# kornelski/cavif-rs

Measured on AMD Instinct MI355X. Metric: MPix/s encoded at speed=4 q=80, 1080p batch; bit-exact vs CPU oracle, higher is better.
Workload: dtype u16 samples / i32 transform / i64 RD cost

## Files before the change

### cavif_rs_amd/csrc/dev_predict.h

```cpp
#pragma once
#include "dev_common.h"

#define EDGE_OFF 16
#define EDGE_LEN(N) (EDGE_OFF + 2 * (N) + 16)

__device__ __forceinline__ const uint8_t *sm_weights_dev(int log2w) {
  static __device__ const uint8_t sw[124] = { 255, 149, 85, 64,
                                              255, 197, 146, 105, 73, 50, 37, 32,
                                              255, 225, 196, 170, 145, 123, 102, 84, 68, 54, 43, 33, 26, 20, 17, 16,
                                              255, 240, 225, 210, 196, 182, 169, 157, 145, 133, 122, 111, 101, 92, 83, 74,
                                              66, 59, 52, 45, 39, 34, 29, 25, 21, 17, 14, 12, 10, 9, 8, 8,
                                              255, 248, 240, 233, 225, 218, 210, 203, 196, 189, 182, 176, 169, 163, 156, 150,
                                              144, 138, 133, 127, 121, 116, 111, 106, 101, 96, 91, 86, 82, 77, 73, 69,
                                              65, 61, 57, 54, 50, 47, 44, 41, 38, 35, 32, 29, 27, 25, 22, 20,
                                              18, 16, 15, 13, 12, 10, 9, 8, 7, 6, 6, 5, 5, 4, 4, 4 };
  const int l = ((log2w >= 2) & (log2w <= 5)) ? log2w : 6;
  return sw + ((1 << l) - 4);
}
__device__ __forceinline__ int dr_deriv_dev(int a) {
  const int aa = (unsigned)a < 90u ? a : 0;
  const int k = (aa * 43) >> 7;
  const unsigned long long w01 = k < 8 ? 0x97b2d7117423ff00ULL : 0x4047505a00667484ULL, w23 = k < 24 ? 0x171b1f23282d3339ULL : 0x000003070b000f13ULL;
  const unsigned long long w = k < 16 ? w01 : w23;
  const int v = lut8(w, k & 7) | ((int)((0x16cULL >> (2 * k)) & 3) << 8);
  const int r = (int)((0xf035554000eaaa03ULL >> (2 * k)) & 3);
  return aa - 3 * k == r ? v : 0;
}
__device__ __forceinline__ int edge_strength_dev(int w, int h, int ft, int delta) {
  const int d = imin_(iabs_(delta), 254), blk = w + h;
  const int c = (blk > 8) + (blk > 12) + (blk > 16) + (blk > 24) + (blk > 32);
  const unsigned long long t1 = ft == 0 ? 0x010108282838ULL : 0x010104141428ULL, t2 = ft == 0 ? 0x010410ffffffULL : 0x010104303040ULL;
  const unsigned long long t3 = ft == 0 ? 0x012020ffffffULL : 0x010104ffffffULL;
  return (d >= lut8(t1, c)) + (d >= lut8(t2, c)) + (d >= lut8(t3, c));
}
__device__ __forceinline__ int edge_upsample_sel_dev(int w, int h, int ft, int delta) {
  const int d = iabs_(delta), blk = w + h;
  return (int)((d > 0) & (d < 40) & (blk <= (ft == 0 ? 16 : 8)));
}
__device__ __forceinline__ void dr_dxdy_dev(int pa, int *dx, int *dy) {
  *dx = dr_deriv_dev(pa < 90 ? pa : 180 - pa);
  *dy = dr_deriv_dev(pa < 180 ? pa - 90 : 270 - pa);
}
static __device__ const uint32_t dr_dxdy_tab[91] = {
    0x300000, 0x0003ff, 0x000223, 0x000174, 0x200111, 0x2000d7, 0x2000b2, 0x200097, 0x200084, 0x200074, 0x200066, 0x300000, 0x00005a,
    0x000050, 0x000047, 0x000040, 0x000039, 0x000033, 0x00002d, 0x100028, 0x100023, 0x10001f, 0x10001b, 0x100017, 0x100013, 0x10000f,
    0x300000, 0x00000b, 0x000007, 0x000003, 0x300000, 0x0ffc03, 0x088c07, 0x05d00b, 0x24440f, 0x235c13, 0x22c817, 0x225c1b, 0x22101f,
    0x21d023, 0x219828, 0x300000, 0x01682d, 0x014033, 0x011c39, 0x010040, 0x00e447, 0x00cc50, 0x00b45a, 0x10a066, 0x108c74, 0x107c84,
    0x106c97, 0x105cb2, 0x104cd7, 0x103d11, 0x300000, 0x002d74, 0x001e23, 0x000fff, 0x300000, 0x000c00, 0x001c00, 0x002c00, 0x203c00,
    0x204c00, 0x205c00, 0x206c00, 0x207c00, 0x208c00, 0x20a000, 0x300000, 0x00b400, 0x00cc00, 0x00e400, 0x010000, 0x011c00, 0x014000,
    0x016800, 0x119800, 0x11d000, 0x121000, 0x125c00, 0x12c800, 0x135c00, 0x144400, 0x300000, 0x05d000, 0x088c00, 0x0ffc00, 0x300000 };
__device__ __forceinline__ void dr_dxdy_uni(int pa, int *dx, int *dy) {
  const int p = (unsigned)pa <= 270u ? pa : 0, k = (p * 683) >> 11;
  const uint32_t e = dr_dxdy_tab[k];
  const bool has = p - 3 * k == (int)(e >> 20);
  *dx = has ? (int)(e & 1023) : 0; *dy = has ? (int)((e >> 10) & 1023) : 0;
}

__device__ inline void load_edges(const LDS FrameDev *f, int plane, int x, int y, int n, int have_left, int have_above,
                                  int have_ar, int have_bl, LDS uint16_t *above , LDS uint16_t *left) {
  const int bd = f->bd, rs = f->stride;
  const uint16_t *rec = f->rec[plane];
  const int max_x = f->mi_cols * 4 - 1, max_y = f->mi_rows * 4 - 1;
  const int tot = 2 * n;
  const int na = x + (have_ar ? 2 * n : n) - 1, nl = y + (have_bl ? 2 * n : n) - 1;
  const int lim_a = imin_(max_x, na), lim_l = imin_(max_y, nl);
  for (int i = LANE; i <= tot; i += 64) {
    const bool corner = i == tot;
    int ia, il;
    if (have_above) ia = (y - 1) * rs + (corner ? (have_left ? x - 1 : x) : imin_(lim_a, x + i));
    else ia = y * rs + (have_left ? x - 1 : x);
    if (have_left) il = imin_(lim_l, y + i) * rs + x - 1;
    else il = (have_above ? y - 1 : y) * rs + x;
    uint16_t a = rec[ia], l = rec[il];
    if (!have_above && !have_left) { a = (uint16_t)(corner ? (1 << (bd - 1)) : (1 << (bd - 1)) - 1); l = (uint16_t)((1 << (bd - 1)) + 1); }
    if (corner) { above[-1] = a; left[-1] = a; }
    else { above[i] = a; left[i] = l; }
  }
  WAVE_SYNC();
}

__device__ inline void edge_filter_dev(LDS uint16_t *buf, int sz, int strength, LDS uint16_t *tmp) {
  if (!strength) return;
  for (int i = LANE; i < sz; i += 64) tmp[i] = buf[i - 1];
  WAVE_SYNC();
  for (int i = 1 + LANE; i < sz; i += 64) {
    int s = 0;
#pragma unroll
    for (int j = 0; j < 5; j++) {
      const int k = iclamp_(i - 2 + j, 0, sz - 1);
      const int kw = strength == 1 ? (j == 0 || j == 4 ? 0 : (j == 2 ? 8 : 4)) : (strength == 2 ? (j == 0 || j == 4 ? 0 : (j == 2 ? 6 : 5)) : (j == 0 || j == 4 ? 2 : 4));
      s += kw * tmp[k];
    }
    buf[i - 1] = (uint16_t)((s + 8) >> 4);
  }
  WAVE_SYNC();
}
__device__ inline void edge_upsample_dev(LDS uint16_t *buf, int num_px, int bd, LDS uint16_t *tmp) {
  for (int i = LANE; i < num_px + 3; i += 64) {
    uint16_t v;
    if (i == 0) v = buf[-1]; else if (i == num_px + 2) v = buf[num_px - 1]; else v = buf[i - 2];
    tmp[i] = v;
  }
  WAVE_SYNC();
  const int mx = (1 << bd) - 1;
  if (LANE == 0) buf[-2] = tmp[0];
  for (int i = LANE; i < num_px; i += 64) {
    int s = -(int)tmp[i] + 9 * (int)tmp[i + 1] + 9 * (int)tmp[i + 2] - (int)tmp[i + 3];
    s = iclamp_(round2_(s, 4), 0, mx);
    buf[2 * i - 1] = (uint16_t)s;
    buf[2 * i] = tmp[i + 2];
  }
  WAVE_SYNC();
}

__device__ inline void predict_block(const LDS FrameDev *f, int x, int y, int log2w, int have_left, int have_above,
                                     int mode, int angle_delta, int ftype, const LDS uint16_t *ra, const LDS uint16_t *rl,
                                     LDS uint16_t *wa, LDS uint16_t *wl, LDS uint16_t *tmp, LDS uint16_t *pred) {
  const int n = 1 << log2w, bd = f->bd, nn = n * n;
  const int max_x = f->mi_cols * 4 - 1, max_y = f->mi_rows * 4 - 1;
  if (mode == PAETH_PRED) {
    const int tl = ra[-1];
    for (int idx = LANE; idx < nn; idx += 64) {
      const int i = idx >> log2w, j = idx & (n - 1);
      const int base = ra[j] + rl[i] - tl;
      const int pl = iabs_(base - rl[i]), pt = iabs_(base - ra[j]), ptl = iabs_(base - tl);
      pred[idx] = (pl <= pt && pl <= ptl) ? rl[i] : (pt <= ptl ? ra[j] : (uint16_t)tl);
    }
  } else if (mode == DC_PRED) {
    int v;
    if (have_left || have_above) {
      int s = 0;
      for (int k = LANE; k < n; k += 64) s += (have_above ? ra[k] : 0) + (have_left ? rl[k] : 0);
      s = wave_sum_i32(s);
      if (have_left && have_above) v = (s + n) / (2 * n);
      else v = (s + (n >> 1)) >> log2w;
    } else v = 1 << (bd - 1);
    for (int idx = LANE; idx < nn; idx += 64) pred[idx] = (uint16_t)v;
  } else if (mode == SMOOTH_PRED || mode == SMOOTH_V_PRED || mode == SMOOTH_H_PRED) {
    const uint8_t *sw = sm_weights_dev(log2w);
    const int bl = rl[n - 1], tr = ra[n - 1];
    for (int idx = LANE; idx < nn; idx += 64) {
      const int i = idx >> log2w, j = idx & (n - 1);
      int p;
      if (mode == SMOOTH_PRED) p = round2_(sw[i] * ra[j] + (256 - sw[i]) * bl + sw[j] * rl[i] + (256 - sw[j]) * tr, 9);
      else if (mode == SMOOTH_V_PRED) p = round2_(sw[i] * ra[j] + (256 - sw[i]) * bl, 8);
      else p = round2_(sw[j] * rl[i] + (256 - sw[j]) * tr, 8);
      pred[idx] = (uint16_t)p;
    }
  } else {
    const int pa = mode_angle_of(mode) + angle_delta * 3;
    for (int i = LANE; i < 2 * n + 1; i += 64) { wa[i - 1] = ra[i - 1]; wl[i - 1] = rl[i - 1]; }
    WAVE_SYNC();
    int up_a = 0, up_l = 0;
    if (pa != 90 && pa != 180) {
      if (pa > 90 && pa < 180 && 2 * n >= 24) {
        if (LANE == 0) { const int v = round2_(wl[0] * 5 + wa[-1] * 6 + wa[0] * 5, 4); wa[-1] = (uint16_t)v; wl[-1] = (uint16_t)v; }
        WAVE_SYNC();
      }
      if (have_above) {
        const int st = edge_strength_dev(n, n, ftype, pa - 90);
        const int num = imin_(n, max_x - x + 1) + (pa < 90 ? n : 0) + 1;
        edge_filter_dev(wa, num, st, tmp);
      }
      if (have_left) {
        const int st = edge_strength_dev(n, n, ftype, pa - 180);
        const int num = imin_(n, max_y - y + 1) + (pa > 180 ? n : 0) + 1;
        edge_filter_dev(wl, num, st, tmp);
      }
    }
    up_a = edge_upsample_sel_dev(n, n, ftype, pa - 90);
    if (up_a) edge_upsample_dev(wa, n + (pa < 90 ? n : 0), bd, tmp);
    up_l = edge_upsample_sel_dev(n, n, ftype, pa - 180);
    if (up_l) edge_upsample_dev(wl, n + (pa > 180 ? n : 0), bd, tmp);
    int dx, dy;
    dr_dxdy_dev(pa, &dx, &dy);
    for (int idx = LANE; idx < nn; idx += 64) {
      const int i = idx >> log2w, j = idx & (n - 1);
      int v;
      if (pa < 90) {
        const int max_base = (2 * n - 1) << up_a;
        const int id = (i + 1) * dx, base = (id >> (6 - up_a)) + (j << up_a), sh = ((id << up_a) >> 1) & 0x1F;
        v = base < max_base ? round2_(wa[base] * (32 - sh) + wa[base + 1] * sh, 5) : wa[max_base];
      } else if (pa > 90 && pa < 180) {
        int id = (j << 6) - (i + 1) * dx, base = id >> (6 - up_a);
        if (base >= -(1 << up_a)) { const int sh = ((id << up_a) >> 1) & 0x1F; v = round2_(wa[base] * (32 - sh) + wa[base + 1] * sh, 5); }
        else { id = (i << 6) - (j + 1) * dy; base = id >> (6 - up_l); const int sh = ((id << up_l) >> 1) & 0x1F; v = round2_(wl[base] * (32 - sh) + wl[base + 1] * sh, 5); }
      } else if (pa > 180) {
        const int id = (j + 1) * dy, base = (id >> (6 - up_l)) + (i << up_l), sh = ((id << up_l) >> 1) & 0x1F;
        v = round2_(wl[base] * (32 - sh) + wl[base + 1] * sh, 5);
      } else if (pa == 90) v = wa[j];
      else v = wl[i];
      pred[idx] = (uint16_t)v;
    }
  }
  WAVE_SYNC();
}

__device__ inline void predict_cfl_dev(const LDS FrameDev *f, int x, int y, int log2w, int alpha, const LDS uint16_t *dcp, LDS uint16_t *out) {
  const int n = 1 << log2w, nn = n * n, mx = (1 << f->bd) - 1, rs = f->stride;
  const uint16_t *luma = f->rec[0] + y * rs + x;
  int s = 0;
  for (int idx = LANE; idx < nn; idx += 64) s += luma[(idx >> log2w) * rs + (idx & (n - 1))] << 3;
  s = wave_sum_i32(s);
  const int avg = round2_(s, 2 * log2w);
  for (int idx = LANE; idx < nn; idx += 64) {
    const int l = (luma[(idx >> log2w) * rs + (idx & (n - 1))] << 3) - avg;
    const int v = alpha * l;
    const int sc = v >= 0 ? round2_(v, 6) : -round2_(-v, 6);
    out[idx] = (uint16_t)iclamp_(dcp[idx] + sc, 0, mx);
  }
  WAVE_SYNC();
}
```

### cavif_rs_amd/csrc/dev_rate.h

```cpp
#pragma once
#include "dev_common.h"

template <typename FP, typename TP> __device__ inline void txb_ctx_dev(FP f, TP t, int plane, int r4, int c4, int txs, int bs, int *skip_ctx, int *dc_ctx) {
  const int w4 = 1 << txs, ms = f->mi_stride;
  int top = 0, left = 0, dcs = 0, any_a = 0, any_l = 0;
  const int k = LANE;
  if (k < w4) {
    const bool ha = r4 - 1 >= t->mi_row_start && c4 + k < f->mi_cols, hl = c4 - 1 >= t->mi_col_start && r4 + k < f->mi_rows;
    const int ia = ha ? (r4 - 1) * ms + c4 + k : r4 * ms + c4, il = hl ? (r4 + k) * ms + c4 - 1 : r4 * ms + c4;
    const int la = f->m_lvl[plane][ia], da = f->m_dc[plane][ia], ll = f->m_lvl[plane][il], dl = f->m_dc[plane][il];
    if (ha) { top = la; any_a = la | da; dcs += da == 1 ? -1 : (da == 2 ? 1 : 0); }
    if (hl) { left = ll; any_l = ll | dl; dcs += dl == 1 ? -1 : (dl == 2 ? 1 : 0); }
  }
  top = wave_max_i32(top); left = wave_max_i32(left); dcs = wave_sum_i32(dcs);
  any_a = wave_or_i32(any_a); any_l = wave_or_i32(any_l);
  *dc_ctx = dcs < 0 ? 1 : (dcs > 0 ? 2 : 0);
  if (plane == 0) {
    int ctx;
    if (bs == txs) ctx = 0;
    else if (top == 0 && left == 0) ctx = 1;
    else if (top == 0 || left == 0) ctx = 2 + (imax_(top, left) > 3);
    else if (imax_(top, left) <= 3) ctx = 4;
    else if (imin_(top, left) <= 3) ctx = 5;
    else ctx = 6;
    *skip_ctx = ctx;
  } else {
    *skip_ctx = 7 + (any_a != 0) + (any_l != 0) + (bs > txs ? 3 : 0);
  }
}
template <typename FP, typename TP> __device__ inline void txb_ctx_wh(FP f, TP t, int plane, int r4, int c4, int w4, int h4, int whole, int *skip_ctx, int *dc_ctx) {
  const int ms = f->mi_stride;
  int top = 0, left = 0, dcs = 0, any_a = 0, any_l = 0;
  const int k = LANE;
  if (k < imax_(w4, h4)) {
    const bool ha = k < w4 && r4 - 1 >= t->mi_row_start && c4 + k < f->mi_cols, hl = k < h4 && c4 - 1 >= t->mi_col_start && r4 + k < f->mi_rows;
    const int ia = ha ? (r4 - 1) * ms + c4 + k : r4 * ms + c4, il = hl ? (r4 + k) * ms + c4 - 1 : r4 * ms + c4;
    const int la = f->m_lvl[plane][ia], da = f->m_dc[plane][ia], ll = f->m_lvl[plane][il], dl = f->m_dc[plane][il];
    if (ha) { top = la; any_a = la | da; dcs += da == 1 ? -1 : (da == 2 ? 1 : 0); }
    if (hl) { left = ll; any_l = ll | dl; dcs += dl == 1 ? -1 : (dl == 2 ? 1 : 0); }
  }
  top = wave_max_i32(top); left = wave_max_i32(left); dcs = wave_sum_i32(dcs);
  any_a = wave_or_i32(any_a); any_l = wave_or_i32(any_l);
  *dc_ctx = dcs < 0 ? 1 : (dcs > 0 ? 2 : 0);
  if (plane == 0) {
    int ctx;
    if (whole) ctx = 0;
    else if (top == 0 && left == 0) ctx = 1;
    else if (top == 0 || left == 0) ctx = 2 + (imax_(top, left) > 3);
    else if (imax_(top, left) <= 3) ctx = 4;
    else if (imin_(top, left) <= 3) ctx = 5;
    else ctx = 6;
    *skip_ctx = ctx;
  } else *skip_ctx = 7 + (any_a != 0) + (any_l != 0) + (whole ? 0 : 3);
}

__device__ __forceinline__ int eob_to_pt(int eob) { return eob < 3 ? eob : (32 - __clz(eob - 1) + 1); }
__device__ __forceinline__ int eob_pt_cdf(int eob_multi, int pt, int cls) {
  const int off[7] = { CDF_EOB_PT_16, CDF_EOB_PT_32, CDF_EOB_PT_64, CDF_EOB_PT_128, CDF_EOB_PT_256, CDF_EOB_PT_512, CDF_EOB_PT_1024 };
  const int str[7] = { CDF_EOB_PT_16_STRIDE, CDF_EOB_PT_32_STRIDE, CDF_EOB_PT_64_STRIDE, CDF_EOB_PT_128_STRIDE,
                       CDF_EOB_PT_256_STRIDE, CDF_EOB_PT_512_STRIDE, CDF_EOB_PT_1024_STRIDE };
  return off[eob_multi] + (pt * 2 + (cls == TXC_2D ? 0 : 1)) * str[eob_multi];
}
__device__ __forceinline__ int base_ctx(const LDS uint8_t *L, int st, int cls, int row, int col) {
  int mag = imin_(L[1], 3) + imin_(L[st], 3);
  if (cls == TXC_2D) {
    mag += imin_(L[st + 1], 3) + imin_(L[2], 3) + imin_(L[2 * st], 3);
    const int m = imin_((mag + 1) >> 1, 4);
    if (row == 0 && col == 0) return 0;
    if (row + col < 2) return m + 1;
    if (row + col < 4) return m + 6;
    return m + 21;
  } else if (cls == TXC_VERT) {
    mag += imin_(L[2 * st], 3) + imin_(L[3 * st], 3) + imin_(L[4 * st], 3);
    const int m = imin_((mag + 1) >> 1, 4);
    return m + (row == 0 ? 26 : (row == 1 ? 31 : 36));
  }
  mag += imin_(L[2], 3) + imin_(L[3], 3) + imin_(L[4], 3);
  const int m = imin_((mag + 1) >> 1, 4);
  return m + (col == 0 ? 26 : (col == 1 ? 31 : 36));
}
__device__ __forceinline__ int br_ctx(const LDS uint8_t *L, int st, int cls, int row, int col, int c) {
  int mag = imin_(L[1], 15) + imin_(L[st], 15);
  if (cls == TXC_2D) { mag += imin_(L[st + 1], 15); mag = imin_((mag + 1) >> 1, 6); return c == 0 ? mag : ((row < 2 && col < 2) ? mag + 7 : mag + 14); }
  if (cls == TXC_HORIZ) { mag += imin_(L[2], 15); mag = imin_((mag + 1) >> 1, 6); return c == 0 ? mag : (col == 0 ? mag + 7 : mag + 14); }
  mag += imin_(L[2 * st], 15); mag = imin_((mag + 1) >> 1, 6); return c == 0 ? mag : (row == 0 ? mag + 7 : mag + 14);
}

__device__ inline void build_level_map(const LDS int32_t *qc, LDS uint8_t *lev, int n) {
  const int st = n + 4, words = (st * st + 3) >> 2, bwl = n == 4 ? 2 : n == 8 ? 3 : n == 16 ? 4 : 5;
  LDS uint32_t *lw = (LDS uint32_t *)lev;
  for (int i = LANE; i < words; i += 64) lw[i] = 0;
  WAVE_SYNC();
  for (int i = LANE; i < n * n; i += 64) lev[(i >> bwl) * st + (i & (n - 1))] = (uint8_t)imin_(iabs_(qc[i]), 127);
  WAVE_SYNC();
}

struct CoefCost { const LDS uint16_t *txb, *eobx, *dcs, *br, *base, *beob, *eobpt[4]; };
__device__ __forceinline__ int coef_cost_entries(int maxtxs) {
  const int t = maxtxs + 1, tb = imin_(maxtxs, 3) + 1;
  return t * 13 * CDF_TXB_SKIP_STRIDE + t * 18 * CDF_EOB_EXTRA_STRIDE + 6 * CDF_DC_SIGN_STRIDE + tb * 42 * CDF_COEFF_BR_STRIDE +
         t * 84 * CDF_COEFF_BASE_STRIDE + t * 8 * CDF_COEFF_BASE_EOB_STRIDE + 4 * (CDF_EOB_PT_16_STRIDE + CDF_EOB_PT_64_STRIDE + CDF_EOB_PT_256_STRIDE + CDF_EOB_PT_1024_STRIDE);
}
#define COEF_COST_MAX_ENTRIES(maxtxs) (((maxtxs) + 1) * (13 * 3 + 18 * 3 + 84 * 5 + 8 * 4) + 18 + ((maxtxs) < 3 ? (maxtxs) + 1 : 4) * 42 * 5 + 4 * (6 + 8 + 10 + 12))
__device__ __forceinline__ CoefCost coef_cost_layout(const LDS uint16_t *dst, int maxtxs, int *src_off = nullptr, int *count = nullptr) {
  const int t = maxtxs + 1, tb = imin_(maxtxs, 3) + 1;
  const int src[10] = { CDF_TXB_SKIP, CDF_EOB_EXTRA, CDF_DC_SIGN, CDF_COEFF_BR, CDF_COEFF_BASE, CDF_COEFF_BASE_EOB, CDF_EOB_PT_16, CDF_EOB_PT_64, CDF_EOB_PT_256, CDF_EOB_PT_1024 };
  const int cnt[10] = { t * 13 * CDF_TXB_SKIP_STRIDE, t * 18 * CDF_EOB_EXTRA_STRIDE, 6 * CDF_DC_SIGN_STRIDE, tb * 42 * CDF_COEFF_BR_STRIDE, t * 84 * CDF_COEFF_BASE_STRIDE,
                        t * 8 * CDF_COEFF_BASE_EOB_STRIDE, 4 * CDF_EOB_PT_16_STRIDE, 4 * CDF_EOB_PT_64_STRIDE, 4 * CDF_EOB_PT_256_STRIDE, 4 * CDF_EOB_PT_1024_STRIDE };
  int o[10]; int acc = 0;
#pragma unroll
  for (int i = 0; i < 10; i++) { o[i] = acc; acc += cnt[i]; if (src_off) src_off[i] = src[i]; if (count) count[i] = cnt[i]; }
  CoefCost cc;
  cc.txb = dst + o[0]; cc.eobx = dst + o[1]; cc.dcs = dst + o[2]; cc.br = dst + o[3]; cc.base = dst + o[4]; cc.beob = dst + o[5];
  cc.eobpt[0] = dst + o[6]; cc.eobpt[1] = dst + o[7]; cc.eobpt[2] = dst + o[8]; cc.eobpt[3] = dst + o[9];
  return cc;
}
__device__ inline void load_coef_cost(LDS uint16_t *dst, const uint16_t *cost, int maxtxs, int tid, int nthreads) {
  int src[10], cnt[10];
  coef_cost_layout(dst, maxtxs, src, cnt);
  int o = 0;
  for (int k = 0; k < 10; k++) { for (int i = tid; i < cnt[k]; i += nthreads) dst[o + i] = cost[src[k] + i]; o += cnt[k]; }
}

template <typename CostPtr> __device__ inline uint32_t coef_rate_dev(const CoefCost &cc, CostPtr cost, const LDS uint16_t *ls, const LDS int32_t *qc, int eob, int plane, int txs, int txtype,
                                         int skip_ctx, int dc_ctx, int tx_off, int tx_sym, LDS uint8_t *lev, int *cul_out, int *dc_cat) {
  const int n = imin_(32, 4 << txs), bwl = n == 4 ? 2 : n == 8 ? 3 : n == 16 ? 4 : 5;
  const int pt = plane > 0, cls = tx_class_of(txtype), txs_ctx = txs;
  *cul_out = 0; *dc_cat = 0;
  uint32_t head = cc.txb[(txs_ctx * 13 + skip_ctx) * CDF_TXB_SKIP_STRIDE + (eob == 0)];
  if (eob == 0) return head;
  if (tx_off >= 0) head += cost[tx_off + tx_sym];
  const int eob_pt = eob_to_pt(eob), eob_multi = 2 * bwl - 4;
  {
    static_assert(CDF_EOB_PT_16_STRIDE == 6 && CDF_EOB_PT_64_STRIDE == 8 && CDF_EOB_PT_256_STRIDE == 10 && CDF_EOB_PT_1024_STRIDE == 12, "stride = 6 + 2 sq");
    const int sq = eob_multi >> 1;
    head += cc.eobpt[sq][(pt * 2 + (cls == TXC_2D ? 0 : 1)) * (6 + 2 * sq) + eob_pt - 1];
  }
  if (eob_pt >= 3) {
    const int nb = eob_pt - 2, rem = eob - ((1 << (eob_pt - 2)) + 1), hi = (rem >> (nb - 1)) & 1;
    head += cc.eobx[((txs_ctx * 2 + pt) * 9 + (eob_pt - 3)) * CDF_EOB_EXTRA_STRIDE + hi];
    head += 512u * (uint32_t)(nb - 1);
  }
  build_level_map(qc, lev, n);
  const int st = n + 4, area = n * n;
  int bits = 0; int cul = 0, dcc = 0;
  for (int c = LANE; c < eob; c += 64) {
    const int p = scan_pos(ls, n, cls, c), row = p >> bwl, col = p & (n - 1);
    const int v = qc[p], level = iabs_(v);
    const LDS uint8_t *L = lev + row * st + col;
    if (c == eob - 1) {
      const int ctx = c == 0 ? 0 : (c <= area / 8 ? 1 : (c <= area / 4 ? 2 : 3));
      bits += cc.beob[((txs_ctx * 2 + pt) * 4 + ctx) * CDF_COEFF_BASE_EOB_STRIDE + imin_(level, 3) - 1];
    } else {
      const int ctx = base_ctx(L, st, cls, row, col);
      bits += cc.base[((txs_ctx * 2 + pt) * 42 + ctx) * CDF_COEFF_BASE_STRIDE + imin_(level, 3)];
    }
    if (level > 2) {
      const int ctx = br_ctx(L, st, cls, row, col, c);
      const int off = ((imin_(txs_ctx, 3) * 2 + pt) * 21 + ctx) * CDF_COEFF_BR_STRIDE;
      int rem = level - 3;
      for (int idx = 0; idx < 4; idx++) { const int s = imin_(rem, 3); bits += cc.br[off + s]; rem -= s; if (s < 3) break; }
    }
    if (level) {
      if (c == 0) { bits += cc.dcs[(pt * 3 + dc_ctx) * CDF_DC_SIGN_STRIDE + (v < 0)]; dcc = v < 0 ? 1 : 2; }
      else bits += 512;
      if (level > 14) { const int len = 32 - __clz(level - 14); bits += 512 * (2 * len - 1); }
    }
    cul += level;
  }
  bits = wave_sum_i32(bits);
  cul = wave_sum_i32(imin_(cul, 1 << 20));
  dcc = __builtin_amdgcn_readfirstlane(dcc);
  *cul_out = imin_(cul, 63); *dc_cat = dcc;
  return head + (uint32_t)bits;
}

#define LEV_OFF(cs) ((cs) == 4 ? 0 : (cs) == 8 ? 64 : (cs) == 16 ? 64 + 144 : 64 + 144 + 400)
#define LEV_BYTES(maxcs) ((maxcs) == 4 ? 64 : (maxcs) == 8 ? 64 + 144 : (maxcs) == 16 ? 64 + 144 + 400 : 64 + 144 + 400 + 1296)

template <int CS, typename CostPtr>
__device__ inline int quant_rate_dev(const CoefCost &cc, CostPtr cost, const LDS uint16_t *ls, LDS int32_t *cbuf, LDS int32_t *qc, LDS uint8_t *levbase,
                                     int plane, int txs, int txtype, int dcq, int acq, uint32_t dc_recip, uint32_t ac_recip, int bd,
                                     int skip_ctx, int dc_ctx, int tx_off, int tx_sym, uint32_t *rate_out, int *cul_out, int *dc_cat) {
  constexpr int n = CS, nc = CS * CS, IT = nc < 64 ? 1 : nc / 64, bwl = CS == 4 ? 2 : CS == 8 ? 3 : CS == 16 ? 4 : 5, st = CS + 4;
  LDS uint8_t *lev = levbase + LEV_OFF(CS);
  const uint32_t tx_cost = cost[tx_off >= 0 ? tx_off + tx_sym : 0];
  const int cls = tx_class_of(txtype), pt = plane > 0, txs_ctx = txs;
  const int lsh = txs == 3 ? 1 : (txs == 4 ? 2 : 0);
  const uint32_t dc_off = (uint32_t)(dcq * 109 / 256), off0 = (uint32_t)(acq * 98 / 256), off1 = (uint32_t)(acq * 109 / 256), off_eob = (uint32_t)(acq * 88 / 256);
  const uint32_t thr = (uint32_t)acq - off_eob, uq = (uint32_t)acq;
  int pos[IT]; uint32_t mag[IT]; int neg[IT];
  int last = 0;
#pragma unroll
  for (int k = 0; k < IT; k++) {
    const int i = LANE + 64 * k;
    const bool valid = nc >= 64 || i < nc;
    pos[k] = valid ? scan_pos(ls, n, cls, i) : 0;
    const int c = valid ? cbuf[pos[k]] : 0;
    mag[k] = (uint32_t)iabs_(c) << lsh; neg[k] = c < 0;
    if (valid && i >= 1 && mag[k] >= thr) last = i + 1;
  }
  last = wave_max_i32(last);
  const uint32_t x0 = ((uint32_t)iabs_(cbuf[0]) << lsh) + dc_off;
  uint32_t l0u = __umulhi(x0, dc_recip);
  if (x0 - l0u * (uint32_t)dcq >= (uint32_t)dcq) l0u++;
  const int l0 = (int)l0u;
  int eob = last;
// ... 83 lines not shown
```

### cavif_rs_amd/csrc/dev_rect.h

```cpp
#pragma once

__device__ inline void load_edges_wh(const LDS FrameDev *f, int plane, int x, int y, int w, int h, int have_left, int have_above, int have_ar, int have_bl,
                                     LDS uint16_t *above, LDS uint16_t *left) {
  const int bd = f->bd, rs = f->stride, tot = w + h;
  const uint16_t *rec = f->rec[plane];
  const int max_x = f->mi_cols * 4 - 1, max_y = f->mi_rows * 4 - 1;
  const int lim_a = imin_(max_x, x + (have_ar ? 2 * w : w) - 1), lim_l = imin_(max_y, y + (have_bl ? 2 * h : h) - 1);
  for (int i = LANE; i <= tot; i += 64) {
    const bool corner = i == tot;
    int ia, il;
    if (have_above) ia = (y - 1) * rs + (corner ? (have_left ? x - 1 : x) : imin_(lim_a, x + i));
    else ia = y * rs + (have_left ? x - 1 : x);
    if (have_left) il = imin_(lim_l, y + i) * rs + x - 1;
    else il = (have_above ? y - 1 : y) * rs + x;
    uint16_t a = rec[ia], l = rec[il];
    if (!have_above && !have_left) { a = (uint16_t)(corner ? (1 << (bd - 1)) : (1 << (bd - 1)) - 1); l = (uint16_t)((1 << (bd - 1)) + 1); }
    if (corner) { above[-1] = a; left[-1] = a; } else { above[i] = a; left[i] = l; }
  }
  WAVE_SYNC();
}

__device__ inline void predict_block_wh(const LDS FrameDev *f, int x, int y, int wl, int hl, int have_left, int have_above, int mode, int angle_delta, int ftype,
                                        const LDS uint16_t *ra, const LDS uint16_t *rl, LDS uint16_t *wa, LDS uint16_t *wl_, LDS uint16_t *tmp, LDS uint16_t *pred) {
  const int w = 1 << wl, h = 1 << hl, bd = f->bd, nn = w * h;
  const int max_x = f->mi_cols * 4 - 1, max_y = f->mi_rows * 4 - 1;
  if (mode == PAETH_PRED) {
    const int tl = ra[-1];
    for (int idx = LANE; idx < nn; idx += 64) {
      const int i = idx >> wl, j = idx & (w - 1);
      const int base = ra[j] + rl[i] - tl;
      const int pl = iabs_(base - rl[i]), pt = iabs_(base - ra[j]), ptl = iabs_(base - tl);
      pred[idx] = (pl <= pt && pl <= ptl) ? rl[i] : (pt <= ptl ? ra[j] : (uint16_t)tl);
    }
  } else if (mode == DC_PRED) {
    int v;
    if (have_left || have_above) {
      int s = 0;
      for (int k = LANE; k < imax_(w, h); k += 64) s += ((have_above && k < w) ? ra[k] : 0) + ((have_left && k < h) ? rl[k] : 0);
      s = wave_sum_i32(s);
      if (have_left && have_above) v = (s + ((w + h) >> 1)) / (w + h);
      else if (have_left) v = (s + (h >> 1)) >> hl;
      else v = (s + (w >> 1)) >> wl;
    } else v = 1 << (bd - 1);
    for (int idx = LANE; idx < nn; idx += 64) pred[idx] = (uint16_t)v;
  } else if (mode == SMOOTH_PRED || mode == SMOOTH_V_PRED || mode == SMOOTH_H_PRED) {
    const uint8_t *sw = sm_weights_dev(wl), *sh = sm_weights_dev(hl);
    const int bl = rl[h - 1], tr = ra[w - 1];
    for (int idx = LANE; idx < nn; idx += 64) {
      const int i = idx >> wl, j = idx & (w - 1);
      int p;
      if (mode == SMOOTH_PRED) p = round2_(sh[i] * ra[j] + (256 - sh[i]) * bl + sw[j] * rl[i] + (256 - sw[j]) * tr, 9);
      else if (mode == SMOOTH_V_PRED) p = round2_(sh[i] * ra[j] + (256 - sh[i]) * bl, 8);
      else p = round2_(sw[j] * rl[i] + (256 - sw[j]) * tr, 8);
      pred[idx] = (uint16_t)p;
    }
  } else {
    const int pa = mode_angle_of(mode) + angle_delta * 3;
    for (int i = LANE; i < w + h + 1; i += 64) { wa[i - 1] = ra[i - 1]; wl_[i - 1] = rl[i - 1]; }
    WAVE_SYNC();
    int up_a = 0, up_l = 0;
    if (pa != 90 && pa != 180) {
      if (pa > 90 && pa < 180 && w + h >= 24) {
        if (LANE == 0) { const int v = round2_(wl_[0] * 5 + wa[-1] * 6 + wa[0] * 5, 4); wa[-1] = (uint16_t)v; wl_[-1] = (uint16_t)v; }
        WAVE_SYNC();
      }
      if (have_above) edge_filter_dev(wa, imin_(w, max_x - x + 1) + (pa < 90 ? h : 0) + 1, edge_strength_dev(w, h, ftype, pa - 90), tmp);
      if (have_left) edge_filter_dev(wl_, imin_(h, max_y - y + 1) + (pa > 180 ? w : 0) + 1, edge_strength_dev(w, h, ftype, pa - 180), tmp);
    }
    up_a = edge_upsample_sel_dev(w, h, ftype, pa - 90);
    if (up_a) edge_upsample_dev(wa, w + (pa < 90 ? h : 0), bd, tmp);
    up_l = edge_upsample_sel_dev(w, h, ftype, pa - 180);
    if (up_l) edge_upsample_dev(wl_, h + (pa > 180 ? w : 0), bd, tmp);
    int dx, dy;
    dr_dxdy_dev(pa, &dx, &dy);
    for (int idx = LANE; idx < nn; idx += 64) {
      const int i = idx >> wl, j = idx & (w - 1);
      int v;
      if (pa < 90) {
        const int max_base = (w + h - 1) << up_a;
        const int id = (i + 1) * dx, base = (id >> (6 - up_a)) + (j << up_a), sh = ((id << up_a) >> 1) & 0x1F;
        v = base < max_base ? round2_(wa[base] * (32 - sh) + wa[base + 1] * sh, 5) : wa[max_base];
      } else if (pa > 90 && pa < 180) {
        int id = (j << 6) - (i + 1) * dx, base = id >> (6 - up_a);
        if (base >= -(1 << up_a)) { const int sh = ((id << up_a) >> 1) & 0x1F; v = round2_(wa[base] * (32 - sh) + wa[base + 1] * sh, 5); }
        else { id = (i << 6) - (j + 1) * dy; base = id >> (6 - up_l); const int sh = ((id << up_l) >> 1) & 0x1F; v = round2_(wl_[base] * (32 - sh) + wl_[base + 1] * sh, 5); }
      } else if (pa > 180) {
        const int id = (j + 1) * dy, base = (id >> (6 - up_l)) + (i << up_l), sh = ((id << up_l) >> 1) & 0x1F;
        v = round2_(wl_[base] * (32 - sh) + wl_[base + 1] * sh, 5);
      } else if (pa == 90) v = wa[j];
      else v = wl_[i];
      pred[idx] = (uint16_t)v;
    }
  }
  WAVE_SYNC();
}

__device__ inline long long satd_wh(const LDS uint16_t *src, const LDS uint16_t *pred, int w, int h) {
  const int units = w * (h >> 2);
  int total = 0;
  for (int u = LANE; u < units; u += 64) {
    const int x = u % w, o = (u / w) * 4 * w + x;
    const int d0 = (int)src[o] - (int)pred[o], d1 = (int)src[o + w] - (int)pred[o + w];
    const int d2 = (int)src[o + 2 * w] - (int)pred[o + 2 * w], d3 = (int)src[o + 3 * w] - (int)pred[o + 3 * w];
    const int a = d0 + d1, b = d0 - d1, c = d2 + d3, e = d2 - d3;
    int t[4] = { a + c, b + e, a - c, b - e };
    int s = 0;
#pragma unroll
    for (int i = 0; i < 4; i++) { int v = satd_quad_step<0xB1>(t[i], 1); v = satd_quad_step<0x4E>(v, 2); s += iabs_(v); }
    total += s;
  }
  return (long long)wave_sum_i32(total);
}

template <int W, int H> __device__ inline void fwd_txfm_rect(LDS int32_t *tbuf, LDS int32_t *coef, int txtype) {
  constexpr int P = W + 1;
  int ck, rk; tx_kinds(txtype, &ck, &rk);
  for (int c = LANE; c < W; c += 64) {
    int32_t x[H];
#pragma unroll
    for (int r = 0; r < H; r++) x[r] = tbuf[r * P + c] << 2;
    tx1d<H>(x, ck, true);
#pragma unroll
    for (int r = 0; r < H; r++) tbuf[r * P + c] = rshift_round_(x[r], 1);
  }
  WAVE_SYNC();
  for (int r = LANE; r < H; r += 64) {
    int32_t x[W];
#pragma unroll
    for (int c = 0; c < W; c++) x[c] = tbuf[r * P + c];
    tx1d<W>(x, rk, true);
#pragma unroll
    for (int c = 0; c < W; c++) coef[r * W + c] = (int32_t)(((long long)x[c] * 5793 + 2048) >> 12);
  }
  WAVE_SYNC();
}
template <int W, int H> __device__ inline void inv_txfm_rect_add(const LDS int32_t *dq, LDS int32_t *tbuf, LDS uint16_t *rec, int txtype, int bd) {
  constexpr int P = W + 1;
  int ck, rk; tx_kinds(txtype, &ck, &rk);
  const int cbits = imax_(bd + 6, 16), cmax = (1 << (cbits - 1)) - 1, cmin = -(1 << (cbits - 1));
  for (int i = LANE; i < H; i += 64) {
    int32_t x[W];
#pragma unroll
    for (int j = 0; j < W; j++) x[j] = round2_(dq[i * W + j] * 2896, 12);
    tx1d<W>(x, rk, false);
#pragma unroll
    for (int j = 0; j < W; j++) tbuf[i * P + j] = iclamp_(x[j], cmin, cmax);
  }
  WAVE_SYNC();
  const int mx = (1 << bd) - 1;
  for (int j = LANE; j < W; j += 64) {
    int32_t x[H];
#pragma unroll
    for (int i = 0; i < H; i++) x[i] = tbuf[i * P + j];
    tx1d<H>(x, ck, false);
#pragma unroll
    for (int i = 0; i < H; i++) rec[i * W + j] = (uint16_t)iclamp_((int)rec[i * W + j] + round2_(x[i], 4), 0, mx);
  }
  WAVE_SYNC();
}

template <typename CostPtr>
__device__ inline int rect_quant_rate(CostPtr cost, LDS int32_t *cbuf, LDS int32_t *qc, LDS uint8_t *lev, int plane, int wl, int hl, int txtype, int dcq, int acq,
                                      uint32_t dc_recip, uint32_t ac_recip, int bd, int skip_ctx, int dc_ctx, int tx_off, int tx_sym, uint32_t *rate_out, int *cul_out, int *dc_cat) {
  const int w = 1 << wl, h = 1 << hl, nc = w * h, st = w + 4;
  const int cls = tx_class_of(txtype), pt = plane > 0, txs_ctx = 1;
  const uint32_t dc_off = (uint32_t)(dcq * 109 / 256), off0 = (uint32_t)(acq * 98 / 256), off1 = (uint32_t)(acq * 109 / 256), off_eob = (uint32_t)(acq * 88 / 256);
  const uint32_t thr = (uint32_t)acq - off_eob, uq = (uint32_t)acq;
  const int i = LANE, valid = i < nc;
  const int pos = valid ? rect_scan_pos(wl, hl, cls, i) : 0;
// ... 155 lines not shown
  int last = 0;
#pragma unroll
  for (int k = 0; k < IT; k++) {
    const int i = gl + 16 * k;
    pos[k] = rect_scan_pos(WL, HL, cls, i);
    const int c = gb->cbuf[pos[k]];
    mag[k] = (uint32_t)iabs_(c); neg[k] = c < 0;
    if (i >= 1 && mag[k] >= thr) last = i + 1;
  }
  last = row_max_i32(last);
  const uint32_t x0 = (uint32_t)iabs_(gb->cbuf[0]) + dc_off;
  uint32_t l0u = __umulhi(x0, dc_recip);
  if (x0 - l0u * (uint32_t)dcq >= (uint32_t)dcq) l0u++;
  const int l0 = (int)l0u;
  int eob = last;
  if (eob == 0) eob = l0 ? 1 : 0;
  const int dmx = (1 << (7 + bd)) - 1, dmn = -(1 << (7 + bd));
  int lvl[IT];
  WAVE_SYNC();
#pragma unroll
  for (int k = 0; k < IT; k++) {
    const int i = gl + 16 * k;
    int lv = 0;
    if (i < eob) {
      if (i == 0) lv = l0;
      else {
        const uint32_t a = mag[k];
        uint32_t lv0 = __umulhi(a, ac_recip);
        if (a - lv0 * uq >= uq) lv0++;
        const uint32_t off = lv0 > 0 ? off1 : off0;
        lv = (int)lv0 + ((a + off) >= (lv0 + 1) * uq);
      }
    }
    lvl[k] = lv;
    const int pp = pos[k];
    gb->qc[pp] = neg[k] ? -lv : lv;
    gb->lev[(pp >> WL) * st + (pp & (W - 1))] = (uint8_t)imin_(lv, 127);
    uint32_t m = (uint32_t)lv * (uint32_t)(pp == 0 ? dcq : acq);
    m &= 0xFFFFFF;
    const int v = neg[k] ? -(int)m : (int)m;
    gb->cbuf[pp] = v < dmn ? dmn : (v > dmx ? dmx : v);
  }
  WAVE_SYNC();
  uint32_t head = cc.txb[(txs_ctx * 13 + skip_ctx) * CDF_TXB_SKIP_STRIDE + (eob == 0)];
  int bits = 0, cul = 0, dcc = 0;
  const int eob_pt = eob_to_pt(imax_(eob, 1));
  const uint32_t ep = (uint32_t)__shfl((int)ep_cost, (LANE & 48) + eob_pt - 1);
  if (eob > 0) {
    if (tx_off >= 0) head += tx_cost;
    head += ep;
    if (eob_pt >= 3) {
      const int nb = eob_pt - 2, rem = eob - ((1 << (eob_pt - 2)) + 1), hi = (rem >> (nb - 1)) & 1;
      head += cc.eobx[((txs_ctx * 2 + pt) * 9 + (eob_pt - 3)) * CDF_EOB_EXTRA_STRIDE + hi];
      head += 512u * (uint32_t)(nb - 1);
    }
#pragma unroll
    for (int k = 0; k < IT; k++) {
      const int c = gl + 16 * k;
      if (c < eob) {
        const int pp = pos[k], row = pp >> WL, col = pp & (W - 1), level = lvl[k];
        const LDS uint8_t *L = gb->lev + row * st + col;
        if (c == eob - 1) {
          const int ctx = c == 0 ? 0 : (c <= nc / 8 ? 1 : (c <= nc / 4 ? 2 : 3));
          bits += cc.beob[((txs_ctx * 2 + pt) * 4 + ctx) * CDF_COEFF_BASE_EOB_STRIDE + imin_(level, 3) - 1];
        } else {
          int ctx = base_ctx(L, st, cls, row, col);
          if (cls == TXC_2D && !(row == 0 && col == 0)) {
            const int mg = imin_(L[1], 3) + imin_(L[st], 3) + imin_(L[st + 1], 3) + imin_(L[2], 3) + imin_(L[2 * st], 3), m = imin_((mg + 1) >> 1, 4);
            ctx = HL > WL ? m + (row < 2 ? 11 : (row + col < 4 ? 6 : 21)) : m + (col < 2 ? 16 : (row + col < 4 ? 6 : 21));
          }
          bits += cc.base[((txs_ctx * 2 + pt) * 42 + ctx) * CDF_COEFF_BASE_STRIDE + imin_(level, 3)];
        }
        if (level > 2) {
          const int off = ((txs_ctx * 2 + pt) * 21 + br_ctx(L, st, cls, row, col, c)) * CDF_COEFF_BR_STRIDE;
          int rem = level - 3;
          for (int idx = 0; idx < 4; idx++) { const int s2 = imin_(rem, 3); bits += cc.br[off + s2]; rem -= s2; if (s2 < 3) break; }
        }
        if (level) {
          if (c == 0) { bits += cc.dcs[(pt * 3 + dc_ctx) * CDF_DC_SIGN_STRIDE + neg[k]]; dcc = neg[k] ? 1 : 2; }
          else bits += 512;
          if (level > 14) { const int len = 32 - __clz(level - 14); bits += 512 * (2 * len - 1); }
        }
        cul += level;
      }
    }
  }
  bits = row_sum_i32(bits);
  cul = row_sum_i32(imin_(cul, 1 << 20));
  dcc = row_max_i32(dcc);
  res->eob = eob; res->cul = imin_(cul, 63); res->dcc = dcc; res->rate = head + (uint32_t)bits;
  {
    const int cbits = imax_(bd + 6, 16), cmax = (1 << (cbits - 1)) - 1, cmin = -(1 << (cbits - 1));
    const bool act_r = gl < H && eob > 0, act_c = gl < W && eob > 0;
    if (act_r) {
      int32_t x[W];
#pragma unroll
      for (int j = 0; j < W; j++) x[j] = round2_(gb->cbuf[gl * W + j] * 2896, 12);
      tx1d<W>(x, rk, false);
#pragma unroll
      for (int j = 0; j < W; j++) gb->tbuf[gl * P + j] = iclamp_(x[j], cmin, cmax);
    }
    WAVE_SYNC();
    const int mx = (1 << bd) - 1;
    if (act_c) {
      int32_t x[H];
#pragma unroll
      for (int i = 0; i < H; i++) x[i] = gb->tbuf[i * P + gl];
      tx1d<H>(x, ck, false);
#pragma unroll
      for (int i = 0; i < H; i++) gb->rec[i * W + gl] = (uint16_t)iclamp_((int)gb->rec[i * W + gl] + round2_(x[i], 4), 0, mx);
    }
    WAVE_SYNC();
  }
  int se[2] = { 0, 0 }, sd[2] = { 0, 0 }, qd[2] = { 0, 0 };
#pragma unroll
  for (int k = 0; k < IT; k++) {
    const int idx = gl + 16 * k, i = idx >> WL, j = idx & (W - 1), cell = W == 8 ? (j >> 2) : (i >> 2);
    const int rv = gb->rec[idx], d = (int)src[idx] - rv;
    se[cell] += __mul24(d, d); sd[cell] += rv; qd[cell] += __mul24(rv, rv);
  }
  if (psv_a >= 0) {
    int dist = 0;
#pragma unroll
    for (int cell = 0; cell < 2; cell++)
      dist += psy_cell_dist((uint32_t)row_sum_i32(se[cell]), (uint32_t)row_sum_i32(sd[cell]), (uint32_t)row_sum_i32(qd[cell]), (uint32_t)(cell ? psv_b : psv_a), (uint32_t)psy_act, 4, bd);
    res->sse = dist;
  } else res->sse = (int)(((unsigned long long)(uint32_t)row_sum_i32(se[0] + se[1]) * (uint32_t)psy_act + 8192) >> 14);
}

template <int WL, int HL> __device__ inline void commit_rect(const LDS FrameDev *f, int plane, int r, int c, const LDS uint16_t *rec, const LDS int32_t *qc, int eob, int cul, int dcc) {
  constexpr int W = 1 << WL, H = 1 << HL;
  uint16_t *gr = f->rec[plane] + (size_t)(r * 4) * f->stride + c * 4;
  int32_t *gc = f->coef[plane] + (size_t)(r * 4) * f->stride + c * 4;
  for (int idx = LANE; idx < W * H; idx += 64) { gr[(idx >> WL) * f->stride + (idx & (W - 1))] = rec[idx]; gc[(idx >> WL) * f->stride + (idx & (W - 1))] = qc[idx]; }
  if (LANE < 2) { const int rr = r + (H == 8 ? LANE : 0), cc = c + (W == 8 ? LANE : 0); f->m_lvl[plane][rr * f->mi_stride + cc] = (uint8_t)cul; f->m_dc[plane][rr * f->mi_stride + cc] = (uint8_t)dcc; }
  if (LANE == 0) f->m_eob[plane][r * f->mi_stride + c] = (uint16_t)eob;
}
template <int WL, int HL> __device__ __forceinline__ void fill_rect(uint8_t *m, int ms, int r, int c, int v) {
  if (LANE < 2) m[(r + (HL == 3 ? LANE : 0)) * ms + c + (WL == 3 ? LANE : 0)] = (uint8_t)v;
}

template <int MAXN, int BSR, int NW, int TS>
__device__ MI_K1_TRY_ATTR long long try_block_rect(const Ctx<MAXN, NW, TS> k, int r, int c, long long budget = J_INF) {
  static_assert(NW == 4 && MAXN <= 32, "the 2:1 block search deals its candidates to four wavefronts (its chroma stages hard-code the wave roles; no one-candidate-per-wave fallback is left)");
  constexpr int WL = BSR == BS_4X8 ? 2 : 3, HL = BSR == BS_4X8 ? 3 : 2, W_ = 1 << WL, H_ = 1 << HL, NN = W_ * H_, w4 = W_ >> 2, h4 = H_ >> 2;
  const LDS FrameDev *f = k.f(); const LDS TileB *t = k.t(); LDS WaveScratch<MAXN> *S = k.s(); LDS SharedScratch<MAXN> *SH = k.sh();
  const int W = NW > 1 ? WAVE_ID : 0;
  const int ms = f->mi_stride, mi = r * ms + c, x = c * 4, y = r * 4;
  const int availU = r > t->mi_row_start, availL = c > t->mi_col_start;
  const int can_ar = availU && (c + w4 < t->mi_col_end), can_bl = availL && (r + h4 < t->mi_row_end);
  const int iU = availU ? mi - ms : mi, iL = availL ? mi - 1 : mi;
  constexpr int SHAPE = BSR == BS_8X4 ? 1 : 2;
  const int have_ar = can_ar && decoded_before(r, c, SHAPE, r - 1, c + w4), have_bl = can_bl && decoded_before(r, c, SHAPE, r + h4, c - 1);
  const int amode = availU ? uni32(f->m_ymode[iU]) : DC_PRED, lmode = availL ? uni32(f->m_ymode[iL]) : DC_PRED;
  const int uvU = f->np > 1 ? uni32(f->m_uvmode[iU]) : 0, uvL = f->np > 1 ? uni32(f->m_uvmode[iL]) : 0;
  const int v_skU = f->m_skip[iU], v_skL = f->m_skip[iL], v_skUL = f->m_skip[availU && availL ? mi - ms - 1 : mi];
  const int nb_skip = (availU ? uni32(v_skU) & 1 : 0) + (availL ? uni32(v_skL) & 1 : 0);
  const int seg_nb = (availU && availL ? (uni32(v_skUL) >> 1) + 1 : 0) | ((availU ? (uni32(v_skU) >> 1) + 1 : 0) << 4) | ((availL ? (uni32(v_skL) >> 1) + 1 : 0) << 8);
  const int nb_txU = availU ? uni32(f->m_txsize[iU]) : -1, nb_txL = availL ? uni32(f->m_txsize[iL]) : -1;
  const uint16_t *ycost = k.cost() + CDF_KF_Y + (intra_mode_ctx(amode) * 5 + intra_mode_ctx(lmode)) * CDF_KF_Y_STRIDE;
  const int ftype_y = IS_SMOOTH_(amode) || IS_SMOOTH_(lmode);
  const int ftype_uv = f->np > 1 && ((availU && IS_SMOOTH_(uvU)) || (availL && IS_SMOOTH_(uvL)));
  LDS uint16_t *wa = S->wa + EDGE_OFF, *wl = S->wl + EDGE_OFF;
  PH_BEGIN();

  for (int p = 0; p < f->np; p++) if (p % NW == W) {
    int sc_, dc_;
    txb_ctx_wh(f, t, p, r, c, w4, h4, 1, &sc_, &dc_);
    if (LANE == 0) { SH->sctx[p] = sc_; SH->dctx[p] = dc_; }
    const uint16_t *g = f->src[p] + (size_t)y * f->stride + x;
    for (int idx = LANE; idx < NN; idx += 64) SH->srcb[p][idx] = g[(idx >> WL) * f->stride + (idx & (W_ - 1))];
    load_edges_wh(f, p, x, y, W_, H_, availL, availU, have_ar, have_bl, SH->ra[p] + EDGE_OFF, SH->rl[p] + EDGE_OFF);
  }
  if (W == NW - 1) {
    const int a = (int)f->act[(y >> 3) * (f->pw >> 3) + (x >> 3)];
    if (LANE < 2) SH->psv4[LANE] = (int)f->svar4[(r + (HL == 3 ? LANE : 0)) * ms + c + (WL == 3 ? LANE : 0)];
    if (LANE == 0) { SH->pact[0] = a; SH->cact = a; SH->seg_nb = seg_nb; }
    seg_select(f, SH, a);
  }
  PH(1);
  WG_SYNC();
  PH(2);
  const int sctx_y = SH->sctx[0], dctx_y = SH->dctx[0];
  const LDS uint16_t *ra = SH->ra[0] + EDGE_OFF, *rl = SH->rl[0] + EDGE_OFF;
  const int psv_a = Tools<TS>::tune_psnr(f) ? 0 : SH->psv4[0], psv_b = Tools<TS>::tune_psnr(f) ? 0 : SH->psv4[1], act = SH->pact[0];

  for (int m = W; m < 13; m += NW) {
    predict_block_wh(f, x, y, WL, HL, availL, availU, m, 0, ftype_y, ra, rl, wa, wl, S->etmp, S->pred);
    const long long sd = satd_wh(SH->srcb[0], S->pred, W_, H_);
    if (LANE == 0) SH->satd[m] = sd;
  }
  PH(3);
  WG_SYNC();
  if (LANE < 13) {
    const long long mine = SH->satd[LANE];
    int rank = 0;
    for (int j = 0; j < 13; j++) { const long long o = SH->satd[j]; rank += (o < mine) || (o == mine && j < LANE); }
    SH->order[rank] = LANE;
  }
  WG_SYNC();
  const int ncand = Tools<TS>::FULL ? 7 : 3;
  int tx_ns = 0, tx_set = 0;
  const int tx_off0 = rect_tx_cdf(f, Tools<TS>::reduced_tx_set(f), 0, &tx_ns, &tx_set);
  const int ntx = (Tools<TS>::rdo_tx(f) && tx_off0 >= 0) ? tx_ns : 1;
  LDS uint16_t *pcache = MAXN <= 16 ? (LDS uint16_t *)SH->lpred : (LDS uint16_t *)SH->split_rec;
  for (int ci = W; ci < ncand; ci += NW) predict_block_wh(f, x, y, WL, HL, availL, availU, SH->order[ci], 0, ftype_y, ra, rl, wa, wl, S->etmp, pcache + ci * NN);
  PH(12);
  WG_SYNC();
  long long my_j = J_INF; int my_e = 1 << 30, my_mode = DC_PRED, my_tx = DCT_DCT, cur = 0; TxRes my_tr = { 0, 0, 0, 0, 0 }; uint32_t my_mrate = 0;
  constexpr bool CAN_GROUP = NW == 4 && MAXN <= 32;
  bool grouped = false, parked = false; int my_g = 0;
  if constexpr (CAN_GROUP) grouped = true;
  if constexpr (CAN_GROUP) if (grouped) {
    const int g = GROUP_ID, total = ncand * ntx, rounds = (total + 15) >> 4;
    LDS uint16_t *park_rec = (LDS uint16_t *)S->dcp; LDS int32_t *park_qc = (LDS int32_t *)(S->dcp + 64);
    for (int rd = 0; rd < rounds; rd++) {
      int e;
      if (ncand == 3 && ntx == 5) e = g < 3 ? g * 5 + W : (W < 3 ? W * 5 + 4 : -1);
      else e = rd * 16 + W * 4 + g;
      const bool live = e >= 0 && e < total;
      const int ee = live ? e : 0, ci = ee / ntx, ti = ee - ci * ntx, m = SH->order[ci];
      const uint32_t mode_rate = ycost[m];
      int ns2, set2;
      const int tx_off = rect_tx_cdf(f, Tools<TS>::reduced_tx_set(f), m, &ns2, &set2);
      int txtype;
      if (ntx > 1) txtype = sym_to_txtype(tx_set, ti);
      else { txtype = mode_to_txtype(m); if (tx_off < 0 || txtype_to_sym(tx_set, txtype) < 0) txtype = DCT_DCT; }
      GroupRes gr;
      eval_group_wh<WL, HL>(k.cc(), k.cost(), f, &S->grp[g], SH->srcb[0], pcache + ci * NN, 0, txtype, sctx_y, dctx_y, tx_off, tx_off >= 0 ? txtype_to_sym(tx_set, txtype) : 0,
                            Tools<TS>::tune_psnr(f) ? -1 : psv_a, psv_b, act, &gr);
      long long j = rd_dist32(f, 0, gr.sse) + rd_rate32(f, gr.rate) + rd_rate32(f, mode_rate);
      if (!live) j = J_INF;
      bool improved = false;
#pragma unroll
      for (int gg = 0; gg < 4; gg++) {
        const long long jg = ((long long)__builtin_amdgcn_readlane((int)(j >> 32), gg * 16) << 32) | (unsigned int)__builtin_amdgcn_readlane((int)j, gg * 16);
        const int eg = __builtin_amdgcn_readlane(e, gg * 16);
        if (jg < my_j || (jg == my_j && eg < my_e)) {
          my_j = jg; my_e = eg; my_g = gg; improved = true;
          my_mode = __builtin_amdgcn_readlane(m, gg * 16); my_tx = __builtin_amdgcn_readlane(txtype, gg * 16);
          my_tr.eob = __builtin_amdgcn_readlane(gr.eob, gg * 16); my_tr.cul = __builtin_amdgcn_readlane(gr.cul, gg * 16); my_tr.dcc = __builtin_amdgcn_readlane(gr.dcc, gg * 16);
          my_mrate = (uint32_t)__builtin_amdgcn_readlane((int)mode_rate, gg * 16);
        }
      }
      if (rounds > 1 && improved) {
        for (int i = LANE; i < NN; i += 64) { park_rec[i] = S->grp[my_g].rec[i]; park_qc[i] = S->grp[my_g].qc[i]; }
        parked = true;
        WAVE_SYNC();
      }
    }
  }
  if (!grouped)
  for (int e = W; e < ncand * ntx; e += NW) {
    const int ci = e / ntx, ti = e - ci * ntx, m = SH->order[ci];
    const LDS uint16_t *cpred = pcache + ci * NN;
    const uint32_t mode_rate = ycost[m];
    int ns2, set2;
    const int tx_off = rect_tx_cdf(f, Tools<TS>::reduced_tx_set(f), m, &ns2, &set2);
    int txtype;
    if (ntx > 1) txtype = sym_to_txtype(tx_set, ti);
    else { txtype = mode_to_txtype(m); if (tx_off < 0 || txtype_to_sym(tx_set, txtype) < 0) txtype = DCT_DCT; }
    TxRes tr;
    long long j = eval_rect<MAXN, WL, HL, NW>(k, 0, sctx_y, dctx_y, SH->srcb[0], cpred, txtype, tx_off, tx_off >= 0 ? txtype_to_sym(tx_set, txtype) : 0, S->rec[cur], S->qc[cur], &tr, psv_a, psv_b, act);
    j += ((long long)mode_rate * f->rdmult + 256) >> 9;
    if (j < my_j) { my_j = j; my_e = e; my_mode = m; my_tx = txtype; my_tr = tr; my_mrate = mode_rate; cur ^= 1; }
  }
  if (LANE == 0) { SH->wbest_j[W] = my_j; SH->wbest_e[W] = my_e; }
  PH(6);
  WG_SYNC();
  int win = 0;
  for (int w2 = 1; w2 < NW; w2++) if (SH->wbest_j[w2] < SH->wbest_j[win] || (SH->wbest_j[w2] == SH->wbest_j[win] && SH->wbest_e[w2] < SH->wbest_e[win])) win = w2;
  const long long best_j = SH->wbest_j[win];
  if (W == win) {
    const int b = cur ^ 1;
    const LDS uint16_t *best_rec = S->rec[b]; const LDS int32_t *best_qc = S->qc[b];
    if constexpr (CAN_GROUP) if (grouped) {
      if (parked) { best_rec = (const LDS uint16_t *)S->dcp; best_qc = (const LDS int32_t *)(S->dcp + 64); }
      else { best_rec = S->grp[my_g].rec; best_qc = S->grp[my_g].qc; }
    }
    commit_rect<WL, HL>(f, 0, r, c, best_rec, best_qc, my_tr.eob, my_tr.cul, my_tr.dcc);
    fill_rect<WL, HL>(f->m_ymode, ms, r, c, my_mode);
    fill_rect<WL, HL>((uint8_t *)f->m_angle_y, ms, r, c, 0);
    fill_rect<WL, HL>(f->m_txtype, ms, r, c, my_tr.eob ? my_tx : DCT_DCT);
    fill_rect<WL, HL>(f->m_bsize, ms, r, c, BSR);
    fill_rect<WL, HL>(f->m_txsize, ms, r, c, BSR);
    if (f->np > 1) for (int i = LANE; i < NN; i += 64) SH->luma_rec[i] = best_rec[i];
    if (LANE == 0) { SH->lm_mode = my_mode; SH->lm_eob = my_tr.eob; SH->lm_mode_j = ((long long)my_mrate * f->rdmult + 256) >> 9; SH->lm_tx = my_tr.cul; SH->lm_delta = my_tr.dcc; }
  }
  WG_SYNC();
  const int best_mode = SH->lm_mode;
  long long luma_j = best_j; int any_coef = SH->lm_eob > 0;
  if (Tools<TS>::tx_mode_select(f)) {
    const int actx = nb_txU >= 0 && dim_wl(nb_txU) >= WL, lctx = nb_txL >= 0 && dim_hl(nb_txL) >= HL;
    const uint16_t *dcost = k.cost() + CDF_TX_SIZE + (actx + lctx) * CDF_TX_SIZE_STRIDE;
    luma_j += ((long long)dcost[0] * f->rdmult + 256) >> 9;
    if (Tools<TS>::rdo_tx(f)) {
      long long j_split = SH->lm_mode_j + (((long long)dcost[1] * f->rdmult + 256) >> 9);
      int stx_ns = 0, stx_set = 0;
      const int stx_off = intra_tx_cdf_r(f, Tools<TS>::reduced_tx_set(f), 0, best_mode, &stx_ns, &stx_set);
      const int sntx = stx_off >= 0 ? stx_ns : 1;
      LDS uint16_t *split_rec = (LDS uint16_t *)SH->ssrc + 64;
      LDS int32_t *split_qc = MAXN <= 16 ? (LDS int32_t *)SH->lpred : (LDS int32_t *)SH->split_qc;
      LDS int *sub = (LDS int *)SH->dsd;
      int sub_any = 0;
      if (W == 0) for (int idx = LANE; idx < NN; idx += 64) { const int q = W_ == 8 ? ((idx & 7) >> 2) : (idx >> 4), i = (idx >> WL) & 3, j = idx & 3; SH->ssrc[q * 16 + i * 4 + j] = SH->srcb[0][idx]; }
      if (W == 1 && LANE < 4) {
        const int q = LANE >> 1, side = LANE & 1, rr = r + (H_ == 8 ? q : 0), cc = c + (W_ == 8 ? q : 0);
        const bool inner = q == 1 && (side == 0 ? H_ == 8 : W_ == 8);
        const bool have = !inner && (side == 0 ? (rr - 1 >= t->mi_row_start && cc < f->mi_cols) : (cc - 1 >= t->mi_col_start && rr < f->mi_rows));
        const int ia = have ? (side == 0 ? (rr - 1) * ms + cc : rr * ms + cc - 1) : rr * ms + cc;
        const int l = f->m_lvl[0][ia], d = f->m_dc[0][ia];
        sub[8 + LANE] = have ? (l | (d << 8) | (1 << 16)) : 0;
      }
      WG_SYNC();
      {
        constexpr int CH_BYTES = NN * 2 + NN * 4 + 2 * 4;
        const int g = GROUP_ID, gl = GROUP_LANE;
        const int e = sntx == 5 ? (W == 0 ? g + 1 : ((W == 1 && g == 0) ? 0 : 64)) : W * 4 + g;
        const bool has_chain = e < sntx, wave_has = sntx == 5 ? W < 2 : W * 4 < sntx;
        LDS long long *const cres_j = (LDS long long *)SH->cj; LDS int *const cres_any = (LDS int *)(cres_j + 8);
        const long long thr = luma_j < budget ? luma_j : budget;
        if (wave_has) {
          LDS uint8_t *cst = (LDS uint8_t *)k.wave(2 + W) + g * CH_BYTES;
          LDS uint16_t *canvas = (LDS uint16_t *)cst; LDS int32_t *cqc = (LDS int32_t *)(cst + NN * 2); LDS uint32_t *cmeta = (LDS uint32_t *)(cst + NN * 2 + NN * 4);
          LDS uint16_t *A = S->pred + g * 64 + EDGE_OFF, *Lf = A + 32, *ppred = S->dcp + g * 64;
          int txtype;
          if (sntx > 1) txtype = sym_to_txtype(stx_set, has_chain ? e : 0);
          else { txtype = mode_to_txtype(best_mode); if (stx_off < 0 || txtype_to_sym(stx_set, txtype) < 0) txtype = DCT_DCT; }
          const int tx_sym = stx_off >= 0 ? txtype_to_sym(stx_set, txtype) : 0;
          const bool dirm = best_mode >= V_PRED && best_mode <= D67_PRED;
          const int pa = dirm ? mode_angle_of(best_mode) : 0;
          const int max_x = f->mi_cols * 4 - 1, max_y = f->mi_rows * 4 - 1, rs = f->stride, bd = f->bd;
          const uint16_t *grec = f->rec[0];
          long long jc = has_chain ? j_split : J_INF;
          int any = 0;
#pragma unroll 1
          for (int q = 0; q < 2; q++) {
            if (MI_BALLOT64(jc < thr) == 0ull) break;
            const int bi = H_ == 8 ? q : 0, bj = W_ == 8 ? q : 0, rr = r + bi, cc = c + bj, sx = x + bj * 4, sy = y + bi * 4;
            const int sU = availU || bi, sL = availL || bj;
            {
              const bool c_ar = sU && cc + 1 < t->mi_col_end, c_bl = sL && rr + 1 < t->mi_row_end;
              const int s_ar = c_ar && decoded_before(r, c, SHAPE, rr - 1, cc + 1), s_bl = c_bl && decoded_before(r, c, SHAPE, rr + 1, cc - 1);
              const int lim_a = imin_(max_x, sx + (s_ar ? 8 : 4) - 1), lim_l = imin_(max_y, sy + (s_bl ? 8 : 4) - 1);
              auto px = [&](int ax, int ay) -> int {
                const int xr = ax - x, yr = ay - y;
                if (xr >= 0 && xr < W_ && yr >= 0 && yr < H_) return (int)canvas[yr * W_ + xr];
                if (yr == -1 && xr >= -1 && xr < W_ + H_) return (int)ra[xr];
                if (xr == -1 && yr >= 0 && yr < W_ + H_) return (int)rl[yr];
                return (int)grec[(size_t)ay * rs + ax];
              };
              for (int i = gl; i <= 8; i += 16) {
                const bool corner = i == 8;
                int a, l;
                if (sU) a = px(corner ? (sL ? sx - 1 : sx) : imin_(lim_a, sx + i), sy - 1); else a = px(sL ? sx - 1 : sx, sy);
                if (sL) l = px(sx - 1, imin_(lim_l, sy + i)); else l = px(sx, sU ? sy - 1 : sy);
                if (!sU && !sL) { a = corner ? (1 << (bd - 1)) : (1 << (bd - 1)) - 1; l = (1 << (bd - 1)) + 1; }
                if (corner) { A[-1] = (uint16_t)a; Lf[-1] = (uint16_t)a; } else { A[i] = (uint16_t)a; Lf[i] = (uint16_t)l; }
              }
            }
            WAVE_SYNC();
            if (dirm) predict_dir_group<4>(f, sx, sy, sL, sU, pa, ftype_y, A, Lf, &S->gpred[g], ppred);
            else predict_nondir_group<4>(best_mode, sL, sU, bd, A, Lf, ppred);
            int ssc, sdc;
            {
              const uint32_t m0 = q ? cmeta[0] : 0u;
              const int inner = (int)(((m0 >> 16) & 0xFF) | ((m0 >> 24) << 8) | (1u << 16));
              const int nt = (q == 1 && H_ == 8) ? inner : sub[8 + 2 * q], nl = (q == 1 && W_ == 8) ? inner : sub[8 + 2 * q + 1];
              const int top = (nt >> 16) ? (nt & 0xFF) : 0, left = (nl >> 16) ? (nl & 0xFF) : 0, dt = (nt >> 16) ? ((nt >> 8) & 0xFF) : 0, dl = (nl >> 16) ? ((nl >> 8) & 0xFF) : 0;
              const int dcs = (dt == 1 ? -1 : (dt == 2 ? 1 : 0)) + (dl == 1 ? -1 : (dl == 2 ? 1 : 0));
              sdc = dcs < 0 ? 1 : (dcs > 0 ? 2 : 0);
              if (top == 0 && left == 0) ssc = 1;
              else if (top == 0 || left == 0) ssc = 2 + (imax_(top, left) > 3);
              else if (imax_(top, left) <= 3) ssc = 4;
              else if (imin_(top, left) <= 3) ssc = 5;
              else ssc = 6;
            }
            GroupRes gr;
            eval_group<4>(k.cc(), k.cost(), k.ls(), f, &S->grp[g], SH->ssrc + q * 16, ppred, 0, 0, txtype, ssc, sdc, stx_off, tx_sym, Tools<TS>::tune_psnr(f) ? -1 : SH->psv4[q], SH->pact[0], &gr);
            if (has_chain) jc += rd_dist32(f, 0, gr.sse) + rd_rate32(f, gr.rate);
            {
              const LDS uint16_t *srec = S->grp[g].rec; const LDS int32_t *sqc = S->grp[g].qc;
              canvas[(bi * 4 + (gl >> 2)) * W_ + bj * 4 + (gl & 3)] = srec[gl]; cqc[q * 16 + gl] = sqc[gl];
              cmeta[q] = (uint32_t)gr.eob | ((uint32_t)gr.cul << 16) | ((uint32_t)gr.dcc << 24);
            }
            any |= gr.eob > 0;
            WAVE_SYNC();
          }
          const int slot = sntx == 5 ? (W == 0 ? g + 1 : (g == 0 ? 0 : 4 + g)) : W * 4 + g;
          cres_j[slot] = (has_chain && jc < thr) ? jc : J_INF; cres_any[slot] = any;
        }
        WG_SYNC();
        int be = -1; long long bjc = J_INF;
        for (int e2 = 0; e2 < sntx; e2++) { const long long v = cres_j[e2]; if (v < bjc) { bjc = v; be = e2; } }
        j_split = bjc;
        if (be >= 0) {
          const int ow = sntx == 5 ? (be == 0 ? 1 : 0) : be >> 2, og = sntx == 5 ? (be == 0 ? 0 : be - 1) : be & 3;
          if (W == ow) {
            const LDS uint8_t *cst = (const LDS uint8_t *)k.wave(2 + W) + og * CH_BYTES;
            const LDS uint16_t *canvas = (const LDS uint16_t *)cst; const LDS int32_t *cqc = (const LDS int32_t *)(cst + NN * 2); const LDS uint32_t *cmeta = (const LDS uint32_t *)(cst + NN * 2 + NN * 4);
            if (LANE < NN) { split_rec[LANE] = canvas[LANE]; split_qc[LANE] = cqc[LANE]; }
            int btx;
            if (sntx > 1) btx = sym_to_txtype(stx_set, be);
            else { btx = mode_to_txtype(best_mode); if (stx_off < 0 || txtype_to_sym(stx_set, btx) < 0) btx = DCT_DCT; }
            if (LANE < 2) { const uint32_t m = cmeta[LANE]; const int eob = (int)(m & 0xFFFF); sub[LANE * 4 + 0] = eob ? btx : DCT_DCT; sub[LANE * 4 + 1] = eob; sub[LANE * 4 + 2] = (int)((m >> 16) & 0xFF); sub[LANE * 4 + 3] = (int)(m >> 24); }
          }
          sub_any = cres_any[be];
          WG_SYNC();
        }
      }
      if (j_split < luma_j) {
        luma_j = j_split; any_coef = sub_any;
        uint16_t *gr_ = f->rec[0] + (size_t)y * f->stride + x;
        int32_t *gc_ = f->coef[0] + (size_t)y * f->stride + x;
        for (int i = threadIdx.x; i < NN; i += 64 * NW) {
          const uint16_t v = split_rec[i]; gr_[(i >> WL) * f->stride + (i & (W_ - 1))] = v; if (f->np > 1) SH->luma_rec[i] = v;
          const int q = W_ == 8 ? ((i & 7) >> 2) : (i >> 4), ii = (i >> WL) & 3, jj = i & 3;
          gc_[(i >> WL) * f->stride + (i & (W_ - 1))] = split_qc[q * 16 + ii * 4 + jj];
        }
        if (W == 0 && LANE < 2) {
          const int rr = r + (H_ == 8 ? LANE : 0), cc = c + (W_ == 8 ? LANE : 0), o = rr * ms + cc;
          f->m_txsize[o] = 0; f->m_txtype[o] = (uint8_t)sub[LANE * 4 + 0]; f->m_eob[0][o] = (uint16_t)sub[LANE * 4 + 1];
          f->m_lvl[0][o] = (uint8_t)sub[LANE * 4 + 2]; f->m_dc[0][o] = (uint8_t)sub[LANE * 4 + 3];
        }
      } else if (W == 0 && LANE < 2) {
        const int o = (r + (H_ == 8 ? LANE : 0)) * ms + c + (W_ == 8 ? LANE : 0);
        f->m_lvl[0][o] = (uint8_t)SH->lm_tx; f->m_dc[0][o] = (uint8_t)SH->lm_delta;
      }
      WG_SYNC();
    }
  }
  if (luma_j >= budget) return luma_j;
  long long total_j = luma_j;
  PH(13);
  bool cgrouped = false;
  if constexpr (CAN_GROUP) cgrouped = f->np > 1 && !Tools<TS>::FULL;
  if constexpr (CAN_GROUP) if (cgrouped) {
    const uint16_t *uvcost = k.cost() + CDF_UV_CFL + best_mode * CDF_UV_CFL_STRIDE;
    const int nplain = best_mode != DC_PRED ? 2 : 1, nc = nplain + 1, uvset = Tools<TS>::reduced_tx_set(f) ? 2 : 1;
    const int mx = (1 << f->bd) - 1;
    {
      const int p = (W >> 1) + 1, half = W & 1;
      const LDS uint16_t *luma = SH->luma_rec;
      int lsum = LANE < NN ? (int)luma[LANE] << 3 : 0;
      lsum = wave_sum_i32(lsum);
      const int avg = round2_(lsum, WL + HL);
      predict_block_wh(f, x, y, WL, HL, availL, availU, DC_PRED, 0, ftype_uv, SH->ra[p] + EDGE_OFF, SH->rl[p] + EDGE_OFF, wa, wl, S->etmp, S->dcp);
      long long best_sse = J_INF; int best_idx = 1 << 20;
      const int l = LANE < NN ? ((int)luma[LANE] << 3) - avg : 0, dcv = LANE < NN ? (int)S->dcp[LANE] : 0, sv = LANE < NN ? (int)SH->srcb[p][LANE] : 0;
      if (half == 0) { const int d = sv - dcv; best_sse = (long long)wave_sum_i32(LANE < NN ? d * d : 0); best_idx = -1; }
      const int la = iabs_(l), ng = l < 0;
#pragma unroll
      for (int kq = 0; kq < 8; kq++) {
        const int mag = half * 8 + kq + 1;
        const int rr = round2_(__mul24(mag, la), 6), sc = ng ? -rr : rr;
        const int dp = sv - iclamp_(dcv + sc, 0, mx), dm = sv - iclamp_(dcv - sc, 0, mx);
        const long long ep = (long long)wave_sum_i32(LANE < NN ? __mul24(dp, dp) : 0), em = (long long)wave_sum_i32(LANE < NN ? __mul24(dm, dm) : 0);
        if (ep < best_sse) { best_sse = ep; best_idx = half * 16 + 2 * kq; }
        if (em < best_sse) { best_sse = em; best_idx = half * 16 + 2 * kq + 1; }
      }
      if (LANE == 0) { SH->ca_sse[p - 1][half] = best_sse; SH->ca_idx[p - 1][half] = best_idx; }
    }
    WG_SYNC();
    int alpha_u = 0, alpha_v = 0;
// ... 40 lines not shown
    for (int cnd = 0; cnd < 3; cnd++) {
      if (cnd < nc) {
        const int is_cfl = cnd == nc - 1, um = is_cfl ? UV_CFL_PRED : (cnd == 0 ? DC_PRED : best_mode);
        int jsign = 0;
        const uint32_t mode_rate = uv_mode_rate(k.cost(), uvcost, um, false, 0, is_cfl && cfl_ok, alpha_u, alpha_v, &jsign);
        if (!is_cfl || cfl_ok) {
          const long long j = SH->cj[cnd][0] + SH->cj[cnd][1] + rd_rate32(f, mode_rate);
          if (j < best_uv) { best_uv = j; bc = cnd; b_sign = jsign; }
        }
      }
    }
    if (cw) {
      const int p = (W >> 1) + 1, chose_cfl = bc == nc - 1;
      const int beob = __builtin_amdgcn_readlane(gr.eob, bc * 16), bcul = __builtin_amdgcn_readlane(gr.cul, bc * 16), bdcc = __builtin_amdgcn_readlane(gr.dcc, bc * 16);
      commit_rect<WL, HL>(f, p, r, c, S->grp[bc].rec, S->grp[bc].qc, beob, bcul, bdcc);
      if (LANE == 0) SH->ceob[p - 1] = beob;
      if (p == 1) {
        fill_rect<WL, HL>(f->m_uvmode, ms, r, c, chose_cfl ? UV_CFL_PRED : (bc == 0 ? DC_PRED : best_mode));
        fill_rect<WL, HL>((uint8_t *)f->m_angle_uv, ms, r, c, 0);
        fill_rect<WL, HL>(f->m_cfl_sign, ms, r, c, chose_cfl ? b_sign : 0);
        fill_rect<WL, HL>(f->m_cfl_au, ms, r, c, (chose_cfl && alpha_u) ? iabs_(alpha_u) - 1 : 0);
        fill_rect<WL, HL>(f->m_cfl_av, ms, r, c, (chose_cfl && alpha_v) ? iabs_(alpha_v) - 1 : 0);
      }
    }
    WG_SYNC();
    any_coef |= (SH->ceob[0] > 0) | (SH->ceob[1] > 0);
    total_j += best_uv;
  }
  if constexpr (Tools<TS>::FULL) if (f->np > 1 && !cgrouped) {
    const uint16_t *uvcost = k.cost() + CDF_UV_CFL + best_mode * CDF_UV_CFL_STRIDE;
    unsigned long long cand_pack = 0; int nc = 0;
    auto push = [&](int m) { cand_pack |= (unsigned long long)m << (4 * nc); nc++; };
    push(DC_PRED);
    if (best_mode != DC_PRED) push(best_mode);
    if (Tools<TS>::FULL) for (int m = 1; m < 13; m++) if (m != best_mode) push(m);
    push(UV_CFL_PRED);
    const int uvset = Tools<TS>::reduced_tx_set(f) ? 2 : 1;
    const int mx = (1 << f->bd) - 1;
    const int p = (W >> 1) + 1, half = W & 1;
    const LDS uint16_t *pra = SH->ra[p] + EDGE_OFF, *prl = SH->rl[p] + EDGE_OFF;
    int lavg;
    {
      const LDS uint16_t *luma = SH->luma_rec;
      int lsum = LANE < NN ? (int)luma[LANE] << 3 : 0;
      lsum = wave_sum_i32(lsum);
      lavg = round2_(lsum, WL + HL);
      predict_block_wh(f, x, y, WL, HL, availL, availU, DC_PRED, 0, ftype_uv, pra, prl, wa, wl, S->etmp, S->dcp);
      long long best_sse = J_INF; int best_idx = 1 << 20;
      const int l = LANE < NN ? ((int)luma[LANE] << 3) - lavg : 0, dcv = LANE < NN ? (int)S->dcp[LANE] : 0, sv = LANE < NN ? (int)SH->srcb[p][LANE] : 0;
      if (half == 0) { const int d = sv - dcv; best_sse = (long long)wave_sum_i32(LANE < NN ? d * d : 0); best_idx = -1; }
      const int la = iabs_(l), ng = l < 0;
#pragma unroll
      for (int kq = 0; kq < 8; kq++) {
        const int mag = half * 8 + kq + 1;
        const int rr = round2_(__mul24(mag, la), 6), sc = ng ? -rr : rr;
        const int dp = sv - iclamp_(dcv + sc, 0, mx), dm = sv - iclamp_(dcv - sc, 0, mx);
        const long long ep = (long long)wave_sum_i32(LANE < NN ? __mul24(dp, dp) : 0), em = (long long)wave_sum_i32(LANE < NN ? __mul24(dm, dm) : 0);
        if (ep < best_sse) { best_sse = ep; best_idx = half * 16 + 2 * kq; }
        if (em < best_sse) { best_sse = em; best_idx = half * 16 + 2 * kq + 1; }
      }
      if (LANE == 0) { SH->ca_sse[p - 1][half] = best_sse; SH->ca_idx[p - 1][half] = best_idx; }
    }
    WG_SYNC();
    int alpha_u = 0, alpha_v = 0;
#pragma unroll
    for (int pp = 0; pp < 2; pp++) {
      const int idx = SH->ca_sse[pp][1] < SH->ca_sse[pp][0] ? SH->ca_idx[pp][1] : SH->ca_idx[pp][0];
      const int al = idx < 0 ? 0 : ((idx & 1) ? -((idx >> 1) + 1) : ((idx >> 1) + 1));
      if (pp == 0) alpha_u = al; else alpha_v = al;
    }
    const int cfl_ok = alpha_u != 0 || alpha_v != 0;
    LDS uint16_t *park_rec = (LDS uint16_t *)SH->lpred + (p - 1) * 96; LDS int32_t *park_qc = (LDS int32_t *)(park_rec + 32); LDS int *park_meta = (LDS int *)SH->order + (p - 1) * 3;
    long long best_uv = J_INF; int b_ci = 1 << 30, b_sign = 0, b_round = 0;
    const int ns = nc <= 4 ? 1 : 2, nrounds = nc > 4 * ns ? 2 : 1, dealt = half < ns;
    GroupRes gr = { 0, 0, 0, 0, 0 };
    const int g = GROUP_ID;
#pragma unroll 1
    for (int rd = 0; rd < nrounds; rd++) {
      const int base = nrounds == 2 && rd == 0 ? 4 * ns : 0;
#pragma unroll 1
      for (int g2 = 0; g2 < 4; g2++) {
        const int ci = base + half + ns * g2;
        if (dealt && ci < nc) {
          const int um = lut4(cand_pack, ci);
          LDS uint16_t *cp = S->pred + g2 * NN;
          if (um == UV_CFL_PRED) {
            const int al = p == 1 ? alpha_u : alpha_v;
            if (LANE < NN) { const int l = ((int)SH->luma_rec[LANE] << 3) - lavg, v = al * l, sc = v >= 0 ? round2_(v, 6) : -round2_(-v, 6); cp[LANE] = (uint16_t)iclamp_((int)S->dcp[LANE] + sc, 0, mx); }
            WAVE_SYNC();
          } else if (um != DC_PRED) predict_block_wh(f, x, y, WL, HL, availL, availU, um, 0, ftype_uv, pra, prl, wa, wl, S->etmp, cp);
        }
      }
      const int ci = base + half + ns * g, live = dealt && ci < nc;
      const int um = lut4(cand_pack, live ? ci : 0);
      int txtype = mode_to_txtype(um);
      if (txtype_to_sym(uvset, txtype) < 0) txtype = DCT_DCT;
      if (dealt) eval_group_wh<WL, HL>(k.cc(), k.cost(), f, &S->grp[g], SH->srcb[p], um == DC_PRED ? (const LDS uint16_t *)S->dcp : (const LDS uint16_t *)(S->pred + g * NN), p, txtype,
                            SH->sctx[p], SH->dctx[p], -1, 0, -1, 0, SH->cact, &gr);
      const long long jp = rd_dist32(f, p, gr.sse) + rd_rate32(f, gr.rate);
      if (GROUP_LANE == 0 && live) SH->cj[ci][p - 1] = jp;
      WG_SYNC();
      long long r_best = J_INF; int r_ci = 1 << 30, r_sign = 0;
      for (int cc = base; cc < imin_(nc, base + 4 * ns); cc++) {
        const int um2 = lut4(cand_pack, cc), is_cfl = um2 == UV_CFL_PRED;
        if (is_cfl && !cfl_ok) continue;
        int jsign = 0;
        const uint32_t mode_rate = uv_mode_rate(k.cost(), uvcost, um2, false, 0, is_cfl, alpha_u, alpha_v, &jsign);
        const long long j = SH->cj[cc][0] + SH->cj[cc][1] + rd_rate32(f, mode_rate);
        if (j < r_best) { r_best = j; r_ci = cc; r_sign = jsign; }
      }
      if (r_best < best_uv || (r_best == best_uv && r_ci < b_ci)) { best_uv = r_best; b_ci = r_ci; b_sign = r_sign; b_round = rd; }
      if (nrounds == 2 && rd == 0 && r_ci < nc && (r_ci - base) % ns == half) {
        const int gg = (r_ci - base) / ns;
        if (LANE < NN) { park_rec[LANE] = S->grp[gg].rec[LANE]; park_qc[LANE] = S->grp[gg].qc[LANE]; }
        const int e_ = __builtin_amdgcn_readlane(gr.eob, gg * 16), c_ = __builtin_amdgcn_readlane(gr.cul, gg * 16), d_ = __builtin_amdgcn_readlane(gr.dcc, gg * 16);
        if (LANE == 0) { park_meta[0] = e_; park_meta[1] = c_; park_meta[2] = d_; }
      }
    }
    const int b_um = lut4(cand_pack, b_ci), chose_cfl = b_um == UV_CFL_PRED;
    const int from_park = nrounds == 2 && b_round == 0;
    if (from_park ? half == 0 : b_ci % ns == half) {
      int beob, bcul, bdcc;
      if (from_park) {
        beob = park_meta[0]; bcul = park_meta[1]; bdcc = park_meta[2];
        commit_rect<WL, HL>(f, p, r, c, (const LDS uint16_t *)park_rec, (const LDS int32_t *)park_qc, beob, bcul, bdcc);
      } else {
        const int gg = b_ci / ns;
        beob = __builtin_amdgcn_readlane(gr.eob, gg * 16); bcul = __builtin_amdgcn_readlane(gr.cul, gg * 16); bdcc = __builtin_amdgcn_readlane(gr.dcc, gg * 16);
        commit_rect<WL, HL>(f, p, r, c, S->grp[gg].rec, S->grp[gg].qc, beob, bcul, bdcc);
      }
      if (LANE == 0) SH->ceob[p - 1] = beob;
      if (p == 1) {
        fill_rect<WL, HL>(f->m_uvmode, ms, r, c, b_um);
        fill_rect<WL, HL>((uint8_t *)f->m_angle_uv, ms, r, c, 0);
        fill_rect<WL, HL>(f->m_cfl_sign, ms, r, c, chose_cfl ? b_sign : 0);
        fill_rect<WL, HL>(f->m_cfl_au, ms, r, c, (chose_cfl && alpha_u) ? iabs_(alpha_u) - 1 : 0);
        fill_rect<WL, HL>(f->m_cfl_av, ms, r, c, (chose_cfl && alpha_v) ? iabs_(alpha_v) - 1 : 0);
      }
    }
    WG_SYNC();
    any_coef |= (SH->ceob[0] > 0) | (SH->ceob[1] > 0);
    total_j += best_uv;
  }
  PH(9);
  const int skip = !any_coef;
  int seg_ctx = 0;
  const int seg_nb2 = SH->seg_nb, seg_ul = (seg_nb2 & 15) - 1, seg_u = ((seg_nb2 >> 4) & 15) - 1, seg_l = (seg_nb2 >> 8) - 1;
  const int seg_p = seg_pred(seg_ul, seg_u, seg_l, &seg_ctx), seg_own = f->seg_n ? SH->seg : 0, seg_fin = f->seg_n ? (skip ? seg_p : seg_own) : 0;
  if (f->seg_n && !skip) total_j += ((long long)k.cost()[CDF_SEG_ID + seg_ctx * CDF_SEG_ID_STRIDE + seg_symbol(seg_own, seg_p, f->seg_n)] * f->rdmult + 256) >> 9;
  if (W == 0) {
    fill_rect<WL, HL>(f->m_skip, ms, r, c, skip | (seg_fin << 1));
    if (skip) for (int p = 0; p < f->np; p++) { fill_rect<WL, HL>(f->m_lvl[p], ms, r, c, 0); fill_rect<WL, HL>(f->m_dc[p], ms, r, c, 0); }
  }
  total_j += ((long long)k.cost()[CDF_SKIP + nb_skip * CDF_SKIP_STRIDE + skip] * f->rdmult + 256) >> 9;
  WG_SYNC();
  return total_j;
}
```

### cavif_rs_amd/csrc/tile_search.h

```cpp
#pragma once
#include "dev_common.h"
#include "dev_predict.h"
#include "dev_txfm.h"
#include "dev_rate.h"
#include "dev_group.h"

#ifndef MI_BALLOT64
#define MI_BALLOT64(p) __builtin_amdgcn_ballot_w64(p)
#endif
#define MI_K1_TRY_ATTR __attribute__((noinline, not_tail_called))
#define MI_K1_WG_PER_CU 4
#define WAVE_ID ((int)(threadIdx.x >> 6))
#ifndef MI_PROFILE
#define MI_PROFILE 0
#endif
#ifndef MI_PROF_MAXN
#define MI_PROF_MAXN 16
#endif
#ifndef MI_DEBUG_HOOKS
#define MI_DEBUG_HOOKS 0
#endif
#if MI_DEBUG_HOOKS
#define DBG_IS(f, v) ((f)->dbg == (v))
#else
#define DBG_IS(f, v) false
#endif
#if MI_PROFILE
#define PH_BEGIN() unsigned long long ph_t_ = clock64()
#define PH(i) do { const unsigned long long n_ = clock64(); if (LANE == 0 && !(MI_PROFILE == 3 && (i) >= 16 && (i) <= 21)) SH->prof[W][i] += n_ - ph_t_; ph_t_ = n_; } while (0)
#define PH_SIZE(slot, call) [&]() { const unsigned long long t0_ = clock64(); const long long r_ = (call); if (MI_PROFILE == 3 && LANE == 0) k.sh()->prof[WAVE_ID][16 + (slot)] += clock64() - t0_; return r_; }()
#else
#define PH_SIZE(slot, call) (call)
#define PH_BEGIN() do {} while (0)
#define PH(i) do {} while (0)
#endif

#define MI_SNAP_BYTES(n) (3 * (n) * (n) * 6 + 18 * ((n) / 4) * ((n) / 4) + 3 * ((n) / 4) * ((n) / 4) * 2 + 64)
#define MI_SNAP_BYTES_SQ(n) (2 * MI_SNAP_BYTES(n))
#define MI_SNAP_BYTES_ALL(n) (MI_SNAP_BYTES_SQ(n) + 2 * MI_SNAP_BYTES(8))

struct Blk64Wave { uint16_t pred[64 * 64]; int32_t tbuf[32 * 65]; int32_t cbuf[32 * 32]; int32_t qc[32 * 32]; };
struct Blk64None { uint8_t none_; };
struct Blk64Shared { uint16_t src64[64 * 64], bnd[2048];      uint8_t cnb_top[2][16][2], cnb_left[2][16][2]; };
template <int N> struct WaveScratch {
  static constexpr int CS = N < 32 ? N : 32, NBUF = 2, DCP_LEN = N * N, E = N == 32 ? 64 : N;
  uint16_t wa[EDGE_LEN(E)], wl[EDGE_LEN(E)], etmp[2 * E + 16];
  union {
    struct {
      uint16_t pred[N * N], dcp[N * N];
      union {
        struct {
          uint16_t rec[2][N * N];
          int32_t tbuf[N * (N + 1)], cbuf[CS * CS], qc[2][CS * CS];
        };
        GroupBuf8 grp[4];
        GroupPredBuf gpred[4];
      };
    };
    typename std::conditional<N == 32, Blk64Wave, Blk64None>::type b64;
  };
  uint8_t lev[LEV_BYTES(CS)];
};
template <int N> struct SharedScratch {
  static constexpr int E = N == 32 ? 64 : N, NC = E >= 16 ? (E / 8) * (E / 8) : 1, SNC = E >= 32 ? (E / 16) * (E / 16) : 1;
  uint16_t ra[3][EDGE_LEN(E)], rl[3][EDGE_LEN(E)];
  uint16_t srcb[3][N * N];
  uint16_t luma_rec[N * N];
  long long satd[13], dsd[7][6];
  long long wbest_j[4], cj[16][2], pbest_j[2];
  int order[13], wbest_e[4], pbest_c[2], calpha[2][2], ldelta[7];
  uint16_t part_cost[40];
  uint16_t lpred[N <= 32 ? 768 : 4];
  long long ca_sse[2][2]; int ca_idx[2][2];
  int lm_mode, lm_delta, lm_tx, lm_eob, ceob[2], sctx[3], dctx[3];
  long long lm_mode_j;
  int psv[NC], pact[NC], psv4[4], spsv[SNC], spact[SNC], cact, seg, seg_nb;
  uint16_t ssrc[N * N], spred[(E / 2) * (E / 2)];
  uint8_t nb_top[16][2], nb_left[16][2];
  int32_t split_qc[N <= 16 ? 1 : (N >= 64 ? 4096 : N * N)];
  uint16_t split_rec[N <= 16 ? 1 : N * N];
  typename std::conditional<N == 32, Blk64Shared, Blk64None>::type x64;
  TileB tile; uint8_t *snap;
  int q_item;
  int fine;
#if MI_PROFILE
  unsigned long long prof[4][32];
#endif
};

struct TxRes { int eob, cul, dcc; long long sse; uint32_t rate; };
#if MI_PROFILE
extern __shared__ __align__(16) uint8_t mi_prof_smem_[];
template <int N> __device__ __forceinline__ LDS unsigned long long &mi_prof_slot_n(int w, int i) { return ((LDS SharedScratch<N> *)mi_prof_smem_)->prof[w][i]; }
#endif

template <int TS> struct Tools {
  static constexpr bool FULL = (TS & 1) != 0, FIXED = (TS & 2) != 0;
  template <typename F> static __device__ __forceinline__ bool rdo_tx(F f) { return FIXED ? true : f->rdo_tx != 0; }
  template <typename F> static __device__ __forceinline__ bool reduced_tx_set(F f) { return FIXED ? true : f->reduced_tx_set != 0; }
  template <typename F> static __device__ __forceinline__ bool fine_directional(F f) { return FIXED ? true : f->fine_directional != 0; }
  template <typename F> static __device__ __forceinline__ bool tx_mode_select(F f) { return FIXED ? true : f->tx_mode_select != 0; }
  template <typename F> static __device__ __forceinline__ bool tune_psnr(F f) { return FIXED ? false : f->tune_psnr != 0; }
};
template <int MAXN, int NW, int TS_ = 0> struct Ctx {
  static constexpr int TS = TS_;
  static constexpr int MAXBS = MAXN == 16 ? 2 : 4;
  static constexpr size_t SH_BYTES = (sizeof(SharedScratch<MAXN>) + 15) & ~(size_t)15, WS_BYTES = (sizeof(WaveScratch<MAXN>) + 15) & ~(size_t)15;
  static constexpr size_t SC_BYTES = SCAN_LDS_ENTRIES(MAXN) * 2, CC_BYTES = (COEF_COST_MAX_ENTRIES(MAXBS) * 2 + 15) & ~(size_t)15;
  static constexpr size_t LS_OFF = SH_BYTES + NW * WS_BYTES, CC_OFF = LS_OFF + SC_BYTES, F_OFF = CC_OFF + CC_BYTES;
  LDS uint8_t *base;
  LDS WaveScratch<MAXN> *ws;
  __device__ __forceinline__ LDS SharedScratch<MAXN> *sh() const { return (LDS SharedScratch<MAXN> *)base; }
  __device__ __forceinline__ LDS WaveScratch<MAXN> *s() const { return ws; }
  __device__ __forceinline__ LDS WaveScratch<MAXN> *wave(int w) const { return (LDS WaveScratch<MAXN> *)(base + SH_BYTES + (size_t)w * WS_BYTES); }
  __device__ __forceinline__ const LDS uint16_t *ls() const { return (const LDS uint16_t *)(base + LS_OFF); }
  __device__ __forceinline__ LDS uint16_t *cc_base() const { return (LDS uint16_t *)(base + CC_OFF); }
  __device__ __forceinline__ CoefCost cc() const { return coef_cost_layout(cc_base(), MAXBS); }
  __device__ __forceinline__ const LDS FrameDev *f() const { return (const LDS FrameDev *)(base + F_OFF); }
  __device__ __forceinline__ const LDS TileB *t() const { return &sh()->tile; }
  __device__ __forceinline__ uint8_t *snap() const { return sh()->snap; }
  __device__ __forceinline__ const uint16_t *cost() const { return f()->cost; }
};

static_assert(offsetof(FrameDev, ac_recip) - offsetof(FrameDev, dc_q) == 36 && sizeof(SegTab::Q) == 48, "a SegTab entry is copied over FrameDev::dc_q .. ac_recip");
template <typename SHT> __device__ __forceinline__ void seg_select(const LDS FrameDev *f, LDS SHT *SH, int scale) {
  if (!f->seg_n) return;
  const SegTab *st = f->seg;
  const int b = seg_bucket((uint32_t)uni32(scale));
  int a = 0;
  for (int j = 0; j + 1 < f->seg_n; j++) a += b >= st->thr[j];
  const int seg = f->seg_n - 1 - a;
  if (LANE < 12) ((LDS uint32_t *)((LDS FrameDev *)f)->dc_q)[LANE] = ((const uint32_t *)&st->q[seg])[LANE];
  if (LANE == 0) SH->seg = seg;
}

#define IS_SMOOTH_(m) ((m) == SMOOTH_PRED || (m) == SMOOTH_V_PRED || (m) == SMOOTH_H_PRED)
#define J_INF 0x7fffffffffffffffLL

__device__ inline void fill_map_dev(uint8_t *m, int ms, int r, int c, int n4, int v) {
  for (int i = LANE; i < n4 * n4; i += 64) m[(r + i / n4) * ms + c + (i % n4)] = (uint8_t)v;
}
__device__ __forceinline__ int morton4_(int v) { v = (v | (v << 2)) & 0x33; return (v | (v << 1)) & 0x55; }
__device__ __forceinline__ int decoded_before(int cur_r, int cur_c, int shape, int pr, int pc) {
  const int dsr = (pr >> 4) - (cur_r >> 4), dsc = (pc >> 4) - (cur_c >> 4);
  if (dsr != 0) return dsr < 0;
  if (dsc != 0) return dsc < 0;
  if (shape != 0 && (pr >> 1) == (cur_r >> 1) && (pc >> 1) == (cur_c >> 1)) return shape == 1 ? pr < cur_r : pc < cur_c;
  return ((morton4_(pr & 15) << 1) | morton4_(pc & 15)) < ((morton4_(cur_r & 15) << 1) | morton4_(cur_c & 15));
}

template <int CTRL> __device__ __forceinline__ int satd_quad_step(int v, int odd_mask) {
  const int p = __builtin_amdgcn_update_dpp(0, v, CTRL, 0xF, 0xF, false);
  return (LANE & odd_mask) ? p - v : v + p;
}
__device__ __forceinline__ int satd8_lane(int d0, int d1, int d2, int d3) {
  const int a = d0 + d1, b = d0 - d1, c = d2 + d3, e = d2 - d3;
  const int t[4] = { a + c, b + e, a - c, b - e };
  const int m4 = (LANE & 4) ? -1 : 0, m1 = (LANE & 1) ? -1 : 0, m2 = (LANE & 2) ? -1 : 0, m8 = (LANE & 8) ? -1 : 0;
  int s = 0;
#pragma unroll
  for (int i = 0; i < 4; i++) {
    int v = t[i];
    v = __builtin_amdgcn_update_dpp(0, v, 0x141, 0xF, 0xF, false) + ((v ^ m4) - m4);
    v = __builtin_amdgcn_update_dpp(0, v, 0xB1, 0xF, 0xF, false) + ((v ^ m1) - m1);
    v = __builtin_amdgcn_update_dpp(0, v, 0x4E, 0xF, 0xF, false) + ((v ^ m2) - m2);
    v = __builtin_amdgcn_update_dpp(0, v, 0x128, 0xF, 0xF, false) + ((v ^ m8) - m8);
    s += iabs_(v);
  }
  return s;
}
__device__ __forceinline__ int satd_row_sum_(int v) {
  v += __builtin_amdgcn_update_dpp(0, v, 0x128, 0xF, 0xF, false); v += __builtin_amdgcn_update_dpp(0, v, 0x124, 0xF, 0xF, false);
  v += __builtin_amdgcn_update_dpp(0, v, 0x122, 0xF, 0xF, false); v += __builtin_amdgcn_update_dpp(0, v, 0x121, 0xF, 0xF, false);
  return v;
}
__device__ inline long long satd_dev(const LDS uint16_t *src, const LDS uint16_t *pred, int n) {
  int total = 0;
  if (n >= 8) {
    const int cells = n >> 3, units = n * (n >> 2);
    for (int u = LANE; u < units; u += 64) {
      const int cell = u >> 4, x = (cell % cells) * 8 + (u & 3) + ((u >> 1) & 4), y = (cell / cells) * 8 + (u & 4), o = y * n + x;
      const int d0 = (int)src[o] - (int)pred[o], d1 = (int)src[o + n] - (int)pred[o + n];
      const int d2 = (int)src[o + 2 * n] - (int)pred[o + 2 * n], d3 = (int)src[o + 3 * n] - (int)pred[o + 3 * n];
      const int cs = satd_row_sum_(satd8_lane(d0, d1, d2, d3));
      if ((u & 15) == 0) total += (cs + 2) >> 2;
    }
    return (long long)wave_sum_i32(total);
  }
  const int units = n * (n >> 2);
  for (int u = LANE; u < units; u += 64) {
    const int x = u % n, o = (u / n) * 4 * n + x;
    const int d0 = (int)src[o] - (int)pred[o], d1 = (int)src[o + n] - (int)pred[o + n];
    const int d2 = (int)src[o + 2 * n] - (int)pred[o + 2 * n], d3 = (int)src[o + 3 * n] - (int)pred[o + 3 * n];
    const int a = d0 + d1, b = d0 - d1, c = d2 + d3, e = d2 - d3;
    int t[4] = { a + c, b + e, a - c, b - e };
    int s = 0;
#pragma unroll
    for (int i = 0; i < 4; i++) {
      int v = satd_quad_step<0xB1>(t[i], 1);
      v = satd_quad_step<0x4E>(v, 2);
      s += iabs_(v);
    }
    total += s;
  }
  return (long long)wave_sum_i32(total);
}
__device__ inline long long sse_dev(const LDS uint16_t *a, const LDS uint16_t *b, int nn) {
  int s = 0;
  for (int i = LANE; i < nn; i += 64) { const int d = (int)a[i] - (int)b[i]; s += __mul24(d, d); }
  if (nn <= 1024) return (long long)wave_sum_i32(s);
  return wave_sum_i64((long long)s);
}

template <int n> __device__ inline long long psy_dist_wave(const LDS uint16_t *src, const LDS uint16_t *rec, const LDS int *sv, const LDS int *act, int bd) {
  constexpr int w = n == 4 ? 4 : 8, cp = n / w, ncell = cp * cp;
  constexpr int LPC = n == 4 ? 16 : 64 / ncell, PPL = n == 4 ? 1 : 64 / LPC;
  const int cell = LANE / LPC, li = LANE % LPC;
  uint32_t sd = 0, qd = 0, se = 0;
  if (cell < ncell) {
    const int cy = cell / cp, cx = cell % cp;
#pragma unroll
    for (int k = 0; k < PPL; k++) {
      const int q = li + LPC * k, o = (cy * w + q / w) * n + cx * w + q % w;
      const int d = rec[o], e = (int)src[o] - d;
      sd += (uint32_t)d; qd += (uint32_t)__mul24(d, d); se += (uint32_t)__mul24(e, e);
    }
  }
  if constexpr (LPC == 64) { sd = (uint32_t)wave_sum_i32((int)sd); qd = (uint32_t)wave_sum_i32((int)qd); se = (uint32_t)wave_sum_i32((int)se); }
  else if constexpr (LPC == 16) { sd = (uint32_t)row_sum_i32((int)sd); qd = (uint32_t)row_sum_i32((int)qd); se = (uint32_t)row_sum_i32((int)se); }
  else if constexpr (LPC == 4) {
    sd += (uint32_t)DPP_(0, sd, 0xB1, 0xF); sd += (uint32_t)DPP_(0, sd, 0x4E, 0xF);
    qd += (uint32_t)DPP_(0, qd, 0xB1, 0xF); qd += (uint32_t)DPP_(0, qd, 0x4E, 0xF);
    se += (uint32_t)DPP_(0, se, 0xB1, 0xF); se += (uint32_t)DPP_(0, se, 0x4E, 0xF);
  }
  int dist = 0;
  if (cell < ncell && li == 0) dist = psy_cell_dist(se, sd, qd, (uint32_t)sv[cell], (uint32_t)act[cell], w, bd);
  if constexpr (n >= 32) return wave_sum_i64((long long)dist);
  return (long long)wave_sum_i32(dist);
}

__device__ __forceinline__ uint32_t y_mode_rate(const uint16_t *cost, const uint16_t *ycost, int m, bool angle_coded, int delta) {
  const uint32_t r_mode = ycost[m], r_ang = cost[CDF_ANGLE + (angle_coded ? (m - V_PRED) * CDF_ANGLE_STRIDE + delta + 3 : 0)];
  return r_mode + (angle_coded ? r_ang : 0u);
}
__device__ __forceinline__ uint32_t uv_mode_rate(const uint16_t *cost, const uint16_t *uvcost, int um, bool angle_coded, int delta, bool cfl, int alpha_u, int alpha_v, int *jsign) {
  const int su = alpha_u == 0 ? 0 : (alpha_u < 0 ? 1 : 2), sv = alpha_v == 0 ? 0 : (alpha_v < 0 ? 1 : 2);
  const int js = cfl ? su * 3 + sv - 1 : 0;
  const uint32_t r_mode = uvcost[um];
  const uint32_t r_ang = cost[CDF_ANGLE + (angle_coded ? (um - V_PRED) * CDF_ANGLE_STRIDE + delta + 3 : 0)];
  const uint32_t r_sign = cost[CDF_CFL_SIGN + js];
  const uint32_t r_au = cost[CDF_CFL_ALPHA + ((cfl && su) ? ((su - 1) * 3 + sv) * CDF_CFL_ALPHA_STRIDE + iabs_(alpha_u) - 1 : 0)];
  const uint32_t r_av = cost[CDF_CFL_ALPHA + ((cfl && sv) ? ((sv - 1) * 3 + su) * CDF_CFL_ALPHA_STRIDE + iabs_(alpha_v) - 1 : 0)];
  *jsign = js;
  return r_mode + (angle_coded ? r_ang : 0u) + (cfl ? r_sign + (su ? r_au : 0u) + (sv ? r_av : 0u) : 0u);
}

template <int MAXN, int BS, int NW, int TS>
__device__ inline long long eval_tx(const Ctx<MAXN, NW, TS> k, int plane, int sctx, int dctx, const LDS uint16_t *pred, int txtype, int tx_off, int tx_sym,
                                    LDS uint16_t *rec_out, LDS int32_t *qc_out, TxRes *tr, const LDS uint16_t *src_override = nullptr,
                                    const LDS int *psv = nullptr, const LDS int *pact = nullptr) {
  constexpr int n = 4 << BS, P = n + 1, CS = n < 32 ? n : 32;
  const LDS FrameDev *f = k.f(); LDS WaveScratch<MAXN> *S = k.s();
  const LDS uint16_t *src = src_override ? src_override : k.sh()->srcb[plane];
#if MI_PROFILE
  LDS SharedScratch<MAXN> *SH = k.sh(); const int W = WAVE_ID;
#endif
  PH_BEGIN();
  for (int idx = LANE; idx < n * n; idx += 64) {
    const int i = idx / n, j = idx % n;
    S->tbuf[i * P + j] = (int)src[idx] - (int)pred[idx];
    rec_out[idx] = pred[idx];
  }
  WAVE_SYNC();
  PH(16);
  fwd_txfm2d_dev<n>(S->tbuf, S->cbuf, txtype);
  PH(17);
  const int eob = quant_rate_dev<CS>(k.cc(), k.cost(), k.ls(), S->cbuf, qc_out, S->lev, plane, BS, txtype, f->dc_q[plane], f->ac_q[plane], f->dc_recip[plane], f->ac_recip[plane],
                                     f->bd, sctx, dctx, tx_off, tx_sym, &tr->rate, &tr->cul, &tr->dcc);
  PH(19);
  if (eob > 0) inv_txfm2d_add_dev<n>(S->cbuf, S->tbuf, rec_out, txtype, f->bd);
  tr->eob = eob;
  PH(20);
  if (plane == 0 && !Tools<TS>::tune_psnr(f)) tr->sse = psy_dist_wave<n>(src, rec_out, psv ? psv : (const LDS int *)k.sh()->psv, pact ? pact : (const LDS int *)k.sh()->pact, f->bd);
  else { const long long e = sse_dev(src, rec_out, n * n); tr->sse = plane == 0 ? e : (e * k.sh()->cact + 8192) >> 14; }
  PH(21);
  return ((tr->sse * f->wq[plane]) >> 5) + (((long long)tr->rate * f->rdmult + 256) >> 9);
}

template <int BS, typename RecPtr, typename QcPtr>
__device__ inline void commit_plane(const LDS FrameDev *f, int plane, int r, int c, RecPtr rec, QcPtr qc, int eob, int cul, int dcc) {
  constexpr int n = 4 << BS, CS = n < 32 ? n : 32, n4 = 1 << BS;
  uint16_t *gr = f->rec[plane] + (size_t)(r * 4) * f->stride + c * 4;
  int32_t *gc = f->coef[plane] + (size_t)(r * 4) * f->stride + c * 4;
  for (int idx = LANE; idx < n * n; idx += 64) gr[(idx / n) * f->stride + (idx % n)] = rec[idx];
  for (int idx = LANE; idx < CS * CS; idx += 64) gc[(idx / CS) * f->stride + (idx % CS)] = qc[idx];
  fill_map_dev(f->m_lvl[plane], f->mi_stride, r, c, n4, cul);
  fill_map_dev(f->m_dc[plane], f->mi_stride, r, c, n4, dcc);
  if (LANE == 0) f->m_eob[plane][r * f->mi_stride + c] = (uint16_t)eob;
}

#include "dev_rect.h"

template <int MAXN, int BS, int NW, int TS>
__device__ MI_K1_TRY_ATTR long long try_block(const Ctx<MAXN, NW, TS> k, int r, int c, long long budget = J_INF) {
  constexpr int n = 4 << BS, n4 = 1 << BS, log2w = 2 + BS, nn = n * n, CS = n < 32 ? n : 32, qn = CS * CS;
  const LDS FrameDev *f = k.f(); const LDS TileB *t = k.t(); LDS WaveScratch<MAXN> *S = k.s(); LDS SharedScratch<MAXN> *SH = k.sh();
  const int W = NW > 1 ? WAVE_ID : 0;
  const int ms = f->mi_stride, mi = r * ms + c, x = c * 4, y = r * 4;
  const int availU = r > t->mi_row_start, availL = c > t->mi_col_start;
  const int can_ar = availU && (c + n4 < t->mi_col_end), can_bl = availL && (r + n4 < t->mi_row_end);
  const int iU = availU ? mi - ms : mi, iL = availL ? mi - 1 : mi;
  const int v_ymU = f->m_ymode[iU], v_ymL = f->m_ymode[iL];
  const int v_uvU = f->np > 1 ? f->m_uvmode[iU] : 0, v_uvL = f->np > 1 ? f->m_uvmode[iL] : 0;
  const int v_skU = f->m_skip[iU], v_skL = f->m_skip[iL], v_txU = f->m_txsize[iU], v_txL = f->m_txsize[iL];
  const int v_skUL = f->m_skip[availU && availL ? mi - ms - 1 : mi];
  const int have_ar = can_ar && decoded_before(r, c, 0, r - 1, c + n4), have_bl = can_bl && decoded_before(r, c, 0, r + n4, c - 1);
  const int amode = availU ? uni32(v_ymU) : DC_PRED, lmode = availL ? uni32(v_ymL) : DC_PRED;
  const int nb_skip = (availU ? uni32(v_skU) & 1 : 0) + (availL ? uni32(v_skL) & 1 : 0);
  const int seg_nb = (availU && availL ? (uni32(v_skUL) >> 1) + 1 : 0) | ((availU ? (uni32(v_skU) >> 1) + 1 : 0) << 4) | ((availL ? (uni32(v_skL) >> 1) + 1 : 0) << 8);
  const int nb_txU = availU ? uni32(v_txU) : -1, nb_txL = availL ? uni32(v_txL) : -1;
  const uint16_t *ycost = k.cost() + CDF_KF_Y + (intra_mode_ctx(amode) * 5 + intra_mode_ctx(lmode)) * CDF_KF_Y_STRIDE;
  const int ftype_y = IS_SMOOTH_(amode) || IS_SMOOTH_(lmode);
  const int ftype_uv = f->np > 1 && ((availU && IS_SMOOTH_(uni32(v_uvU))) || (availL && IS_SMOOTH_(uni32(v_uvL))));
  LDS uint16_t *wa = S->wa + EDGE_OFF, *wl = S->wl + EDGE_OFF;
  PH_BEGIN();

  for (int p = 0; p < f->np; p++) if ((p + 1) % NW == W) {
    int sc_, dc_;
    txb_ctx_dev(f, t, p, r, c, BS, BS, &sc_, &dc_);
    if (LANE == 0) { SH->sctx[p] = sc_; SH->dctx[p] = dc_; }
    const uint16_t *g = f->src[p] + (size_t)y * f->stride + x;
    for (int idx = LANE; idx < nn; idx += 64) SH->srcb[p][idx] = g[(idx / n) * f->stride + (idx % n)];
    load_edges(f, p, x, y, n, availL, availU, have_ar, have_bl, SH->ra[p] + EDGE_OFF, SH->rl[p] + EDGE_OFF);
  }
  if (W == 0) {
    constexpr int cp = n >= 8 ? n / 8 : 1, ncell = cp * cp;
    const int cw = f->pw >> 3;
    int a = 0;
    if (LANE < ncell) {
      const int cell = ((y >> 3) + LANE / cp) * cw + (x >> 3) + LANE % cp;
      a = (int)f->act[cell]; SH->pact[LANE] = a; SH->psv[LANE] = (int)(n == 4 ? f->svar4[mi] : f->svar8[cell]);
    }
    if (BS == 1 && LANE < 4) SH->psv4[LANE] = (int)f->svar4[(r + (LANE >> 1)) * ms + c + (LANE & 1)];
    const int tot = wave_sum_i32(a);
    const int cact = (tot + ncell / 2) / ncell;
    if (LANE == 0) { SH->cact = cact; SH->seg_nb = seg_nb; }
    seg_select(f, SH, cact);
  }
  PH(1);
  WG_SYNC();
  PH(2);
  if (DBG_IS(f, 3)) return 0;
  const int sctx_y = SH->sctx[0], dctx_y = SH->dctx[0];
  const LDS uint16_t *ra = SH->ra[0] + EDGE_OFF, *rl = SH->rl[0] + EDGE_OFF;

  constexpr bool SMALL_GROUPED = BS <= BS_8 && NW == 4 && MAXN <= 32;
  if constexpr (SMALL_GROUPED) {
    if (W < 2) {
      const int g = GROUP_ID;
      const int m = W == 0 ? (g == 0 ? V_PRED : g == 1 ? D203_PRED : g == 2 ? D45_PRED : D67_PRED) : (g < 3 ? D135_PRED + g : H_PRED);
      LDS GroupPredBuf *gp = &S->gpred[g];
      predict_dir_group<n>(f, x, y, availL, availU, mode_angle_of(m), ftype_y, ra, rl, gp);
      const int sd = satd_group<n>(SH->srcb[0], gp->pred);
      if (GROUP_LANE == 0) SH->satd[m] = (long long)sd;
    } else {
      const int g = GROUP_ID;
      const int m = W == 2 ? (g == 0 ? DC_PRED : g == 1 ? PAETH_PRED : g == 2 ? SMOOTH_PRED : -1) : (g == 0 ? SMOOTH_V_PRED : g == 1 ? SMOOTH_H_PRED : -1);
      LDS GroupPredBuf *gp = &S->gpred[g];
      predict_nondir_group<n>(m, availL, availU, f->bd, ra, rl, gp->pred);
      const int sd = satd_group<n>(SH->srcb[0], gp->pred);
      if (m >= 0 && GROUP_LANE == 0) SH->satd[m] = (long long)sd;
    }
  } else if constexpr (NW == 4) {
    const int deal = W == 0 ? 0x0F043 : W == 1 ? 0x0F165 : W == 2 ? 0x2C97 : 0x0FBA8;
#pragma unroll
    for (int i = 0; i < 4; i++) {
      const int m = (deal >> (4 * i)) & 15;
      if (m < 13) {
        predict_block(f, x, y, log2w, availL, availU, m, 0, ftype_y, ra, rl, wa, wl, S->etmp, S->pred);
        const long long sd = satd_dev(SH->srcb[0], S->pred, n);
        if (LANE == 0) SH->satd[m] = sd;
      }
    }
  } else {
    for (int m = W; m < 13; m += NW) {
      predict_block(f, x, y, log2w, availL, availU, m, 0, ftype_y, ra, rl, wa, wl, S->etmp, S->pred);
      const long long sd = satd_dev(SH->srcb[0], S->pred, n);
      if (LANE == 0) SH->satd[m] = sd;
    }
  }
  PH(3);
  WG_SYNC();
  PH(2);
  if (LANE < 13) {
    const long long mine = SH->satd[LANE];
    int rank = 0;
    for (int j = 0; j < 13; j++) { const long long o = SH->satd[j]; rank += (o < mine) || (o == mine && j < LANE); }
    SH->order[rank] = LANE;
  }
  WAVE_SYNC();
  PH(4);
  const int ncand = Tools<TS>::FULL ? 7 : 3;
  auto dl_of = [](int q) { const int a = (q >> 1) + 1; return (q & 1) ? a : -a; };
  const int refine = BS >= BS_8 && Tools<TS>::fine_directional(f);
  bool refine_grouped = false;
  if constexpr (SMALL_GROUPED) refine_grouped = refine && ncand == 3;
  if constexpr (SMALL_GROUPED) if (refine_grouped) {
    const int g = GROUP_ID;
    const int o0 = SH->order[0], o1 = SH->order[1], o2 = SH->order[2];
    const bool d0 = o0 >= V_PRED && o0 <= D67_PRED, d1 = o1 >= V_PRED && o1 <= D67_PRED, d2 = o2 >= V_PRED && o2 <= D67_PRED;
    const int nprobe = 6 * ((int)d0 + (int)d1 + (int)d2);
    for (int pass = 0; pass * 16 + W * 4 < nprobe; pass++) {
      const int pr = pass * 16 + W * 4 + g;
      const bool live = pr < nprobe;
      const int kd = live ? pr / 6 : 0, q = live ? pr - kd * 6 : 0;
      const int ci = d0 ? (kd == 0 ? 0 : (d1 ? (kd == 1 ? 1 : 2) : 2)) : (d1 ? (kd == 0 ? 1 : 2) : 2);
      const int m = SH->order[ci];
      LDS GroupPredBuf *gp = &S->gpred[g];
      predict_dir_group<n>(f, x, y, availL, availU, live ? mode_angle_of(m) + 3 * dl_of(q) : 90, ftype_y, ra, rl, gp);
      const int sd = satd_group<n>(SH->srcb[0], gp->pred);
      if (live && GROUP_LANE == 0) SH->dsd[ci][q] = (long long)sd;
    }
    PH(5);
    WG_SYNC();
    PH(2);
  }
  if (refine && !refine_grouped) {
    for (int u = W; u < ncand * 6; u += NW) {
      const int ci = u / 6, q = u - ci * 6, m = SH->order[ci];
      if (m >= V_PRED && m <= D67_PRED) {
        predict_block(f, x, y, log2w, availL, availU, m, dl_of(q), ftype_y, ra, rl, wa, wl, S->etmp, S->pred);
        const long long sd = satd_dev(SH->srcb[0], S->pred, n);
        if (LANE == 0) SH->dsd[ci][q] = sd;
      }
    }
    PH(5);
    WG_SYNC();
    PH(2);
  }
  int tx_ns = 0, tx_set = 0;
  const int tx_off0 = intra_tx_cdf_r(f, Tools<TS>::reduced_tx_set(f), BS, 0, &tx_ns, &tx_set);
  const int ntx = (Tools<TS>::rdo_tx(f) && tx_off0 >= 0) ? tx_ns : 1;
  const bool tx_trial = BS > 0 && Tools<TS>::tx_mode_select(f) && Tools<TS>::rdo_tx(f);
  LDS int32_t *split_qc = MAXN <= 16 ? (LDS int32_t *)SH->lpred : (LDS int32_t *)SH->split_qc;
  LDS uint16_t *split_rec = MAXN <= 16 ? SH->lpred + 512 : (LDS uint16_t *)SH->split_rec;
  LDS uint16_t *spred = SH->spred;
  const bool pred_cached = MAXN <= 32 && NW > 1 && ncand * nn <= 768;
  if (pred_cached) {
    for (int ci = NW - 1 - W; ci < ncand; ci += NW) {
      const int m = SH->order[ci];
      int delta = 0;
      if (m >= V_PRED && m <= D67_PRED && refine) {
        long long bsd = SH->satd[m];
        for (int q = 0; q < 6; q++) { const long long sd = SH->dsd[ci][q]; if (sd < bsd) { bsd = sd; delta = dl_of(q); } }
      }
      predict_block(f, x, y, log2w, availL, availU, m, delta, ftype_y, ra, rl, wa, wl, S->etmp, SH->lpred + ci * nn);
      if (LANE == 0) SH->ldelta[ci] = delta;
    }
    PH(12);
    WG_SYNC();
    PH(2);
  }
  long long my_j = J_INF; int my_e = 1 << 30, my_mode = DC_PRED, my_delta = 0, my_tx = DCT_DCT, cur = 0; TxRes my_tr = { 0, 0, 0, 0, 0 };
  uint32_t my_mrate = 0;
  bool grouped = false, parked = false; int my_g = 0;
  if constexpr (SMALL_GROUPED) {
    grouped = pred_cached;
    if (grouped) {
      const int g = GROUP_ID, total = ncand * ntx, rounds = (total + 15) >> 4;
      LDS uint16_t *park_rec = (LDS uint16_t *)S->dcp; LDS int32_t *park_qc = (LDS int32_t *)(S->dcp + 64);
      for (int rd = 0; rd < rounds; rd++) {
        int e;
        if (ncand == 3 && ntx == 5) e = g < 3 ? g * 5 + W + 1 : (W < 3 ? W * 5 : -1);
        else e = rd * 16 + W * 4 + g;
        const bool live = e >= 0 && e < total;
        const int ee = live ? e : 0, ci = ee / ntx, ti = ee - ci * ntx, m = SH->order[ci];
        const int delta = SH->ldelta[ci];
        const uint32_t mode_rate = y_mode_rate(k.cost(), ycost, m, m >= V_PRED && m <= D67_PRED && BS >= BS_8, delta);
        int ns2, set2;
        const int tx_off = intra_tx_cdf_r(f, Tools<TS>::reduced_tx_set(f), BS, m, &ns2, &set2);
        int txtype;
        if (ntx > 1) txtype = sym_to_txtype(tx_set, ti);
        else { txtype = mode_to_txtype(m); if (tx_off < 0 || txtype_to_sym(tx_set, txtype) < 0) txtype = DCT_DCT; }
        GroupRes gr;
        eval_group<n>(k.cc(), k.cost(), k.ls(), f, &S->grp[g], SH->srcb[0], SH->lpred + ci * nn, 0, BS, txtype, sctx_y, dctx_y, tx_off,
                      tx_off >= 0 ? txtype_to_sym(tx_set, txtype) : 0, Tools<TS>::tune_psnr(f) ? -1 : SH->psv[0], SH->pact[0], &gr);
        long long j = rd_dist32(f, 0, gr.sse) + rd_rate32(f, gr.rate) + rd_rate32(f, mode_rate);
        if (!live) j = J_INF;
        bool improved = false;
#pragma unroll
        for (int gg = 0; gg < 4; gg++) {
          const long long jg = ((long long)__builtin_amdgcn_readlane((int)(j >> 32), gg * 16) << 32) | (unsigned int)__builtin_amdgcn_readlane((int)j, gg * 16);
          const int eg = __builtin_amdgcn_readlane(e, gg * 16);
          if (jg < my_j || (jg == my_j && eg < my_e)) {
            my_j = jg; my_e = eg; my_g = gg; improved = true;
            my_mode = __builtin_amdgcn_readlane(m, gg * 16); my_delta = __builtin_amdgcn_readlane(delta, gg * 16); my_tx = __builtin_amdgcn_readlane(txtype, gg * 16);
            my_tr.eob = __builtin_amdgcn_readlane(gr.eob, gg * 16); my_tr.cul = __builtin_amdgcn_readlane(gr.cul, gg * 16); my_tr.dcc = __builtin_amdgcn_readlane(gr.dcc, gg * 16);
            my_mrate = (uint32_t)__builtin_amdgcn_readlane((int)mode_rate, gg * 16);
          }
        }
        if (rounds > 1 && improved) {
          for (int i = LANE; i < nn; i += 64) { park_rec[i] = S->grp[my_g].rec[i]; park_qc[i] = S->grp[my_g].qc[i]; }
          parked = true;
          WAVE_SYNC();
        }
      }
    }
  }
  if (!grouped)
  for (int e = W; e < ncand * ntx; e += NW) {
    const int ci = e / ntx, ti = e - ci * ntx, m = SH->order[ci];
    const int directional = m >= V_PRED && m <= D67_PRED;
    int delta = 0;
    const LDS uint16_t *lpred = S->pred;
    if (pred_cached) { delta = SH->ldelta[ci]; lpred = SH->lpred + ci * nn; }
    else {
      if (directional && refine) {
        long long bsd = SH->satd[m];
        for (int q = 0; q < 6; q++) { const long long sd = SH->dsd[ci][q]; if (sd < bsd) { bsd = sd; delta = dl_of(q); } }
      }
      predict_block(f, x, y, log2w, availL, availU, m, delta, ftype_y, ra, rl, wa, wl, S->etmp, S->pred);
    }
    const uint32_t mode_rate = y_mode_rate(k.cost(), ycost, m, directional && BS >= BS_8, delta);
    int ns2, set2;
    const int tx_off = intra_tx_cdf_r(f, Tools<TS>::reduced_tx_set(f), BS, m, &ns2, &set2);
    int txtype;
    if (ntx > 1) txtype = sym_to_txtype(tx_set, ti);
    else { txtype = mode_to_txtype(m); if (tx_off < 0 || txtype_to_sym(tx_set, txtype) < 0) txtype = DCT_DCT; }
    TxRes tr;
    long long j = eval_tx<MAXN, BS, NW>(k, 0, sctx_y, dctx_y, lpred, txtype, tx_off, tx_off >= 0 ? txtype_to_sym(tx_set, txtype) : 0, S->rec[cur], S->qc[cur], &tr);
    j += ((long long)mode_rate * f->rdmult + 256) >> 9;
    if (j < my_j) {
      my_j = j; my_e = e; my_mode = m; my_delta = delta; my_tx = txtype; my_tr = tr; my_mrate = mode_rate;
      cur ^= 1;
    }
  }
  if (LANE == 0) { SH->wbest_j[W] = my_j; SH->wbest_e[W] = my_e; }
  PH(6);
  WG_SYNC();
  PH(2);
  int win = 0;
  for (int w2 = 1; w2 < NW; w2++) if (SH->wbest_j[w2] < SH->wbest_j[win] || (SH->wbest_j[w2] == SH->wbest_j[win] && SH->wbest_e[w2] < SH->wbest_e[win])) win = w2;
  const long long best_j = SH->wbest_j[win];
  if (W == win) {
    const int b = cur ^ 1;
    const LDS uint16_t *best_rec = S->rec[b]; const LDS int32_t *best_qc = S->qc[b];
    if constexpr (SMALL_GROUPED) if (grouped) {
      if (parked) { best_rec = (const LDS uint16_t *)S->dcp; best_qc = (const LDS int32_t *)(S->dcp + 64); }
      else { best_rec = S->grp[my_g].rec; best_qc = S->grp[my_g].qc; }
    }
    commit_plane<BS>(f, 0, r, c, best_rec, best_qc, my_tr.eob, my_tr.cul, my_tr.dcc);
    fill_map_dev(f->m_ymode, ms, r, c, n4, my_mode);
    fill_map_dev((uint8_t *)f->m_angle_y, ms, r, c, n4, (uint8_t)(int8_t)my_delta);
    fill_map_dev(f->m_txtype, ms, r, c, n4, my_tr.eob ? my_tx : DCT_DCT);
    fill_map_dev(f->m_bsize, ms, r, c, n4, BS);
    fill_map_dev(f->m_txsize, ms, r, c, n4, BS);
    if (f->np > 1) for (int i = LANE; i < nn; i += 64) SH->luma_rec[i] = best_rec[i];
    if (LANE == 0) {
      SH->lm_mode = my_mode; SH->lm_delta = my_delta; SH->lm_tx = my_tx; SH->lm_eob = my_tr.eob;
      SH->lm_mode_j = ((long long)my_mrate * f->rdmult + 256) >> 9;
    }
  }
  PH(7);
  WG_SYNC();
  PH(2);
  if (DBG_IS(f, 5)) return 0;
  const int best_mode = SH->lm_mode, best_delta = SH->lm_delta;
  long long luma_j = best_j; int any_coef = SH->lm_eob > 0;
  if constexpr (BS > 0) if (Tools<TS>::tx_mode_select(f)) {
    const int maxw = 4 << BS;
    const int actx = nb_txU >= 0 && (1 << dim_wl(nb_txU)) >= maxw, lctx = nb_txL >= 0 && (1 << dim_hl(nb_txL)) >= maxw;
    const uint16_t *dcost = k.cost() + CDF_TX_SIZE + ((BS - 1) * 3 + actx + lctx) * CDF_TX_SIZE_STRIDE;
    luma_j += ((long long)dcost[0] * f->rdmult + 256) >> 9;
    if (tx_trial) {
      LDS int *const sub_tx = (LDS int *)SH->dsd, *const sub_eob = sub_tx + 16, *const sub_cul = sub_tx + 32, *const sub_dcc = sub_tx + 48, *const psv16 = sub_tx + 64;
      LDS int *const sfl_r = (LDS int *)SH->satd, *const sfl_b = sfl_r + 4;
      LDS uint16_t *ssrc = (LDS uint16_t *)SH->ssrc;
      auto trial = [&](auto depth_c) -> bool {
        constexpr int D = decltype(depth_c)::value;
        constexpr int SBS = BS - D, G = 1 << D, hn = n >> D, half = n4 >> D, hnn = hn * hn, SCS = hn < 32 ? hn : 32, sqn = SCS * SCS;
        long long j_split = SH->lm_mode_j + (((long long)dcost[D] * f->rdmult + 256) >> 9);
        int stx_ns = 0, stx_set = 0;
        const int stx_off = intra_tx_cdf_r(f, Tools<TS>::reduced_tx_set(f), SBS, best_mode, &stx_ns, &stx_set);
        const int sntx = stx_off >= 0 ? stx_ns : 1;
        int sub_any = 0;
#if MI_PROFILE
        const unsigned long long tr_t0_ = clock64();
        auto tr_done_ = [&]() { if (LANE == 0) SH->prof[W][BS == 1 ? 31 : (D == 1 ? 29 : 30)] += clock64() - tr_t0_; };
#else
        auto tr_done_ = []() {};
#endif
        PH(13);
        for (int q = W; q < G * G; q += NW) {
          const int so = (q / G) * hn * n + (q % G) * hn;
          for (int idx = LANE; idx < hnn; idx += 64) ssrc[q * hnn + idx] = SH->srcb[0][so + (idx / hn) * n + (idx % hn)];
        }
        if (W == 0) {
          if (LANE < n4) {
            const int k2 = LANE;
            const bool ha = availU && c + k2 < f->mi_cols, hl = availL && r + k2 < f->mi_rows;
            const int ia = ha ? (r - 1) * ms + c + k2 : mi, il = hl ? (r + k2) * ms + c - 1 : mi;
            const int la = f->m_lvl[0][ia], da = f->m_dc[0][ia], ll = f->m_lvl[0][il], dl2 = f->m_dc[0][il];
            SH->nb_top[k2][0] = (uint8_t)(ha ? la : 0); SH->nb_top[k2][1] = (uint8_t)(ha ? da : 0);
            SH->nb_left[k2][0] = (uint8_t)(hl ? ll : 0); SH->nb_left[k2][1] = (uint8_t)(hl ? dl2 : 0);
          }
          if (hn == 4 && n == 16 && LANE < 16) psv16[LANE] = (int)f->svar4[(r + (LANE >> 2)) * ms + c + (LANE & 3)];
          if (LANE >= 1 && LANE < G) {
            const bool ca = c + n4 < t->mi_col_end, cb = r + n4 < t->mi_row_end;
            sfl_r[LANE] = ca && decoded_before(r, c, 0, r + LANE * half - 1, c + n4); sfl_b[LANE] = cb && decoded_before(r, c, 0, r + n4, c + LANE * half - 1);
          }
        }
        WG_SYNC();
        PH(22);
        [[maybe_unused]] const int x_ = x, y_ = y, r_ = r, c_ = c, availU_ = availU, availL_ = availL, have_ar_ = have_ar, have_bl_ = have_bl, best_mode_ = best_mode, best_delta_ = best_delta, ftype_y_ = ftype_y;
        if constexpr (SBS <= BS_8 && NW == 4 && MAXN <= 32) {
          constexpr int CH_BYTES = nn * 2 + G * G * sqn * 4 + G * G * 4;
          static_assert(4 * CH_BYTES <= (int)sizeof(WaveScratch<MAXN>) && hnn <= 64 && 4 * 64 <= MAXN * MAXN, "four chains fit a wavefront's scratch; edges and predictions of four rows fit pred / dcp");
          const int g = GROUP_ID, gl = GROUP_LANE;
          const bool paired = MAXN == 16 && sntx == 5 && n >= 8 && hn <= 8;
          const int mem = paired ? (g & 1) : 0;
          const int e = paired ? (W == 0 ? 1 + (g >> 1) : (W == 1 ? 3 + (g >> 1) : ((W == 2 && g < 2) ? 0 : 64)))
                               : (sntx == 5 ? (W == 0 ? g + 1 : ((W == 1 && g == 0) ? 0 : 64)) : W * 4 + g);
          const bool has_chain = e < sntx, wave_has = paired ? W < 3 : (sntx == 5 ? W < 2 : W * 4 < sntx);
          LDS long long *const cres_j = (LDS long long *)SH->cj;
          LDS int *const cres_any = (LDS int *)(cres_j + 8);
          LDS uint32_t *const meta_idtx = (LDS uint32_t *)SH->cj + 32;
          const long long thr = uni64(luma_j < budget ? luma_j : budget);
          auto chain_state = [&](int ce, int cw, int cg, LDS uint16_t **cv, LDS int32_t **cq, LDS uint32_t **cm) {
            if (paired && ce == 0) { *cv = split_rec; *cq = split_qc; *cm = meta_idtx; return; }
            LDS uint8_t *cst = paired ? (LDS uint8_t *)k.wave(3) + (ce >= 1 && ce <= 4 ? ce - 1 : 0) * CH_BYTES : (LDS uint8_t *)k.wave(2 + cw) + cg * CH_BYTES;
            *cv = (LDS uint16_t *)cst; *cq = (LDS int32_t *)(cst + nn * 2); *cm = (LDS uint32_t *)(cst + nn * 2 + G * G * sqn * 4);
          };
          if (wave_has) {
            const int x = uni32(x_), y = uni32(y_), r = uni32(r_), c = uni32(c_), availU = uni32(availU_), availL = uni32(availL_), have_ar = uni32(have_ar_), have_bl = uni32(have_bl_);
            const int best_mode = uni32(best_mode_), best_delta = uni32(best_delta_), ftype_y = uni32(ftype_y_);
            LDS uint16_t *canvas; LDS int32_t *cqc; LDS uint32_t *cmeta;
            chain_state(e, W, g, &canvas, &cqc, &cmeta);
            LDS uint16_t *A = S->pred + g * 64 + EDGE_OFF, *Lf = A + 32, *ppred = S->dcp + g * 64;
            int txtype;
            if (sntx > 1) txtype = sym_to_txtype(stx_set, has_chain ? e : 0);
            else { txtype = mode_to_txtype(best_mode); if (stx_off < 0 || txtype_to_sym(stx_set, txtype) < 0) txtype = DCT_DCT; }
            const int tx_sym = stx_off >= 0 ? txtype_to_sym(stx_set, txtype) : 0;
            const bool dirm = best_mode >= V_PRED && best_mode <= D67_PRED;
            const int pa = dirm ? mode_angle_of(best_mode) + 3 * best_delta : 0;
            const int max_x = f->mi_cols * 4 - 1, max_y = f->mi_rows * 4 - 1, rs = f->stride, bd = f->bd;
            const uint16_t *grec = f->rec[0];
            long long jc = has_chain ? j_split : J_INF;
            int any = 0;
            const bool uses_ar = dirm && pa < 90;
            const int nslot = paired ? (G == 4 ? 10 : (uses_ar ? 4 : 3)) : G * G;
#pragma unroll 1
            for (int slot = 0; slot < nslot; slot++) {
              if (MI_BALLOT64(jc < thr) == 0ull) break;
              int q0 = slot, q1 = -1;
              if (paired) {
                if (G == 4) { const int lo = imax_(0, (slot - 2) >> 1), hi = imin_(3, slot >> 1); q0 = lo * 4 + slot - 2 * lo; q1 = lo + 1 <= hi ? (lo + 1) * 4 + slot - 2 * (lo + 1) : -1; }
                else if (!uses_ar) { q0 = slot == 0 ? 0 : (slot == 1 ? 1 : 3); q1 = slot == 1 ? 2 : -1; }
              }
              const int q = (mem == 1 && q1 >= 0) ? q1 : q0;
              const int bi = q / G, bj = q % G;
              const int sx = x + bj * hn, sy = y + bi * hn;
              const int sU = availU || bi, sL = availL || bj;
              {
                const int s_ar = bi == 0 ? (bj < G - 1 ? availU : have_ar) : (bj < G - 1 ? 1 : sfl_r[bi]);
                const int s_bl = bj == 0 ? (bi < G - 1 ? availL : have_bl) : (bi < G - 1 ? 0 : sfl_b[bj]);
                const int lim_a = imin_(max_x, sx + (s_ar ? 2 * hn : hn) - 1), lim_l = imin_(max_y, sy + (s_bl ? 2 * hn : hn) - 1);
                auto px = [&](int ax, int ay) -> int {
                  const int xr = ax - x, yr = ay - y;
                  const bool in_blk = xr >= 0 && xr < n && yr >= 0 && yr < n, on_a = yr == -1 && xr >= -1 && xr < 2 * n, on_l = xr == -1 && yr >= 0 && yr < 2 * n;
                  const LDS uint16_t *p = in_blk ? (const LDS uint16_t *)canvas + (yr * n + xr) : (on_a ? ra + xr : rl + (on_l ? yr : 0));
                  int v = (int)*p;
                  if (!(in_blk || on_a || on_l)) v = (int)grec[(size_t)ay * rs + ax];
                  return v;
                };
#pragma unroll
                for (int it = 0; it < (2 * hn + 16) / 16; it++) {
                  const int i = gl + 16 * it;
                  const bool act = i <= 2 * hn, corner = i == 2 * hn;
                  const int ii = act ? i : 0;
                  int a, l;
                  if (sU) a = px(corner ? (sL ? sx - 1 : sx) : imin_(lim_a, sx + ii), sy - 1); else a = px(sL ? sx - 1 : sx, sy);
                  if (sL) l = px(sx - 1, imin_(lim_l, sy + ii)); else l = px(sx, sU ? sy - 1 : sy);
                  if (!sU && !sL) { a = corner ? (1 << (bd - 1)) : (1 << (bd - 1)) - 1; l = (1 << (bd - 1)) + 1; }
                  if (act && corner) { A[-1] = (uint16_t)a; Lf[-1] = (uint16_t)a; }
                  if (act && !corner) { A[ii] = (uint16_t)a; Lf[ii] = (uint16_t)l; }
                }
              }
              WAVE_SYNC();
              if (dirm) predict_dir_group<hn>(f, sx, sy, sL, sU, pa, ftype_y, A, Lf, &S->gpred[g], ppred);
              else predict_nondir_group<hn>(best_mode, sL, sU, bd, A, Lf, ppred);
              PH(23);
              int ssc, sdc;
              {
                int top = 0, left = 0, dcs = 0;
                const uint32_t mt = bi ? cmeta[q - G] : 0u, ml = bj ? cmeta[q - 1] : 0u;
#pragma unroll
                for (int k2 = 0; k2 < half; k2++) {
                  int l, d;
                  if (bi == 0) { l = SH->nb_top[bj * half + k2][0]; d = SH->nb_top[bj * half + k2][1]; } else { l = (int)((mt >> 16) & 0xFF); d = (int)(mt >> 24); if (n >= 32 && c + bj * half + k2 >= f->mi_cols) l = d = 0; }
                  top = imax_(top, l); dcs += d == 1 ? -1 : (d == 2 ? 1 : 0);
                  if (bj == 0) { l = SH->nb_left[bi * half + k2][0]; d = SH->nb_left[bi * half + k2][1]; } else { l = (int)((ml >> 16) & 0xFF); d = (int)(ml >> 24); if (n >= 32 && r + bi * half + k2 >= f->mi_rows) l = d = 0; }
                  left = imax_(left, l); dcs += d == 1 ? -1 : (d == 2 ? 1 : 0);
                }
                sdc = dcs < 0 ? 1 : (dcs > 0 ? 2 : 0);
                if (top == 0 && left == 0) ssc = 1;
                else if (top == 0 || left == 0) ssc = 2 + (imax_(top, left) > 3);
                else if (imax_(top, left) <= 3) ssc = 4;
                else if (imin_(top, left) <= 3) ssc = 5;
                else ssc = 6;
              }
              constexpr int pcp = n >= 8 ? n / 8 : 1;
              const int psv_q = hn == 4 ? (n == 8 ? SH->psv4[q] : psv16[q]) : SH->psv[bi * pcp + bj];
              const int pact_q = hn == 4 ? SH->pact[(bi >> 1) * pcp + (bj >> 1)] : SH->pact[bi * pcp + bj];
              GroupRes gr;
              eval_group<hn>(k.cc(), k.cost(), k.ls(), f, &S->grp[g], ssrc + q * hnn, ppred, 0, SBS, txtype, ssc, sdc, stx_off, tx_sym, Tools<TS>::tune_psnr(f) ? -1 : psv_q, pact_q, &gr);
              {
                const long long j = rd_dist32(f, 0, gr.sse) + rd_rate32(f, gr.rate);
                long long jslot = j;
                if (paired) {
                  const long long jo = ((long long)__shfl((int)(j >> 32), LANE ^ 16) << 32) | (unsigned int)__shfl((int)j, LANE ^ 16);
                  jslot = q1 >= 0 ? j + jo : (mem == 0 ? j : jo);
                }
                if (has_chain) jc += jslot;
              }
              if (has_chain) {
                const LDS uint16_t *srec = S->grp[g].rec; const LDS int32_t *sqc = S->grp[g].qc;
                const int ro = bi * hn * n + bj * hn;
#pragma unroll
                for (int i = gl; i < hnn; i += 16) canvas[ro + (i / hn) * n + (i % hn)] = srec[i];
#pragma unroll
                for (int i = gl; i < sqn; i += 16) cqc[q * sqn + i] = sqc[i];
                cmeta[q] = (uint32_t)gr.eob | ((uint32_t)gr.cul << 16) | ((uint32_t)gr.dcc << 24);
              }
              any |= gr.eob > 0;
              WAVE_SYNC();
              PH(25);
            }
            if (paired) any |= __shfl(any, LANE ^ 16);
            const int rslot = paired ? (has_chain ? e : 5 + (g & 1)) : (sntx == 5 ? (W == 0 ? g + 1 : (g == 0 ? 0 : 4 + g)) : W * 4 + g);
            cres_j[rslot] = (has_chain && jc < thr) ? jc : J_INF; cres_any[rslot] = any;
          }
          __builtin_amdgcn_s_setprio(0);
          WG_SYNC();
          PH(26);
          int be = -1; long long bjc = J_INF;
          for (int e2 = 0; e2 < sntx; e2++) { const long long v = cres_j[e2]; if (v < bjc) { bjc = v; be = e2; } }
          j_split = bjc;
          if (be >= 0) {
            const int ow = paired ? 0 : (sntx == 5 ? (be == 0 ? 1 : 0) : be >> 2), og = sntx == 5 ? (be == 0 ? 0 : be - 1) : be & 3;
            if (W == ow) {
              LDS uint16_t *canvas; LDS int32_t *cqc; LDS uint32_t *cmeta;
              chain_state(be, ow, og, &canvas, &cqc, &cmeta);
              if (canvas != split_rec) {
                for (int i = LANE; i < nn; i += 64) split_rec[i] = canvas[i];
                for (int i = LANE; i < G * G * sqn; i += 64) split_qc[i] = cqc[i];
              }
              int btx;
              if (sntx > 1) btx = sym_to_txtype(stx_set, be);
              else { btx = mode_to_txtype(best_mode); if (stx_off < 0 || txtype_to_sym(stx_set, btx) < 0) btx = DCT_DCT; }
// ... 419 lines not shown
    const uint16_t *uvcost = cfl_allowed ? k.cost() + CDF_UV_CFL + best_mode * CDF_UV_CFL_STRIDE : k.cost() + CDF_UV_NOCFL + best_mode * CDF_UV_NOCFL_STRIDE;
    unsigned long long cand_pack = 0; int nc = 0;
    auto push = [&](int m) { cand_pack |= (unsigned long long)m << (4 * nc); nc++; };
    push(DC_PRED);
    if (best_mode != DC_PRED) push(best_mode);
    if (Tools<TS>::FULL) for (int m = 1; m < 13; m++) if (m != best_mode) push(m);
    if (cfl_allowed) push(UV_CFL_PRED);
    const int uvset = tx_set_of(BS, Tools<TS>::reduced_tx_set(f));
    constexpr int NPAIR = 2;
    const int pair = ((W >> 1) & 1) ^ 1, active = W < 4;
    long long pb_j = J_INF; int pb_c = 1 << 30, pb_delta = 0, pb_sign = 0, pb_au = 0, pb_av = 0, ccur = 0; TxRes pb_tr = { 0, 0, 0, 0, 0 };
    int mine[16], nmine = 0, nother = 0;
    for (int i = 0; i < nc; i++) {
      const int pr = (lut4(cand_pack, i) == UV_CFL_PRED) ? 1 : (i == 0 || (i & 1)) ? 0 : 1;
      if (pr == pair) mine[nmine++] = i; else nother++;
    }
    const int rounds = imax_(nmine, nother);
    for (int rd = 0; rd < rounds; rd++) {
      const int valid = active && rd < nmine;
      int ci2 = 0;
      for (int q = 0; q < 16; q++) if (q == rd && valid) ci2 = mine[q];
      const int um = valid ? lut4(cand_pack, ci2) : DC_PRED;
      const int delta = (um == best_mode && um >= V_PRED && um <= D67_PRED && BS >= BS_8) ? best_delta : 0;
      int txtype = mode_to_txtype(um);
      if (txtype_to_sym(uvset, txtype) < 0) txtype = DCT_DCT;
      {
        const int p = (W & 1) + 1;
        const int cfl_main = valid && um == UV_CFL_PRED;
        const int cfl_help = cfl_allowed && active && pair == 0 && rd == nother - 1;
        if (cfl_main || cfl_help) {
          const int half = cfl_help ? 1 : 0;
          const LDS uint16_t *luma = SH->luma_rec;
          int lsum = 0;
          for (int idx = LANE; idx < nn; idx += 64) lsum += luma[idx] << 3;
          lsum = wave_sum_i32(lsum);
          const int avg = round2_(lsum, 2 * log2w), mx = (1 << f->bd) - 1;
          predict_block(f, x, y, log2w, availL, availU, DC_PRED, 0, ftype_uv, SH->ra[p] + EDGE_OFF, SH->rl[p] + EDGE_OFF, wa, wl, S->etmp, S->dcp);
          long long best_sse = J_INF; int best_idx = 1 << 20;
          if (half == 0) {
            int e0 = 0;
            for (int idx = LANE; idx < nn; idx += 64) { const int d = (int)SH->srcb[p][idx] - (int)S->dcp[idx]; e0 += __mul24(d, d); }
            best_sse = wave_sum_i64((long long)e0); best_idx = -1;
          }
          int e[16];
#pragma unroll
          for (int a = 0; a < 16; a++) e[a] = 0;
          for (int idx = LANE; idx < nn; idx += 64) {
            const int l = ((int)luma[idx] << 3) - avg, dcv = S->dcp[idx], sv = SH->srcb[p][idx];
            const int la = iabs_(l), neg = l < 0;
#pragma unroll
            for (int kq = 0; kq < 8; kq++) {
              const int mag = half * 8 + kq + 1;
              const int r = round2_(__mul24(mag, la), 6), sc = neg ? -r : r;
              const int dp = sv - iclamp_(dcv + sc, 0, mx), dm = sv - iclamp_(dcv - sc, 0, mx);
              e[2 * kq] += __mul24(dp, dp); e[2 * kq + 1] += __mul24(dm, dm);
            }
          }
#pragma unroll
          for (int a = 0; a < 16; a++) {
            const long long ea = (long long)wave_sum_i32(e[a]);
            if (ea < best_sse) { best_sse = ea; best_idx = half * 16 + a; }
          }
          if (LANE == 0) { SH->ca_sse[p - 1][half] = best_sse; SH->ca_idx[p - 1][half] = best_idx; }
        }
      }
      PH(8);
      WG_SYNC();
      PH(2);
      int alpha_u = 0, alpha_v = 0, jsign = 0, ok = valid;
      if (valid && um == UV_CFL_PRED) {
#pragma unroll
        for (int pp = 0; pp < 2; pp++) {
          const int idx = SH->ca_sse[pp][1] < SH->ca_sse[pp][0] ? SH->ca_idx[pp][1] : SH->ca_idx[pp][0];
          const int al = idx < 0 ? 0 : ((idx & 1) ? -((idx >> 1) + 1) : ((idx >> 1) + 1));
          if (pp == 0) alpha_u = al; else alpha_v = al;
        }
        if (alpha_u == 0 && alpha_v == 0) ok = 0;
      }
      const uint32_t mode_rate = uv_mode_rate(k.cost(), uvcost, um, um >= V_PRED && um <= D67_PRED && BS >= BS_8, delta,
                                              valid && um == UV_CFL_PRED && ok, alpha_u, alpha_v, &jsign);
      TxRes trp = { 0, 0, 0, 0, 0 };
      if (ok) {
        {
          const int p = (W & 1) + 1;
          const LDS uint16_t *pra = SH->ra[p] + EDGE_OFF, *prl = SH->rl[p] + EDGE_OFF;
          if (um == UV_CFL_PRED) {
            const int al = p == 1 ? alpha_u : alpha_v;
            predict_block(f, x, y, log2w, availL, availU, DC_PRED, 0, ftype_uv, pra, prl, wa, wl, S->etmp, S->dcp);
            if (al) {
              int lsum = 0;
              for (int idx = LANE; idx < nn; idx += 64) lsum += SH->luma_rec[idx] << 3;
              lsum = wave_sum_i32(lsum);
              const int avg = round2_(lsum, 2 * log2w), mx = (1 << f->bd) - 1;
              for (int idx = LANE; idx < nn; idx += 64) {
                const int l = ((int)SH->luma_rec[idx] << 3) - avg, v = al * l, sc = v >= 0 ? round2_(v, 6) : -round2_(-v, 6);
                S->pred[idx] = (uint16_t)iclamp_((int)S->dcp[idx] + sc, 0, mx);
              }
            } else { for (int i = LANE; i < nn; i += 64) S->pred[i] = S->dcp[i]; }
            WAVE_SYNC();
          } else {
            predict_block(f, x, y, log2w, availL, availU, um, delta, ftype_uv, pra, prl, wa, wl, S->etmp, S->pred);
          }
          const long long jp = eval_tx<MAXN, BS, NW>(k, p, SH->sctx[p], SH->dctx[p], S->pred, txtype, -1, 0, S->rec[ccur], S->qc[ccur], &trp);
          if (LANE == 0) SH->cj[ci2][p - 1] = jp;
        }
      }
      PH(9);
      WG_SYNC();
      PH(2);
      if (valid && ok) {
        const long long j = SH->cj[ci2][0] + SH->cj[ci2][1] + rd_rate32(f, mode_rate);
        if (j < pb_j) {
          pb_j = j; pb_c = ci2; pb_delta = delta; pb_sign = jsign; pb_au = alpha_u; pb_av = alpha_v; pb_tr = trp;
          ccur ^= 1;
        }
      }
    }
    if (LANE == 0 && (W & 1) == 0 && W < 4) { SH->pbest_j[pair] = pb_j; SH->pbest_c[pair] = pb_c; }
    WG_SYNC();
    PH(2);
    int wp = 0;
    if ((SH->pbest_j[1] < SH->pbest_j[0] || (SH->pbest_j[1] == SH->pbest_j[0] && SH->pbest_c[1] < SH->pbest_c[0]))) wp = 1;
    const long long best_uv = SH->pbest_j[wp];
    if (active && pair == wp) {
      const int p = (W & 1) + 1, b = ccur ^ 1;
      commit_plane<BS>(f, p, r, c, (const LDS uint16_t *)S->rec[b], (const LDS int32_t *)S->qc[b], pb_tr.eob, pb_tr.cul, pb_tr.dcc);
      if (LANE == 0) SH->ceob[p - 1] = pb_tr.eob;
      if (p == 1) {
        const int buv = lut4(cand_pack, pb_c);
        fill_map_dev(f->m_uvmode, ms, r, c, n4, buv);
        fill_map_dev((uint8_t *)f->m_angle_uv, ms, r, c, n4, (uint8_t)(int8_t)pb_delta);
        fill_map_dev(f->m_cfl_sign, ms, r, c, n4, pb_sign);
        fill_map_dev(f->m_cfl_au, ms, r, c, n4, pb_au ? iabs_(pb_au) - 1 : 0);
        fill_map_dev(f->m_cfl_av, ms, r, c, n4, pb_av ? iabs_(pb_av) - 1 : 0);
      }
    }
    PH(10);
    WG_SYNC();
    PH(2);
    any_coef |= (SH->ceob[0] > 0) | (SH->ceob[1] > 0);
    total_j += best_uv;
    (void)qn;
  }
  if (DBG_IS(f, 6)) return 0;
  const int skip = !any_coef;
  int seg_ctx = 0;
  const int seg_nb2 = SH->seg_nb, seg_ul = (seg_nb2 & 15) - 1, seg_u = ((seg_nb2 >> 4) & 15) - 1, seg_l = (seg_nb2 >> 8) - 1;
  const int seg_p = seg_pred(seg_ul, seg_u, seg_l, &seg_ctx), seg_own = f->seg_n ? SH->seg : 0, seg_fin = f->seg_n ? (skip ? seg_p : seg_own) : 0;
  if (W == 0) {
    fill_map_dev(f->m_skip, ms, r, c, n4, skip | (seg_fin << 1));
    if (skip) for (int p = 0; p < f->np; p++) { fill_map_dev(f->m_lvl[p], ms, r, c, n4, 0); fill_map_dev(f->m_dc[p], ms, r, c, n4, 0); }
  }
  const int sctx = nb_skip;
  total_j += ((long long)k.cost()[CDF_SKIP + sctx * CDF_SKIP_STRIDE + skip] * f->rdmult + 256) >> 9;
  if (f->seg_n && !skip) total_j += ((long long)k.cost()[CDF_SEG_ID + seg_ctx * CDF_SEG_ID_STRIDE + seg_symbol(seg_own, seg_p, f->seg_n)] * f->rdmult + 256) >> 9;
  PH(11);
  WG_SYNC();
  PH(2);
  return total_j;
}

#include "dev_blk64.h"
template <int MAXN, int BS, int NW, int TS> __device__ __forceinline__ long long blk_eval(const Ctx<MAXN, NW, TS> k, int r, int c, long long budget = J_INF) {
  if constexpr (MAXN == 32 && BS == 4) return PH_SIZE(3, try_block64<NW>(k, r, c, budget)); else return PH_SIZE(BS < 3 ? BS : 3, (try_block<MAXN, BS, NW>(k, r, c, budget)));
}

template <int BYTES> __device__ __forceinline__ void copy_row_(void *dst, const void *src) {
  if constexpr (BYTES == 1) *(uint8_t *)dst = *(const uint8_t *)src;
  else if constexpr (BYTES == 2) *(uint16_t *)dst = *(const uint16_t *)src;
  else if constexpr (BYTES == 4) *(uint32_t *)dst = *(const uint32_t *)src;
  else if constexpr (BYTES == 8) *(uint2 *)dst = *(const uint2 *)src;
  else { for (int i = 0; i < BYTES / 16; i++) ((uint4 *)dst)[i] = ((const uint4 *)src)[i]; }
}
static_assert(offsetof(FrameDev, m_eob) - offsetof(FrameDev, m_bsize) == 18 * sizeof(void *), "area_copy_dev indexes m_bsize .. m_dc[2] as one array of 18 map pointers");
template <int BS, int NW> __device__ inline void area_copy_dev(const LDS FrameDev *f, uint8_t *snap, int r, int c, int save) {
  constexpr int n = 4 << BS, n4 = 1 << BS, Q = n / 4;
#if MI_PROFILE
  const unsigned long long ac_t0_ = clock64();
#define mi_prof_slot(w, i) mi_prof_slot_n<MI_PROF_MAXN>(w, i)
#endif
  uint8_t *smaps = snap + 3 * n * n * 6;
  uint8_t *seob = smaps + 18 * n4 * n4;
  const int W = NW > 1 ? WAVE_ID : 0, np = f->np, rs = f->stride, ms = f->mi_stride;
  for (int p = W; p < np; p += NW) {
    uint16_t *gr = f->rec[p] + (size_t)(r * 4) * rs + c * 4;
    int32_t *gc = f->coef[p] + (size_t)(r * 4) * rs + c * 4;
    uint2 *srec = (uint2 *)(snap + (size_t)p * n * n * 2);
    uint4 *scoef = (uint4 *)(snap + 3 * n * n * 2 + (size_t)p * n * n * 4);
    for (int u = LANE; u < n * Q; u += 64) {
      const int o = (u / Q) * rs + 4 * (u % Q);
      if (save) { srec[u] = *(const uint2 *)(gr + o); scoef[u] = *(const uint4 *)(gc + o); }
      else { *(uint2 *)(gr + o) = srec[u]; *(uint4 *)(gc + o) = scoef[u]; }
    }
  }
  if (W == NW - 1) {
    const LDS unsigned long long *mp = (const LDS unsigned long long *)&f->m_bsize;
    for (int u = LANE; u < 17 * n4; u += 64) {
      const int m = u / n4, row = u - m * n4, mi = m + (m >= 8);
      if (np == 1 && (mi == 13 || mi == 14 || mi == 16 || mi == 17)) continue;
      uint8_t *g = (uint8_t *)mp[mi] + (r + row) * ms + c, *sp = smaps + m * n4 * n4 + row * n4;
      if (save) copy_row_<n4>(sp, g); else copy_row_<n4>(g, sp);
    }
    const LDS unsigned long long *ep = (const LDS unsigned long long *)&f->m_eob[0];
    for (int u = LANE; u < np * n4; u += 64) {
      const int p = u / n4, row = u - p * n4;
      uint8_t *g = (uint8_t *)((uint16_t *)ep[p] + (r + row) * ms + c), *sp = seob + (p * n4 * n4 + row * n4) * 2;
      if (save) copy_row_<2 * n4>(sp, g); else copy_row_<2 * n4>(g, sp);
    }
  }
  WG_SYNC();
#if MI_PROFILE
  if (LANE == 0) mi_prof_slot(WAVE_ID, 14) += clock64() - ac_t0_;
#endif
}

__device__ __forceinline__ int part_cost_idx(int bs, int ctx, int part) { return bs == 1 ? ctx * 4 + part : 16 + (bs - 2) * 8 + ctx * 2 + (part == 3); }
template <typename SHT> __device__ inline void load_part_cost(LDS SHT *SH, const uint16_t *cost, int tid) {
  if (tid < 40) {
    const int bs = tid < 16 ? 1 : 2 + (tid - 16) / 8, e = tid < 16 ? tid : (tid - 16) % 8, ctx = tid < 16 ? e >> 2 : e >> 1, part = tid < 16 ? (e & 3) : ((e & 1) ? 3 : 0);
    SH->part_cost[tid] = cost[CDF_PARTITION + ((bs - 1) * 4 + ctx) * CDF_PARTITION_STRIDE + part];
  }
}
__device__ __forceinline__ int part_ctx_of(int bs, int availU, int availL, int code_above, int code_left) {
  return ((availL && dim_hl(code_left) < 2 + bs) ? 2 : 0) + ((availU && dim_wl(code_above) < 2 + bs) ? 1 : 0);
}
struct PartNb { int a0, a1, l0, l1, availU, availL; };
template <int BS> __device__ __forceinline__ PartNb part_neighbours(const LDS FrameDev *f, const LDS TileB *t, int r, int c, bool halves) {
  constexpr int half = (1 << BS) >> 1;
  const int ms = f->mi_stride, mi = r * ms + c;
  PartNb n; n.availU = r > t->mi_row_start; n.availL = c > t->mi_col_start;
  const int v0 = f->m_bsize[n.availU ? mi - ms : mi], v1 = f->m_bsize[(n.availU && halves) ? mi - ms + half : mi];
  const int v2 = f->m_bsize[n.availL ? mi - 1 : mi], v3 = f->m_bsize[(n.availL && halves) ? mi + half * ms - 1 : mi];
  n.a0 = uni32(v0); n.a1 = uni32(v1); n.l0 = uni32(v2); n.l1 = uni32(v3);
  return n;
}
template <typename SHT> __device__ __forceinline__ long long part_j(const LDS SHT *SH, const LDS FrameDev *f, int bs, int ctx, int part) {
  return ((long long)SH->part_cost[part_cost_idx(bs, ctx, part)] * f->rdmult + 256) >> 9;
}

#if defined(__gfx942__) || defined(__gfx950__)
#define MI_K1_ACQUIRE() do { if (WAVE_ID == 0) __builtin_amdgcn_fence(__ATOMIC_ACQUIRE, "agent"); WG_SYNC(); } while (0)
#else
#define MI_K1_ACQUIRE() do { __builtin_amdgcn_fence(__ATOMIC_ACQUIRE, "agent"); WG_SYNC(); } while (0)
#endif
#ifndef MI_K1_POLL_LOG2
#define MI_K1_POLL_LOG2 25
#endif
#define MI_K1_POLL_MAX (1u << MI_K1_POLL_LOG2)
__device__ __forceinline__ int root_z(int bi, int bj) { return ((bi & 1) << 1) | (bj & 1) | ((bi & 2) << 2) | ((bj & 2) << 1); }
template <int MAXBS, int MAXN, int NW, int TS> __device__ inline void root_wait(const Ctx<MAXN, NW, TS> k, int r, int c) {
  constexpr int G = 1 << (4 - MAXBS);
  const LDS FrameDev *f = k.f(); const LDS TileB *t = k.t();
  if (((r >> MAXBS) & (G - 1)) != 0 && ((c >> MAXBS) & (G - 1)) != 0) return;
  if (threadIdx.x == 0) {
    const int *mask = f->sb_prog + f->sb_rows * f->tile_cols;
    const int gr = r >> MAXBS, gc = c >> MAXBS, zc = root_z(gr & (G - 1), gc & (G - 1)), sr = r >> 4, sc = c >> 4;
    auto need = [&](int dr, int dc, bool only_if_earlier) {
      const int rr = (gr + dr) << MAXBS, cc = (gc + dc) << MAXBS;
      if (rr < t->mi_row_start || rr >= t->mi_row_end || cc < t->mi_col_start || cc >= t->mi_col_end) return;
      const int sr2 = rr >> 4, sc2 = cc >> 4, z2 = root_z((gr + dr) & (G - 1), (gc + dc) & (G - 1));
      if (sr2 == sr && sc2 == sc) return;
      if (only_if_earlier && !(sr2 < sr || (sr2 == sr && (sc2 < sc || (sc2 == sc && z2 < zc))))) return;
      const int *w = mask + sr2 * f->sb_cols + sc2;
      unsigned spin = 0;
      while (!((__hip_atomic_load(w, __ATOMIC_RELAXED, __HIP_MEMORY_SCOPE_AGENT) >> z2) & 1) && spin < MI_K1_POLL_MAX) {
        __builtin_amdgcn_s_sleep(16); spin++;
        if ((spin & 4095u) == 0u && __hip_atomic_load(search_error_word(f), __ATOMIC_RELAXED, __HIP_MEMORY_SCOPE_AGENT) != 0) spin = MI_K1_POLL_MAX;
      }
      if (spin >= MI_K1_POLL_MAX) __hip_atomic_store(search_error_word(f), 1, __ATOMIC_RELAXED, __HIP_MEMORY_SCOPE_AGENT);
    };
    need(0, -1, false); need(-1, 0, false); need(-1, -1, false); need(-1, 1, true); need(1, -1, true);
  }
  WG_SYNC();
  MI_K1_ACQUIRE();
}
template <int MAXBS, int MAXN, int NW, int TS> __device__ inline void root_publish(const Ctx<MAXN, NW, TS> k, int r, int c) {
  constexpr int G = 1 << (4 - MAXBS);
  const LDS FrameDev *f = k.f();
  if (((r >> MAXBS) & (G - 1)) != G - 1 && ((c >> MAXBS) & (G - 1)) != G - 1) return;
  WG_SYNC();
  if (threadIdx.x == 0) {
    int *w = f->sb_prog + f->sb_rows * f->tile_cols + (r >> 4) * f->sb_cols + (c >> 4);
    __hip_atomic_fetch_or(w, 1 << root_z((r >> MAXBS) & (G - 1), (c >> MAXBS) & (G - 1)), __ATOMIC_RELEASE, __HIP_MEMORY_SCOPE_AGENT);
  }
}

template <int MAXN, int MAXBS, int BS, int NW> struct RdPart {
  template <int TS> static __device__ __forceinline__ int run(const Ctx<MAXN, NW, TS> k, int r, int c, long long known_j) {
    const LDS FrameDev *f = k.f();
    if (r >= f->mi_rows || c >= f->mi_cols) return 0;
    constexpr int half = (1 << BS) >> 1, px = 4 << BS, n4 = 1 << BS;
    const int has_rows = (r + half) < f->mi_rows, has_cols = (c + half) < f->mi_cols;
    const int must_split = px > f->part_max || !has_rows || !has_cols;
    const int can_split = px > f->part_min || must_split;
    if (!can_split || (DBG_IS(f, 9) && BS == 1)) {
      if constexpr (BS <= MAXBS) { if (known_j < 0) blk_eval<MAXN, BS, NW>(k, r, c); }
      return 0;
    }
    int do_split = must_split;
    long long sub_j[4] = { -1, -1, -1, -1 };
    if constexpr (BS <= MAXBS) {
      if (!must_split) {
        const PartNb nb = part_neighbours<BS>(f, k.t(), r, c, BS - 1 >= BS_8);
        const int pctx = part_ctx_of(BS, nb.availU, nb.availL, nb.a0, nb.l0);
        const long long j_blk = known_j >= 0 ? known_j : uni64(blk_eval<MAXN, BS, NW>(k, r, c));
        const long long j_none = uni64(j_blk + part_j(k.sh(), f, BS, pctx, 0));
        area_copy_dev<BS, NW>(f, k.snap(), r, c, 1);
        long long j_split = uni64(part_j(k.sh(), f, BS, pctx, 3));
#pragma unroll
        for (int q = 0; q < 4; q++) {
          if (!(j_split < j_none) || DBG_IS(f, 7)) break;
          const int rr = r + (q >> 1) * half, cc = c + (q & 1) * half;
          if (rr >= f->mi_rows || cc >= f->mi_cols) continue;
          sub_j[q] = uni64(blk_eval<MAXN, BS - 1, NW>(k, rr, cc, j_none - j_split));
          j_split += sub_j[q];
          if (BS - 1 >= BS_8) {
            const int cctx = part_ctx_of(BS - 1, (q >> 1) ? 1 : nb.availU, (q & 1) ? 1 : nb.availL, (q >> 1) ? BS - 1 : ((q & 1) ? nb.a1 : nb.a0), (q & 1) ? BS - 1 : ((q >> 1) ? nb.l1 : nb.l0));
            j_split += uni64(part_j(k.sh(), f, BS - 1, cctx, 0));
          }
        }
        if constexpr (BS == 1) {
          uint8_t *best_snap = k.snap() + MI_SNAP_BYTES_SQ(4 << MAXBS), *split_snap = best_snap + MI_SNAP_BYTES(8);
          long long j_best = j_none; int have_split = 0, rect_won = 0;
          if (j_split < j_none) { j_best = j_split; area_copy_dev<BS, NW>(f, split_snap, r, c, 1); have_split = 1; }
          {
            long long j = uni64(part_j(k.sh(), f, BS, pctx, 1));
            for (int k2 = 0; k2 < 2 && j < j_best; k2++) j += uni64(PH_SIZE(4, (try_block_rect<MAXN, BS_8X4, NW>(k, r + k2, c, j_best - j))));
            if (j < j_best) { j_best = j; rect_won = 1; area_copy_dev<BS, NW>(f, best_snap, r, c, 1); }
          }
          {
            long long j = uni64(part_j(k.sh(), f, BS, pctx, 2));
            for (int k2 = 0; k2 < 2 && j < j_best; k2++) j += uni64(PH_SIZE(5, (try_block_rect<MAXN, BS_4X8, NW>(k, r, c + k2, j_best - j))));
            if (j < j_best) { j_best = j; rect_won = 2; area_copy_dev<BS, NW>(f, best_snap, r, c, 1); }
          }
          if (rect_won) { area_copy_dev<BS, NW>(f, best_snap, r, c, 0); return 1; }
          if (have_split) area_copy_dev<BS, NW>(f, split_snap, r, c, 0);
        }
        if (j_split < j_none && !DBG_IS(f, 7) && !DBG_IS(f, 8) && !(DBG_IS(f, 10) && BS == 1)) do_split = 1;
        else { area_copy_dev<BS, NW>(f, k.snap(), r, c, 0); }
      }
    }
    if (do_split) {
      int chain = !must_split && !DBG_IS(f, 11);
#pragma unroll 1
      for (int q = 0; q < 4; q++)
      {
        const int rr = r + (q >> 1) * half, cc = c + (q & 1) * half;
        const bool sync_root = BS - 1 == MAXBS && MAXBS < 4 && k.sh()->fine && rr < f->mi_rows && cc < f->mi_cols;
        if constexpr (BS - 1 == MAXBS && MAXBS < 4) if (sync_root) root_wait<MAXBS>(k, rr, cc);
        if (RdPart<MAXN, MAXBS, BS - 1, NW>::run(k, rr, cc, chain ? sub_j[q] : -1)) chain = 0;
        if constexpr (BS - 1 == MAXBS && MAXBS < 4) if (sync_root) root_publish<MAXBS>(k, rr, cc);
      }
      return 1;
    }
    return 0;
  }
};
template <int MAXN, int MAXBS, int NW> struct RdPart<MAXN, MAXBS, 0, NW> {
  template <int TS> static __device__ __forceinline__ int run(const Ctx<MAXN, NW, TS> k, int r, int c, long long known_j) {
    const LDS FrameDev *f = k.f();
    if (r >= f->mi_rows || c >= f->mi_cols) return 0;
    if (known_j >= 0) return 0;
    blk_eval<MAXN, 0, NW>(k, r, c);
    return 0;
  }
};

template <int MAXN> __device__ __forceinline__ constexpr size_t snap_level_off(int bs, int maxbs) {
  size_t o = 0;
  for (int b = maxbs; b > bs; b--) o += MI_SNAP_BYTES(4 << b);
  return o;
}
template <int MAXN, int MAXBS, int BS, int NW> struct RdPartBU {
  template <int TS> static __device__ __forceinline__ long long run(const Ctx<MAXN, NW, TS> k, int r, int c) {
    const LDS FrameDev *f = k.f();
    if (r >= f->mi_rows || c >= f->mi_cols) return 0;
    constexpr int half = (1 << BS) >> 1, px = 4 << BS, n4 = 1 << BS;
    const int has_rows = (r + half) < f->mi_rows, has_cols = (c + half) < f->mi_cols;
    const int must_split = px > f->part_max || !has_rows || !has_cols;
    const int can_split = px > f->part_min || must_split;
    long long j_none = J_INF;
    int pctx = 0;
    if (!must_split) { const PartNb nb = part_neighbours<BS>(f, k.t(), r, c, false); pctx = part_ctx_of(BS, nb.availU, nb.availL, nb.a0, nb.l0); }
    if constexpr (BS <= MAXBS) {
      if (!must_split) {
        j_none = uni64(blk_eval<MAXN, BS, NW>(k, r, c));
        j_none += uni64(part_j(k.sh(), f, BS, pctx, 0));
        if (!can_split) return j_none;
        area_copy_dev<BS, NW>(f, k.snap() + snap_level_off<MAXN>(BS, MAXBS), r, c, 1);
      }
    }
    long long j_split = must_split ? 0 : uni64(part_j(k.sh(), f, BS, pctx, 3));
#pragma unroll 1
    for (int q = 0; q < 4; q++) {
      if (!must_split && j_split >= j_none) break;
      const int rr = r + (q >> 1) * half, cc = c + (q & 1) * half;
      const bool sync_root = BS - 1 == MAXBS && MAXBS < 4 && k.sh()->fine && rr < f->mi_rows && cc < f->mi_cols;
      if constexpr (BS - 1 == MAXBS && MAXBS < 4) if (sync_root) root_wait<MAXBS>(k, rr, cc);
      j_split += RdPartBU<MAXN, MAXBS, BS - 1, NW>::run(k, rr, cc);
      if constexpr (BS - 1 == MAXBS && MAXBS < 4) if (sync_root) root_publish<MAXBS>(k, rr, cc);
    }
    if constexpr (BS == 1) if (!must_split) {
      uint8_t *best_snap = k.snap() + MI_SNAP_BYTES_SQ(4 << MAXBS), *split_snap = best_snap + MI_SNAP_BYTES(8);
      long long j_best = j_none; int have_split = 0, rect_won = 0;
      if (j_split < j_none) { j_best = j_split; area_copy_dev<BS, NW>(f, split_snap, r, c, 1); have_split = 1; }
      {
        long long j = uni64(part_j(k.sh(), f, BS, pctx, 1));
        for (int k2 = 0; k2 < 2 && j < j_best; k2++) j += uni64(PH_SIZE(4, (try_block_rect<MAXN, BS_8X4, NW>(k, r + k2, c, j_best - j))));
        if (j < j_best) { j_best = j; rect_won = 1; area_copy_dev<BS, NW>(f, best_snap, r, c, 1); }
      }
      {
        long long j = uni64(part_j(k.sh(), f, BS, pctx, 2));
        for (int k2 = 0; k2 < 2 && j < j_best; k2++) j += uni64(PH_SIZE(5, (try_block_rect<MAXN, BS_4X8, NW>(k, r, c + k2, j_best - j))));
        if (j < j_best) { j_best = j; rect_won = 2; area_copy_dev<BS, NW>(f, best_snap, r, c, 1); }
      }
      if (rect_won) { area_copy_dev<BS, NW>(f, best_snap, r, c, 0); return j_best; }
      if (have_split) { area_copy_dev<BS, NW>(f, split_snap, r, c, 0); return j_split; }
    }
    if (must_split || j_split < j_none) return j_split;
    if constexpr (BS <= MAXBS) { area_copy_dev<BS, NW>(f, k.snap() + snap_level_off<MAXN>(BS, MAXBS), r, c, 0); }
    return j_none;
  }
};
template <int MAXN, int MAXBS, int NW> struct RdPartBU<MAXN, MAXBS, 0, NW> {
  template <int TS> static __device__ __forceinline__ long long run(const Ctx<MAXN, NW, TS> k, int r, int c) {
    const LDS FrameDev *f = k.f();
    if (r >= f->mi_rows || c >= f->mi_cols) return 0;
    return uni64(blk_eval<MAXN, 0, NW>(k, r, c));
  }
};

constexpr int k1_maxn(int maxbs) { return maxbs <= 2 ? 16 : 32; }
#define MI_K1_POOL_BYTES(maxbs) ((maxbs) <= 2 ? (size_t)MI_SNAP_BYTES_ALL(16) : (size_t)MI_SNAP_BYTES_ALL(64) + MI_BLK64_HBM_BYTES)
template <int MAXBS, int NW> constexpr size_t k1_lds_bytes() {
  constexpr int MAXN = k1_maxn(MAXBS);
  return ((sizeof(SharedScratch<MAXN>) + 15) & ~(size_t)15) + NW * ((sizeof(WaveScratch<MAXN>) + 15) & ~(size_t)15) + SCAN_LDS_ENTRIES(MAXN) * 2 +
         ((COEF_COST_MAX_ENTRIES(MAXBS) * 2 + 15) & ~(size_t)15) + (size_t)FRAMEDEV_K1_BYTES;
}

static_assert(MI_PROFILE || k1_lds_bytes<2, 4>() <= 40960, "K1 <2,4> must fit four workgroups per CU (160 KB LDS)");
static_assert(MI_PROFILE || k1_lds_bytes<4, 4>() <= 163840, "K1 <4,4> must fit the CU's 160 KB of LDS");
static_assert(sizeof(Blk64Wave) <= offsetof(WaveScratch<32>, lev) - offsetof(WaveScratch<32>, pred), "the 64x64 candidate's working set lies over the wave's block scratch, not over its level maps");

struct SbItem { uint32_t job; uint16_t sbr, sbc; };
template <int MAXBS, int NW, bool BU, int TS>
__global__ __launch_bounds__(64 * NW, (NW == 4 && MAXBS == 2 ? MI_K1_WG_PER_CU : 1)) void tile_search_kernel(const FrameDev *__restrict__ frames, const TileJob *__restrict__ jobs,
                                                                                                          const SbItem *__restrict__ items, int nitems, int *next_item, uint8_t *snap_pool, int items_per_wg) {
  constexpr int MAXN = k1_maxn(MAXBS);
  extern __shared__ __align__(16) uint8_t smem[];
  using K = Ctx<MAXN, NW, TS>;
  K k;
  k.base = (LDS uint8_t *)smem;
  k.ws = (LDS WaveScratch<MAXN> *)(smem + K::SH_BYTES + (size_t)(NW > 1 ? WAVE_ID : 0) * K::WS_BYTES);
  LDS uint16_t *lsc = (LDS uint16_t *)(smem + K::LS_OFF);
  LDS FrameDev *lf = (LDS FrameDev *)(smem + K::F_OFF);
  if (WAVE_ID == 0) load_scans_to_lds(lsc, MAXN);
  for (int i = LANE; i < (int)sizeof(k.s()->lev); i += 64) k.s()->lev[i] = 0;
  if (threadIdx.x == 0) k.sh()->snap = snap_pool + (size_t)blockIdx.x * MI_K1_POOL_BYTES(MAXBS);
#if MI_PROFILE
  if (threadIdx.x < 128) ((LDS unsigned long long *)k.sh()->prof)[threadIdx.x] = 0;
  const FrameDev *prof_f = nullptr;
#endif
  int cur_frame = -1, cur_job = -1;
#if MI_PROFILE
  const unsigned long long k_t0_ = clock64(); unsigned long long w_acc_ = 0;
#endif
  for (int done_items = 0; items_per_wg <= 0 || done_items < items_per_wg; done_items++) {
#if MI_PROFILE
    const unsigned long long w_t0_ = clock64();
#endif
    WG_SYNC();
    if (threadIdx.x == 0) k.sh()->q_item = atomicAdd(next_item, 1);
    WG_SYNC();
    const int it = k.sh()->q_item;
    if (it >= nitems) break;
    const SbItem item = items[it];
    const int job = (int)(item.job & 0x7fffffffu), sbr = item.sbr, sbc = item.sbc;
    const bool fine = (item.job >> 31) != 0;
    const TileJob tj = jobs[job];
    const FrameDev *gf = frames + tj.frame;
    if (frame_idle(gf)) continue;
    if (tj.frame != cur_frame) {
      for (int i = threadIdx.x; i < FRAMEDEV_K1_BYTES / 4; i += 64 * NW) ((LDS uint32_t *)lf)[i] = ((const uint32_t *)gf)[i];
      load_coef_cost(k.cc_base(), gf->cost, MAXBS, threadIdx.x, 64 * NW);
      load_part_cost(k.sh(), gf->cost, (int)threadIdx.x);
      cur_frame = tj.frame;
    }
    if (job != cur_job) {
      if (threadIdx.x == 0) {
        LDS TileB *t = &k.sh()->tile;
        t->mi_row_start = gf->tile_row_start[tj.tile_row] * 16; t->mi_row_end = imin_(gf->tile_row_start[tj.tile_row + 1] * 16, gf->mi_rows);
        t->mi_col_start = gf->tile_col_start[tj.tile_col] * 16; t->mi_col_end = imin_(gf->tile_col_start[tj.tile_col + 1] * 16, gf->mi_cols);
      }
    }
    const bool new_tile = job != cur_job;
    cur_job = job;
    if (threadIdx.x == 0) k.sh()->fine = fine;
    WG_SYNC();
    if (new_tile && gf->tile_cost != nullptr) {
      const uint16_t *tc = gf->tile_cost + (size_t)(tj.tile_row * gf->tile_cols + tj.tile_col) * CDF_TOTAL;
      if (threadIdx.x == 0) lf->cost = tc;
      load_coef_cost(k.cc_base(), tc, MAXBS, threadIdx.x, 64 * NW);
      load_part_cost(k.sh(), tc, (int)threadIdx.x);
      WG_SYNC();
    }
    const int row0 = k.t()->mi_row_start, row1 = k.t()->mi_row_end, col0 = k.t()->mi_col_start, col1 = k.t()->mi_col_end;
    const int ncols = (col1 - col0 + 15) >> 4, nrows = (row1 - row0 + 15) >> 4, r = row0 + 16 * sbr, c = col0 + 16 * sbc;
    int *const prog = gf->sb_prog + (r >> 4) * gf->tile_cols + tj.tile_col;
    if (!fine && (sbc > 0 || sbr > 0)) {
      if (threadIdx.x == 0) {
        unsigned spin = 0;
        auto gave_up = [&]() { return (spin & 4095u) == 0u && __hip_atomic_load(search_error_word(gf), __ATOMIC_RELAXED, __HIP_MEMORY_SCOPE_AGENT) != 0; };
        if (sbc > 0) while (__hip_atomic_load(prog, __ATOMIC_RELAXED, __HIP_MEMORY_SCOPE_AGENT) < sbc && spin < MI_K1_POLL_MAX) { __builtin_amdgcn_s_sleep(16); spin++; if (gave_up()) spin = MI_K1_POLL_MAX; }
        if (sbr > 0) { const int need = imin_(sbc + 2, ncols); while (__hip_atomic_load(prog - gf->tile_cols, __ATOMIC_RELAXED, __HIP_MEMORY_SCOPE_AGENT) < need && spin < MI_K1_POLL_MAX) { __builtin_amdgcn_s_sleep(16); spin++; if (gave_up()) spin = MI_K1_POLL_MAX; } }
        if (spin >= MI_K1_POLL_MAX) __hip_atomic_store(search_error_word(gf), 1, __ATOMIC_RELAXED, __HIP_MEMORY_SCOPE_AGENT);
      }
      WG_SYNC();
      MI_K1_ACQUIRE();
    }
    unsigned long long *tc = gf->tile_clk + (size_t)(tj.tile_row * gf->tile_cols + tj.tile_col) * 4;
    if (threadIdx.x == 0 && sbr == 0 && sbc == 0) tc[0] = wall_clock64();
#if MI_PROFILE
    w_acc_ += clock64() - w_t0_;
#endif
    if constexpr (BU) RdPartBU<MAXN, MAXBS, 4, NW>::run(k, r, c); else RdPart<MAXN, MAXBS, 4, NW>::run(k, r, c, -1);
    WG_SYNC();
    if (threadIdx.x == 0) {
      if (!fine) __hip_atomic_store(prog, sbc + 1, __ATOMIC_RELEASE, __HIP_MEMORY_SCOPE_AGENT);
      if (sbr == nrows - 1 && sbc == ncols - 1) tc[1] = wall_clock64();
    }
#if MI_PROFILE
    prof_f = gf;
#endif
  }
  if (threadIdx.x == 0 && atomicAdd(next_item + 1, 1) == (int)gridDim.x - 1) { next_item[1] = 0; next_item[0] = 0; }
#if MI_PROFILE
  if (LANE == 0) { k.sh()->prof[WAVE_ID][0] = w_acc_; k.sh()->prof[WAVE_ID][15] = clock64() - k_t0_; }
  WG_SYNC();
  if (prof_f && prof_f->prof_out && threadIdx.x < 128) prof_f->prof_out[(size_t)blockIdx.x * 128 + threadIdx.x] = ((LDS unsigned long long *)k.sh()->prof)[threadIdx.x];
#endif
}
```

Measured before the change: 559.4.

## Batch head global loads into registers, cache skip costs, skip redundant rect snapshot copies

```diff
diff --git a/cavif_rs_amd/csrc/dev_predict.h b/cavif_rs_amd/csrc/dev_predict.h
--- a/cavif_rs_amd/csrc/dev_predict.h
+++ b/cavif_rs_amd/csrc/dev_predict.h
@@ -56,23 +56,32 @@
   *dx = has ? (int)(e & 1023) : 0; *dy = has ? (int)((e >> 10) & 1023) : 0;
 }
 
+struct EdgeAddr { int ia, il; };
+__device__ __forceinline__ EdgeAddr edge_addr(int rs, int mi_rows, int mi_cols, int x, int y, int w, int h, int have_left, int have_above, int have_ar, int have_bl, int i) {
+  const int max_x = mi_cols * 4 - 1, max_y = mi_rows * 4 - 1;
+  const int lim_a = imin_(max_x, x + (have_ar ? 2 * w : w) - 1), lim_l = imin_(max_y, y + (have_bl ? 2 * h : h) - 1);
+  const bool corner = i == w + h;
+  EdgeAddr e;
+  if (have_above) e.ia = (y - 1) * rs + (corner ? (have_left ? x - 1 : x) : imin_(lim_a, x + i));
+  else e.ia = y * rs + (have_left ? x - 1 : x);
+  if (have_left) e.il = imin_(lim_l, y + i) * rs + x - 1;
+  else e.il = (have_above ? y - 1 : y) * rs + x;
+  if (i > w + h) e.ia = e.il = y * rs + x;
+  return e;
+}
+__device__ __forceinline__ void edge_value(int bd, int have_left, int have_above, bool corner, uint16_t *a, uint16_t *l) {
+  if (!have_above && !have_left) { *a = (uint16_t)(corner ? (1 << (bd - 1)) : (1 << (bd - 1)) - 1); *l = (uint16_t)((1 << (bd - 1)) + 1); }
+}
 __device__ inline void load_edges(const LDS FrameDev *f, int plane, int x, int y, int n, int have_left, int have_above,
                                   int have_ar, int have_bl, LDS uint16_t *above , LDS uint16_t *left) {
-  const int bd = f->bd, rs = f->stride;
+  const int bd = f->bd, rs = f->stride, mi_rows = f->mi_rows, mi_cols = f->mi_cols;
   const uint16_t *rec = f->rec[plane];
-  const int max_x = f->mi_cols * 4 - 1, max_y = f->mi_rows * 4 - 1;
   const int tot = 2 * n;
-  const int na = x + (have_ar ? 2 * n : n) - 1, nl = y + (have_bl ? 2 * n : n) - 1;
-  const int lim_a = imin_(max_x, na), lim_l = imin_(max_y, nl);
   for (int i = LANE; i <= tot; i += 64) {
     const bool corner = i == tot;
-    int ia, il;
-    if (have_above) ia = (y - 1) * rs + (corner ? (have_left ? x - 1 : x) : imin_(lim_a, x + i));
-    else ia = y * rs + (have_left ? x - 1 : x);
-    if (have_left) il = imin_(lim_l, y + i) * rs + x - 1;
-    else il = (have_above ? y - 1 : y) * rs + x;
-    uint16_t a = rec[ia], l = rec[il];
-    if (!have_above && !have_left) { a = (uint16_t)(corner ? (1 << (bd - 1)) : (1 << (bd - 1)) - 1); l = (uint16_t)((1 << (bd - 1)) + 1); }
+    const EdgeAddr e = edge_addr(rs, mi_rows, mi_cols, x, y, n, n, have_left, have_above, have_ar, have_bl, i);
+    uint16_t a = rec[e.ia], l = rec[e.il];
+    edge_value(bd, have_left, have_above, corner, &a, &l);
     if (corner) { above[-1] = a; left[-1] = a; }
     else { above[i] = a; left[i] = l; }
   }
diff --git a/cavif_rs_amd/csrc/dev_rate.h b/cavif_rs_amd/csrc/dev_rate.h
--- a/cavif_rs_amd/csrc/dev_rate.h
+++ b/cavif_rs_amd/csrc/dev_rate.h
@@ -1,44 +1,23 @@
 #pragma once
 #include "dev_common.h"
 
-template <typename FP, typename TP> __device__ inline void txb_ctx_dev(FP f, TP t, int plane, int r4, int c4, int txs, int bs, int *skip_ctx, int *dc_ctx) {
-  const int w4 = 1 << txs, ms = f->mi_stride;
+struct TxbCtxAddr { int ia, il; bool ha, hl; };
+struct TxbCtxVal { int la, da, ll, dl; };
+__device__ __forceinline__ TxbCtxAddr txb_ctx_addr(int ms, int mi_rows, int mi_cols, int row_start, int col_start, int r4, int c4, int w4, int h4, int k) {
+  TxbCtxAddr a;
+  a.ha = k < w4 && r4 - 1 >= row_start && c4 + k < mi_cols; a.hl = k < h4 && c4 - 1 >= col_start && r4 + k < mi_rows;
+  a.ia = a.ha ? (r4 - 1) * ms + c4 + k : r4 * ms + c4; a.il = a.hl ? (r4 + k) * ms + c4 - 1 : r4 * ms + c4;
+  return a;
+}
+template <typename FP> __device__ __forceinline__ TxbCtxVal txb_ctx_load(FP f, int plane, const TxbCtxAddr a) {
+  TxbCtxVal v;
+  v.la = f->m_lvl[plane][a.ia]; v.da = f->m_dc[plane][a.ia]; v.ll = f->m_lvl[plane][a.il]; v.dl = f->m_dc[plane][a.il];
+  return v;
+}
+__device__ __forceinline__ void txb_ctx_reduce(int plane, int whole, const TxbCtxAddr a, const TxbCtxVal v, int *skip_ctx, int *dc_ctx) {
   int top = 0, left = 0, dcs = 0, any_a = 0, any_l = 0;
-  const int k = LANE;
-  if (k < w4) {
-    const bool ha = r4 - 1 >= t->mi_row_start && c4 + k < f->mi_cols, hl = c4 - 1 >= t->mi_col_start && r4 + k < f->mi_rows;
-    const int ia = ha ? (r4 - 1) * ms + c4 + k : r4 * ms + c4, il = hl ? (r4 + k) * ms + c4 - 1 : r4 * ms + c4;
-    const int la = f->m_lvl[plane][ia], da = f->m_dc[plane][ia], ll = f->m_lvl[plane][il], dl = f->m_dc[plane][il];
-    if (ha) { top = la; any_a = la | da; dcs += da == 1 ? -1 : (da == 2 ? 1 : 0); }
-    if (hl) { left = ll; any_l = ll | dl; dcs += dl == 1 ? -1 : (dl == 2 ? 1 : 0); }
-  }
-  top = wave_max_i32(top); left = wave_max_i32(left); dcs = wave_sum_i32(dcs);
-  any_a = wave_or_i32(any_a); any_l = wave_or_i32(any_l);
-  *dc_ctx = dcs < 0 ? 1 : (dcs > 0 ? 2 : 0);
-  if (plane == 0) {
-    int ctx;
-    if (bs == txs) ctx = 0;
-    else if (top == 0 && left == 0) ctx = 1;
-    else if (top == 0 || left == 0) ctx = 2 + (imax_(top, left) > 3);
-    else if (imax_(top, left) <= 3) ctx = 4;
-    else if (imin_(top, left) <= 3) ctx = 5;
-    else ctx = 6;
-    *skip_ctx = ctx;
-  } else {
-    *skip_ctx = 7 + (any_a != 0) + (any_l != 0) + (bs > txs ? 3 : 0);
-  }
-}
-template <typename FP, typename TP> __device__ inline void txb_ctx_wh(FP f, TP t, int plane, int r4, int c4, int w4, int h4, int whole, int *skip_ctx, int *dc_ctx) {
-  const int ms = f->mi_stride;
-  int top = 0, left = 0, dcs = 0, any_a = 0, any_l = 0;
-  const int k = LANE;
-  if (k < imax_(w4, h4)) {
-    const bool ha = k < w4 && r4 - 1 >= t->mi_row_start && c4 + k < f->mi_cols, hl = k < h4 && c4 - 1 >= t->mi_col_start && r4 + k < f->mi_rows;
-    const int ia = ha ? (r4 - 1) * ms + c4 + k : r4 * ms + c4, il = hl ? (r4 + k) * ms + c4 - 1 : r4 * ms + c4;
-    const int la = f->m_lvl[plane][ia], da = f->m_dc[plane][ia], ll = f->m_lvl[plane][il], dl = f->m_dc[plane][il];
-    if (ha) { top = la; any_a = la | da; dcs += da == 1 ? -1 : (da == 2 ? 1 : 0); }
-    if (hl) { left = ll; any_l = ll | dl; dcs += dl == 1 ? -1 : (dl == 2 ? 1 : 0); }
-  }
+  if (a.ha) { top = v.la; any_a = v.la | v.da; dcs += v.da == 1 ? -1 : (v.da == 2 ? 1 : 0); }
+  if (a.hl) { left = v.ll; any_l = v.ll | v.dl; dcs += v.dl == 1 ? -1 : (v.dl == 2 ? 1 : 0); }
   top = wave_max_i32(top); left = wave_max_i32(left); dcs = wave_sum_i32(dcs);
   any_a = wave_or_i32(any_a); any_l = wave_or_i32(any_l);
   *dc_ctx = dcs < 0 ? 1 : (dcs > 0 ? 2 : 0);
@@ -53,6 +32,13 @@
     *skip_ctx = ctx;
   } else *skip_ctx = 7 + (any_a != 0) + (any_l != 0) + (whole ? 0 : 3);
 }
+template <typename FP, typename TP> __device__ inline void txb_ctx_wh(FP f, TP t, int plane, int r4, int c4, int w4, int h4, int whole, int *skip_ctx, int *dc_ctx) {
+  const TxbCtxAddr a = txb_ctx_addr(f->mi_stride, f->mi_rows, f->mi_cols, t->mi_row_start, t->mi_col_start, r4, c4, w4, h4, LANE);
+  txb_ctx_reduce(plane, whole, a, txb_ctx_load(f, plane, a), skip_ctx, dc_ctx);
+}
+template <typename FP, typename TP> __device__ inline void txb_ctx_dev(FP f, TP t, int plane, int r4, int c4, int txs, int bs, int *skip_ctx, int *dc_ctx) {
+  txb_ctx_wh(f, t, plane, r4, c4, 1 << txs, 1 << txs, bs == txs, skip_ctx, dc_ctx);
+}
 
 __device__ __forceinline__ int eob_to_pt(int eob) { return eob < 3 ? eob : (32 - __clz(eob - 1) + 1); }
 __device__ __forceinline__ int eob_pt_cdf(int eob_multi, int pt, int cls) {
diff --git a/cavif_rs_amd/csrc/dev_rect.h b/cavif_rs_amd/csrc/dev_rect.h
--- a/cavif_rs_amd/csrc/dev_rect.h
+++ b/cavif_rs_amd/csrc/dev_rect.h
@@ -2,19 +2,13 @@
 
 __device__ inline void load_edges_wh(const LDS FrameDev *f, int plane, int x, int y, int w, int h, int have_left, int have_above, int have_ar, int have_bl,
                                      LDS uint16_t *above, LDS uint16_t *left) {
-  const int bd = f->bd, rs = f->stride, tot = w + h;
+  const int bd = f->bd, rs = f->stride, tot = w + h, mi_rows = f->mi_rows, mi_cols = f->mi_cols;
   const uint16_t *rec = f->rec[plane];
-  const int max_x = f->mi_cols * 4 - 1, max_y = f->mi_rows * 4 - 1;
-  const int lim_a = imin_(max_x, x + (have_ar ? 2 * w : w) - 1), lim_l = imin_(max_y, y + (have_bl ? 2 * h : h) - 1);
   for (int i = LANE; i <= tot; i += 64) {
     const bool corner = i == tot;
-    int ia, il;
-    if (have_above) ia = (y - 1) * rs + (corner ? (have_left ? x - 1 : x) : imin_(lim_a, x + i));
-    else ia = y * rs + (have_left ? x - 1 : x);
-    if (have_left) il = imin_(lim_l, y + i) * rs + x - 1;
-    else il = (have_above ? y - 1 : y) * rs + x;
-    uint16_t a = rec[ia], l = rec[il];
-    if (!have_above && !have_left) { a = (uint16_t)(corner ? (1 << (bd - 1)) : (1 << (bd - 1)) - 1); l = (uint16_t)((1 << (bd - 1)) + 1); }
+    const EdgeAddr e = edge_addr(rs, mi_rows, mi_cols, x, y, w, h, have_left, have_above, have_ar, have_bl, i);
+    uint16_t a = rec[e.ia], l = rec[e.il];
+    edge_value(bd, have_left, have_above, corner, &a, &l);
     if (corner) { above[-1] = a; left[-1] = a; } else { above[i] = a; left[i] = l; }
   }
   WAVE_SYNC();
@@ -476,29 +470,34 @@
   const int iU = availU ? mi - ms : mi, iL = availL ? mi - 1 : mi;
   constexpr int SHAPE = BSR == BS_8X4 ? 1 : 2;
   const int have_ar = can_ar && decoded_before(r, c, SHAPE, r - 1, c + w4), have_bl = can_bl && decoded_before(r, c, SHAPE, r + h4, c - 1);
-  const int amode = availU ? uni32(f->m_ymode[iU]) : DC_PRED, lmode = availL ? uni32(f->m_ymode[iL]) : DC_PRED;
-  const int uvU = f->np > 1 ? uni32(f->m_uvmode[iU]) : 0, uvL = f->np > 1 ? uni32(f->m_uvmode[iL]) : 0;
+  const int v_ymU = f->m_ymode[iU], v_ymL = f->m_ymode[iL];
+  const int v_uvU = f->np > 1 ? f->m_uvmode[iU] : 0, v_uvL = f->np > 1 ? f->m_uvmode[iL] : 0;
   const int v_skU = f->m_skip[iU], v_skL = f->m_skip[iL], v_skUL = f->m_skip[availU && availL ? mi - ms - 1 : mi];
+  const int v_txU = f->m_txsize[iU], v_txL = f->m_txsize[iL];
+  PH_BEGIN();
+  const bool stager = W < f->np;
+  HeadStage<W_, H_> hs;
+  int hp_a = 0, hp_sv4 = 0;
+  if (stager) head_stage_issue<W_, H_>(f, t, W, r, c, availL, availU, have_ar, have_bl, hs);
+  if (W == NW - 1) {
+    const int l2 = LANE < 2 ? LANE : 0;
+    hp_a = (int)f->act[(y >> 3) * (f->pw >> 3) + (x >> 3)];
+    hp_sv4 = (int)f->svar4[(r + (HL == 3 ? l2 : 0)) * ms + c + (WL == 3 ? l2 : 0)];
+  }
+  const int amode = availU ? uni32(v_ymU) : DC_PRED, lmode = availL ? uni32(v_ymL) : DC_PRED;
+  const int uvU = uni32(v_uvU), uvL = uni32(v_uvL);
   const int nb_skip = (availU ? uni32(v_skU) & 1 : 0) + (availL ? uni32(v_skL) & 1 : 0);
   const int seg_nb = (availU && availL ? (uni32(v_skUL) >> 1) + 1 : 0) | ((availU ? (uni32(v_skU) >> 1) + 1 : 0) << 4) | ((availL ? (uni32(v_skL) >> 1) + 1 : 0) << 8);
-  const int nb_txU = availU ? uni32(f->m_txsize[iU]) : -1, nb_txL = availL ? uni32(f->m_txsize[iL]) : -1;
+  const int nb_txU = availU ? uni32(v_txU) : -1, nb_txL = availL ? uni32(v_txL) : -1;
   const uint16_t *ycost = k.cost() + CDF_KF_Y + (intra_mode_ctx(amode) * 5 + intra_mode_ctx(lmode)) * CDF_KF_Y_STRIDE;
   const int ftype_y = IS_SMOOTH_(amode) || IS_SMOOTH_(lmode);
   const int ftype_uv = f->np > 1 && ((availU && IS_SMOOTH_(uvU)) || (availL && IS_SMOOTH_(uvL)));
   LDS uint16_t *wa = S->wa + EDGE_OFF, *wl = S->wl + EDGE_OFF;
-  PH_BEGIN();
-
-  for (int p = 0; p < f->np; p++) if (p % NW == W) {
-    int sc_, dc_;
-    txb_ctx_wh(f, t, p, r, c, w4, h4, 1, &sc_, &dc_);
-    if (LANE == 0) { SH->sctx[p] = sc_; SH->dctx[p] = dc_; }
-    const uint16_t *g = f->src[p] + (size_t)y * f->stride + x;
-    for (int idx = LANE; idx < NN; idx += 64) SH->srcb[p][idx] = g[(idx >> WL) * f->stride + (idx & (W_ - 1))];
-    load_edges_wh(f, p, x, y, W_, H_, availL, availU, have_ar, have_bl, SH->ra[p] + EDGE_OFF, SH->rl[p] + EDGE_OFF);
-  }
+
+  if (stager) head_stage_consume<W_, H_, true>(f, SH, W, availL, availU, hs);
   if (W == NW - 1) {
-    const int a = (int)f->act[(y >> 3) * (f->pw >> 3) + (x >> 3)];
-    if (LANE < 2) SH->psv4[LANE] = (int)f->svar4[(r + (HL == 3 ? LANE : 0)) * ms + c + (WL == 3 ? LANE : 0)];
+    const int a = hp_a;
+    if (LANE < 2) SH->psv4[LANE] = hp_sv4;
     if (LANE == 0) { SH->pact[0] = a; SH->cact = a; SH->seg_nb = seg_nb; }
     seg_select(f, SH, a);
   }
@@ -632,8 +631,8 @@
         const int q = LANE >> 1, side = LANE & 1, rr = r + (H_ == 8 ? q : 0), cc = c + (W_ == 8 ? q : 0);
         const bool inner = q == 1 && (side == 0 ? H_ == 8 : W_ == 8);
         const bool have = !inner && (side == 0 ? (rr - 1 >= t->mi_row_start && cc < f->mi_cols) : (cc - 1 >= t->mi_col_start && rr < f->mi_rows));
-        const int ia = have ? (side == 0 ? (rr - 1) * ms + cc : rr * ms + cc - 1) : rr * ms + cc;
-        const int l = f->m_lvl[0][ia], d = f->m_dc[0][ia];
+        const int kk = inner ? 0 : q;
+        const int l = side == 0 ? SH->nb_top[kk][0] : SH->nb_left[kk][0], d = side == 0 ? SH->nb_top[kk][1] : SH->nb_left[kk][1];
         sub[8 + LANE] = have ? (l | (d << 8) | (1 << 16)) : 0;
       }
       WG_SYNC();
@@ -980,7 +979,7 @@
     fill_rect<WL, HL>(f->m_skip, ms, r, c, skip | (seg_fin << 1));
     if (skip) for (int p = 0; p < f->np; p++) { fill_rect<WL, HL>(f->m_lvl[p], ms, r, c, 0); fill_rect<WL, HL>(f->m_dc[p], ms, r, c, 0); }
   }
-  total_j += ((long long)k.cost()[CDF_SKIP + nb_skip * CDF_SKIP_STRIDE + skip] * f->rdmult + 256) >> 9;
+  total_j += ((long long)SH->part_cost[40 + nb_skip * 2 + skip] * f->rdmult + 256) >> 9;
   WG_SYNC();
   return total_j;
 }
diff --git a/cavif_rs_amd/csrc/tile_search.h b/cavif_rs_amd/csrc/tile_search.h
--- a/cavif_rs_amd/csrc/tile_search.h
+++ b/cavif_rs_amd/csrc/tile_search.h
@@ -69,7 +69,7 @@
   long long satd[13], dsd[7][6];
   long long wbest_j[4], cj[16][2], pbest_j[2];
   int order[13], wbest_e[4], pbest_c[2], calpha[2][2], ldelta[7];
-  uint16_t part_cost[40];
+  uint16_t part_cost[46];
   uint16_t lpred[N <= 32 ? 768 : 4];
   long long ca_sse[2][2]; int ca_idx[2][2];
   int lm_mode, lm_delta, lm_tx, lm_eob, ceob[2], sctx[3], dctx[3];
@@ -299,6 +299,53 @@
   if (LANE == 0) f->m_eob[plane][r * f->mi_stride + c] = (uint16_t)eob;
 }
 
+template <int W_, int H_> struct HeadStage {
+  static constexpr int NN = W_ * H_, NS = (NN + 63) / 64, NE = (W_ + H_ + 64) / 64;
+  TxbCtxAddr ca; TxbCtxVal cv;
+  uint16_t src[NS], ea[NE], el[NE];
+};
+template <int W_, int H_> __device__ __forceinline__ void head_stage_issue(const LDS FrameDev *f, const LDS TileB *t, int p, int r, int c, int have_left, int have_above,
+                                                                            int have_ar, int have_bl, HeadStage<W_, H_> &h) {
+  using H = HeadStage<W_, H_>;
+  const int rs = f->stride, x = c * 4, y = r * 4, mi_rows = f->mi_rows, mi_cols = f->mi_cols;
+  const uint16_t *g = f->src[p] + (size_t)y * rs + x, *rec = f->rec[p];
+  h.ca = txb_ctx_addr(f->mi_stride, mi_rows, mi_cols, t->mi_row_start, t->mi_col_start, r, c, W_ >> 2, H_ >> 2, LANE);
+  int so[H::NS]; EdgeAddr e[H::NE];
+#pragma unroll
+  for (int i = 0; i < H::NS; i++) { const int idx = LANE + 64 * i < H::NN ? LANE + 64 * i : 0; so[i] = (idx / W_) * rs + (idx % W_); }
+#pragma unroll
+  for (int i = 0; i < H::NE; i++) e[i] = edge_addr(rs, mi_rows, mi_cols, x, y, W_, H_, have_left, have_above, have_ar, have_bl, LANE + 64 * i);
+  h.cv = txb_ctx_load(f, p, h.ca);
+#pragma unroll
+  for (int i = 0; i < H::NS; i++) h.src[i] = g[so[i]];
+#pragma unroll
+  for (int i = 0; i < H::NE; i++) { h.ea[i] = rec[e[i].ia]; h.el[i] = rec[e[i].il]; }
+}
+template <int W_, int H_, bool keep_nb, typename SHT> __device__ __forceinline__ void head_stage_consume(const LDS FrameDev *f, LDS SHT *SH, int p, int have_left, int have_above, const HeadStage<W_, H_> &h) {
+  using H = HeadStage<W_, H_>;
+  constexpr int tot = W_ + H_;
+  int sc_, dc_;
+  txb_ctx_reduce(p, 1, h.ca, h.cv, &sc_, &dc_);
+  if constexpr (keep_nb) if (p == 0) {
+    if (LANE < (W_ >> 2)) { SH->nb_top[LANE][0] = (uint8_t)(h.ca.ha ? h.cv.la : 0); SH->nb_top[LANE][1] = (uint8_t)(h.ca.ha ? h.cv.da : 0); }
+    if (LANE < (H_ >> 2)) { SH->nb_left[LANE][0] = (uint8_t)(h.ca.hl ? h.cv.ll : 0); SH->nb_left[LANE][1] = (uint8_t)(h.ca.hl ? h.cv.dl : 0); }
+  }
+#pragma unroll
+  for (int i = 0; i < H::NS; i++) if (LANE + 64 * i < H::NN) SH->srcb[p][LANE + 64 * i] = h.src[i];
+  LDS uint16_t *above = SH->ra[p] + EDGE_OFF, *left = SH->rl[p] + EDGE_OFF;
+  const int bd = f->bd;
+#pragma unroll
+  for (int i = 0; i < H::NE; i++) {
+    const int ii = LANE + 64 * i;
+    uint16_t a = h.ea[i], l = h.el[i];
+    edge_value(bd, have_left, have_above, ii == tot, &a, &l);
+    if (ii == tot) { above[-1] = a; left[-1] = a; }
+    else if (ii < tot) { above[ii] = a; left[ii] = l; }
+  }
+  SH->sctx[p] = sc_; SH->dctx[p] = dc_;
+  WAVE_SYNC();
+}
+
 #include "dev_rect.h"
 
 template <int MAXN, int BS, int NW, int TS>
@@ -315,6 +362,19 @@
   const int v_skU = f->m_skip[iU], v_skL = f->m_skip[iL], v_txU = f->m_txsize[iU], v_txL = f->m_txsize[iL];
   const int v_skUL = f->m_skip[availU && availL ? mi - ms - 1 : mi];
   const int have_ar = can_ar && decoded_before(r, c, 0, r - 1, c + n4), have_bl = can_bl && decoded_before(r, c, 0, r + n4, c - 1);
+  PH_BEGIN();
+  static_assert(NW == 4, "the head deals its staging roles to four wavefronts (as every launch has: host_frames.h MI_LAUNCH_)");
+  constexpr int psy_cp = n >= 8 ? n / 8 : 1, psy_ncell = psy_cp * psy_cp;
+  const bool stager = W >= 1 && W - 1 < f->np;
+  HeadStage<n, n> hs;
+  int hp_a = 0, hp_sv = 0, hp_sv4 = 0;
+  if (stager) head_stage_issue<n, n>(f, t, W - 1, r, c, availL, availU, have_ar, have_bl, hs);
+  if (W == 0) {
+    const int l = LANE < psy_ncell ? LANE : 0, l4 = LANE < 4 ? LANE : 0;
+    const int cell = ((y >> 3) + l / psy_cp) * (f->pw >> 3) + (x >> 3) + l % psy_cp;
+    hp_a = (int)f->act[cell]; hp_sv = (int)(n == 4 ? f->svar4[mi] : f->svar8[cell]);
+    if constexpr (BS == 1) hp_sv4 = (int)f->svar4[(r + (l4 >> 1)) * ms + c + (l4 & 1)];
+  }
   const int amode = availU ? uni32(v_ymU) : DC_PRED, lmode = availL ? uni32(v_ymL) : DC_PRED;
   const int nb_skip = (availU ? uni32(v_skU) & 1 : 0) + (availL ? uni32(v_skL) & 1 : 0);
   const int seg_nb = (availU && availL ? (uni32(v_skUL) >> 1) + 1 : 0) | ((availU ? (uni32(v_skU) >> 1) + 1 : 0) << 4) | ((availL ? (uni32(v_skL) >> 1) + 1 : 0) << 8);
@@ -323,25 +383,13 @@
   const int ftype_y = IS_SMOOTH_(amode) || IS_SMOOTH_(lmode);
   const int ftype_uv = f->np > 1 && ((availU && IS_SMOOTH_(uni32(v_uvU))) || (availL && IS_SMOOTH_(uni32(v_uvL))));
   LDS uint16_t *wa = S->wa + EDGE_OFF, *wl = S->wl + EDGE_OFF;
-  PH_BEGIN();
-
-  for (int p = 0; p < f->np; p++) if ((p + 1) % NW == W) {
-    int sc_, dc_;
-    txb_ctx_dev(f, t, p, r, c, BS, BS, &sc_, &dc_);
-    if (LANE == 0) { SH->sctx[p] = sc_; SH->dctx[p] = dc_; }
-    const uint16_t *g = f->src[p] + (size_t)y * f->stride + x;
-    for (int idx = LANE; idx < nn; idx += 64) SH->srcb[p][idx] = g[(idx / n) * f->stride + (idx % n)];
-    load_edges(f, p, x, y, n, availL, availU, have_ar, have_bl, SH->ra[p] + EDGE_OFF, SH->rl[p] + EDGE_OFF);
-  }
+
+  if (stager) head_stage_consume<n, n, (BS > 0)>(f, SH, W - 1, availL, availU, hs);
   if (W == 0) {
-    constexpr int cp = n >= 8 ? n / 8 : 1, ncell = cp * cp;
-    const int cw = f->pw >> 3;
-    int a = 0;
-    if (LANE < ncell) {
-      const int cell = ((y >> 3) + LANE / cp) * cw + (x >> 3) + LANE % cp;
-      a = (int)f->act[cell]; SH->pact[LANE] = a; SH->psv[LANE] = (int)(n == 4 ? f->svar4[mi] : f->svar8[cell]);
-    }
-    if (BS == 1 && LANE < 4) SH->psv4[LANE] = (int)f->svar4[(r + (LANE >> 1)) * ms + c + (LANE & 1)];
+    constexpr int ncell = psy_ncell;
+    const int a = LANE < ncell ? hp_a : 0;
+    if (LANE < ncell) { SH->pact[LANE] = a; SH->psv[LANE] = hp_sv; }
+    if (BS == 1 && LANE < 4) SH->psv4[LANE] = hp_sv4;
     const int tot = wave_sum_i32(a);
     const int cact = (tot + ncell / 2) / ncell;
     if (LANE == 0) { SH->cact = cact; SH->seg_nb = seg_nb; }
@@ -591,20 +639,14 @@
         auto tr_done_ = []() {};
 #endif
         PH(13);
+        int v_psv16 = 0;
+        if constexpr (hn == 4 && n == 16) if (W == 0) v_psv16 = (int)f->svar4[(r + ((LANE & 15) >> 2)) * ms + c + (LANE & 3)];
         for (int q = W; q < G * G; q += NW) {
           const int so = (q / G) * hn * n + (q % G) * hn;
           for (int idx = LANE; idx < hnn; idx += 64) ssrc[q * hnn + idx] = SH->srcb[0][so + (idx / hn) * n + (idx % hn)];
         }
         if (W == 0) {
-          if (LANE < n4) {
-            const int k2 = LANE;
-            const bool ha = availU && c + k2 < f->mi_cols, hl = availL && r + k2 < f->mi_rows;
-            const int ia = ha ? (r - 1) * ms + c + k2 : mi, il = hl ? (r + k2) * ms + c - 1 : mi;
-            const int la = f->m_lvl[0][ia], da = f->m_dc[0][ia], ll = f->m_lvl[0][il], dl2 = f->m_dc[0][il];
-            SH->nb_top[k2][0] = (uint8_t)(ha ? la : 0); SH->nb_top[k2][1] = (uint8_t)(ha ? da : 0);
-            SH->nb_left[k2][0] = (uint8_t)(hl ? ll : 0); SH->nb_left[k2][1] = (uint8_t)(hl ? dl2 : 0);
-          }
-          if (hn == 4 && n == 16 && LANE < 16) psv16[LANE] = (int)f->svar4[(r + (LANE >> 2)) * ms + c + (LANE & 3)];
+          if (hn == 4 && n == 16 && LANE < 16) psv16[LANE] = v_psv16;
           if (LANE >= 1 && LANE < G) {
             const bool ca = c + n4 < t->mi_col_end, cb = r + n4 < t->mi_row_end;
             sfl_r[LANE] = ca && decoded_before(r, c, 0, r + LANE * half - 1, c + n4); sfl_b[LANE] = cb && decoded_before(r, c, 0, r + n4, c + LANE * half - 1);
@@ -1330,7 +1372,7 @@
     if (skip) for (int p = 0; p < f->np; p++) { fill_map_dev(f->m_lvl[p], ms, r, c, n4, 0); fill_map_dev(f->m_dc[p], ms, r, c, n4, 0); }
   }
   const int sctx = nb_skip;
-  total_j += ((long long)k.cost()[CDF_SKIP + sctx * CDF_SKIP_STRIDE + skip] * f->rdmult + 256) >> 9;
+  total_j += ((long long)SH->part_cost[40 + sctx * 2 + skip] * f->rdmult + 256) >> 9;
   if (f->seg_n && !skip) total_j += ((long long)k.cost()[CDF_SEG_ID + seg_ctx * CDF_SEG_ID_STRIDE + seg_symbol(seg_own, seg_p, f->seg_n)] * f->rdmult + 256) >> 9;
   PH(11);
   WG_SYNC();
@@ -1343,13 +1385,12 @@
   if constexpr (MAXN == 32 && BS == 4) return PH_SIZE(3, try_block64<NW>(k, r, c, budget)); else return PH_SIZE(BS < 3 ? BS : 3, (try_block<MAXN, BS, NW>(k, r, c, budget)));
 }
 
-template <int BYTES> __device__ __forceinline__ void copy_row_(void *dst, const void *src) {
-  if constexpr (BYTES == 1) *(uint8_t *)dst = *(const uint8_t *)src;
-  else if constexpr (BYTES == 2) *(uint16_t *)dst = *(const uint16_t *)src;
-  else if constexpr (BYTES == 4) *(uint32_t *)dst = *(const uint32_t *)src;
-  else if constexpr (BYTES == 8) *(uint2 *)dst = *(const uint2 *)src;
-  else { for (int i = 0; i < BYTES / 16; i++) ((uint4 *)dst)[i] = ((const uint4 *)src)[i]; }
-}
+typedef uint32_t copy_u32x2 __attribute__((vector_size(8))); typedef uint32_t copy_u32x4 __attribute__((vector_size(16))); typedef uint32_t copy_u32x8 __attribute__((vector_size(32), aligned(16)));
+template <int BYTES> struct CopyRow {
+  static_assert(BYTES == 1 || BYTES == 2 || BYTES == 4 || BYTES == 8 || BYTES == 16 || BYTES == 32, "a row of 1 .. 16 cells of one or two bytes");
+  using T = typename std::conditional<BYTES == 1, uint8_t, typename std::conditional<BYTES == 2, uint16_t, typename std::conditional<BYTES == 4, uint32_t,
+            typename std::conditional<BYTES == 8, copy_u32x2, typename std::conditional<BYTES == 16, copy_u32x4, copy_u32x8>::type>::type>::type>::type>::type;
+};
 static_assert(offsetof(FrameDev, m_eob) - offsetof(FrameDev, m_bsize) == 18 * sizeof(void *), "area_copy_dev indexes m_bsize .. m_dc[2] as one array of 18 map pointers");
 template <int BS, int NW> __device__ inline void area_copy_dev(const LDS FrameDev *f, uint8_t *snap, int r, int c, int save) {
   constexpr int n = 4 << BS, n4 = 1 << BS, Q = n / 4;
@@ -1360,31 +1401,52 @@
   uint8_t *smaps = snap + 3 * n * n * 6;
   uint8_t *seob = smaps + 18 * n4 * n4;
   const int W = NW > 1 ? WAVE_ID : 0, np = f->np, rs = f->stride, ms = f->mi_stride;
+  constexpr int PU = n * Q, PB = PU > 256 ? 4 : (PU + 63) / 64;
   for (int p = W; p < np; p += NW) {
     uint16_t *gr = f->rec[p] + (size_t)(r * 4) * rs + c * 4;
     int32_t *gc = f->coef[p] + (size_t)(r * 4) * rs + c * 4;
-    uint2 *srec = (uint2 *)(snap + (size_t)p * n * n * 2);
-    uint4 *scoef = (uint4 *)(snap + 3 * n * n * 2 + (size_t)p * n * n * 4);
-    for (int u = LANE; u < n * Q; u += 64) {
-      const int o = (u / Q) * rs + 4 * (u % Q);
-      if (save) { srec[u] = *(const uint2 *)(gr + o); scoef[u] = *(const uint4 *)(gc + o); }
-      else { *(uint2 *)(gr + o) = srec[u]; *(uint4 *)(gc + o) = scoef[u]; }
+    copy_u32x2 *srec = (copy_u32x2 *)(snap + (size_t)p * n * n * 2);
+    copy_u32x4 *scoef = (copy_u32x4 *)(snap + 3 * n * n * 2 + (size_t)p * n * n * 4);
+    for (int b = 0; b < PU; b += 64 * PB) {
+      int u[PB], o[PB]; copy_u32x2 rv[PB]; copy_u32x4 cv[PB];
+#pragma unroll
+      for (int j = 0; j < PB; j++) { u[j] = b + 64 * j + LANE < PU ? b + 64 * j + LANE : 0; o[j] = (u[j] / Q) * rs + 4 * (u[j] % Q); }
+      if (save) {
+#pragma unroll
+        for (int j = 0; j < PB; j++) { rv[j] = *(const copy_u32x2 *)(gr + o[j]); cv[j] = *(const copy_u32x4 *)(gc + o[j]); }
+#pragma unroll
+        for (int j = 0; j < PB; j++) { srec[u[j]] = rv[j]; scoef[u[j]] = cv[j]; }
+      } else {
+#pragma unroll
+        for (int j = 0; j < PB; j++) { rv[j] = srec[u[j]]; cv[j] = scoef[u[j]]; }
+#pragma unroll
+        for (int j = 0; j < PB; j++) { *(copy_u32x2 *)(gr + o[j]) = rv[j]; *(copy_u32x4 *)(gc + o[j]) = cv[j]; }
+      }
     }
   }
   if (W == NW - 1) {
     const LDS unsigned long long *mp = (const LDS unsigned long long *)&f->m_bsize;
-    for (int u = LANE; u < 17 * n4; u += 64) {
-      const int m = u / n4, row = u - m * n4, mi = m + (m >= 8);
-      if (np == 1 && (mi == 13 || mi == 14 || mi == 16 || mi == 17)) continue;
-      uint8_t *g = (uint8_t *)mp[mi] + (r + row) * ms + c, *sp = smaps + m * n4 * n4 + row * n4;
-      if (save) copy_row_<n4>(sp, g); else copy_row_<n4>(g, sp);
-    }
     const LDS unsigned long long *ep = (const LDS unsigned long long *)&f->m_eob[0];
-    for (int u = LANE; u < np * n4; u += 64) {
-      const int p = u / n4, row = u - p * n4;
-      uint8_t *g = (uint8_t *)((uint16_t *)ep[p] + (r + row) * ms + c), *sp = seob + (p * n4 * n4 + row * n4) * 2;
-      if (save) copy_row_<2 * n4>(sp, g); else copy_row_<2 * n4>(g, sp);
-    }
+    constexpr int MB = (17 * n4 + 63) / 64;
+    static_assert(3 * n4 <= 64, "one eob row per lane");
+    using MRow = typename CopyRow<n4>::T; using ERow = typename CopyRow<2 * n4>::T;
+    uint8_t *mg[MB], *msp[MB]; MRow mv[MB];
+#pragma unroll
+    for (int j = 0; j < MB; j++) {
+      const int u0 = LANE + 64 * j, m0 = u0 / n4, mi0 = m0 + (m0 >= 8);
+      const bool idle = u0 >= 17 * n4 || (np == 1 && (mi0 == 13 || mi0 == 14 || mi0 == 16 || mi0 == 17));
+      const int u = idle ? 0 : u0, m = u / n4, row = u - m * n4, mi = m + (m >= 8);
+      mg[j] = (uint8_t *)mp[mi] + (r + row) * ms + c; msp[j] = smaps + m * n4 * n4 + row * n4;
+    }
+    const int eu = LANE < np * n4 ? LANE : 0, epl = eu / n4, erow = eu - epl * n4;
+    uint8_t *eg = (uint8_t *)((uint16_t *)ep[epl] + (r + erow) * ms + c), *esp = seob + (epl * n4 * n4 + erow * n4) * 2;
+    ERow ev;
+#pragma unroll
+    for (int j = 0; j < MB; j++) mv[j] = *(const MRow *)(save ? mg[j] : msp[j]);
+    ev = *(const ERow *)(save ? eg : esp);
+#pragma unroll
+    for (int j = 0; j < MB; j++) *(MRow *)(save ? msp[j] : mg[j]) = mv[j];
+    *(ERow *)(save ? esp : eg) = ev;
   }
   WG_SYNC();
 #if MI_PROFILE
@@ -1397,7 +1459,7 @@
   if (tid < 40) {
     const int bs = tid < 16 ? 1 : 2 + (tid - 16) / 8, e = tid < 16 ? tid : (tid - 16) % 8, ctx = tid < 16 ? e >> 2 : e >> 1, part = tid < 16 ? (e & 3) : ((e & 1) ? 3 : 0);
     SH->part_cost[tid] = cost[CDF_PARTITION + ((bs - 1) * 4 + ctx) * CDF_PARTITION_STRIDE + part];
-  }
+  } else if (tid < 46) SH->part_cost[tid] = cost[CDF_SKIP + ((tid - 40) >> 1) * CDF_SKIP_STRIDE + ((tid - 40) & 1)];
 }
 __device__ __forceinline__ int part_ctx_of(int bs, int availU, int availL, int code_above, int code_left) {
   return ((availL && dim_hl(code_left) < 2 + bs) ? 2 : 0) + ((availU && dim_wl(code_above) < 2 + bs) ? 1 : 0);
@@ -1509,9 +1571,10 @@
           {
             long long j = uni64(part_j(k.sh(), f, BS, pctx, 2));
             for (int k2 = 0; k2 < 2 && j < j_best; k2++) j += uni64(PH_SIZE(5, (try_block_rect<MAXN, BS_4X8, NW>(k, r, c + k2, j_best - j))));
-            if (j < j_best) { j_best = j; rect_won = 2; area_copy_dev<BS, NW>(f, best_snap, r, c, 1); }
+            if (j < j_best) { j_best = j; rect_won = 2; }
           }
-          if (rect_won) { area_copy_dev<BS, NW>(f, best_snap, r, c, 0); return 1; }
+          if (rect_won == 1) area_copy_dev<BS, NW>(f, best_snap, r, c, 0);
+          if (rect_won) return 1;
           if (have_split) area_copy_dev<BS, NW>(f, split_snap, r, c, 0);
         }
         if (j_split < j_none && !DBG_IS(f, 7) && !DBG_IS(f, 8) && !(DBG_IS(f, 10) && BS == 1)) do_split = 1;
@@ -1590,9 +1653,10 @@
       {
         long long j = uni64(part_j(k.sh(), f, BS, pctx, 2));
         for (int k2 = 0; k2 < 2 && j < j_best; k2++) j += uni64(PH_SIZE(5, (try_block_rect<MAXN, BS_4X8, NW>(k, r, c + k2, j_best - j))));
-        if (j < j_best) { j_best = j; rect_won = 2; area_copy_dev<BS, NW>(f, best_snap, r, c, 1); }
-      }
-      if (rect_won) { area_copy_dev<BS, NW>(f, best_snap, r, c, 0); return j_best; }
+        if (j < j_best) { j_best = j; rect_won = 2; }
+      }
+      if (rect_won == 1) area_copy_dev<BS, NW>(f, best_snap, r, c, 0);
+      if (rect_won) return j_best;
       if (have_split) { area_copy_dev<BS, NW>(f, split_snap, r, c, 0); return j_split; }
     }
     if (must_split || j_split < j_none) return j_split;
```

Result: faster. 572.9 (median of 6 runs) (+2.4%).
